# xcmyz/FastVocoder

Measured on AMD Instinct MI355X. Metric: audio samples/sec + RTF @22.05kHz, HiFi-GAN-light, 1/2/4/8 MI355X, higher is better.
Workload: dtype f32 (products as split-f16 pairs, fp32 accumulate); 1 GPU; HiFi-GAN light (conf/hifigan/light.yaml) generator forward, mel 80x1000, batch 1 utterance(s) per GPU, 240000 samples each; BASELINE.json configs[1]; global_batch=1, frames=1000, parallelism=single GPU, plan_ops_per_forward=33

## Files before the change

### fastvocoder_amd/_native.py

```python
import ctypes
import os
import subprocess

import torch

_HERE = os.path.dirname(os.path.abspath(__file__))
LIB_PATH = os.path.join(_HERE, "libfastvocoder_hip.so")
_CSRC = os.path.join(_HERE, "csrc")
SOURCES = ["conv_mfma.hip", "api.hip", "plan.hip", "pack.hip", "pqmf.hip", "wav_sink.hip", "mel.hip", "resample.hip", "griffin_lim.hip", "stft_loss.hip", "stft_loss_grad.hip", "stft_mag_grad.hip", "disc.hip", "disc_grad.hip", "disc_wgrad.hip", "mpd.hip", "mpd_grad.hip", "mpd_wgrad.hip", "gen_grad.hip", "gen_grad_bf16.hip", "basis_grad.hip", "basis_learn.hip", "optim.hip", "conv_inst_narrow.hip",
           "pair_launch.hip", "pair_inst_c16.hip", "pair_inst_c32.hip", "pairh_inst_c16.hip", "pairh_inst_c32.hip",
           "convh_launch.hip", "convh_inst_c64.hip", "convh_inst_c128.hip", "convt_inst.hip",
           "convg_inst.hip", "convr_inst.hip", "convtn_inst.hip", "convk_inst.hip", "convq2_inst.hip",
           "mrfh_launch.hip", "mrfh_inst_a.hip", "mrfh_inst_b.hip", "mrfw_inst.hip", "convtl_inst.hip", "convs2_inst.hip", "convu2_inst.hip"] + \
          [f"conv_inst_s{i}.hip" for i in range(6)]
HEADERS = ["fv_internal.h", "launch_host.hpp", "conv_kernels.hpp", "pair_kernels.hpp", "pair_inst.hpp", "pairh_kernels.hpp",
           "pairh_inst.hpp", "convh_kernels.hpp", "convh_inst.hpp", "convr_kernels.hpp",
           "convtn_kernels.hpp", "convk_kernels.hpp", "convq2_kernels.hpp", "mrfh_kernels.hpp", "mrfh_inst.hpp", "mrfw_kernels.hpp", "convtl_kernels.hpp", "convs2_kernels.hpp", "convu2_kernels.hpp", "api_internal.h", "stft_core.hpp", "basis_grad_host.hpp", "wgrad_tile.hpp", "gen_grad_host.hpp"]

PAD_ZERO, PAD_REFLECT = 0, 1
PAD_CAUSAL = 2
POST_NONE, POST_TANH, POST_RELU = 0, 1, 2
SLOT_NONE, SLOT_IN, SLOT_OUT, SLOT_TMP0, MAX_SLOTS = -1, 0, 1, 2, 32
SLOT_AUX_IN0, SLOT_AUX_IN1, SLOT_OUT2 = 28, 29, 30
ABI_VERSION = 18
# ... 260 lines not shown
                                     ctypes.POINTER(f), i, i, vp]
    L.fv_mpd_conv_first.argtypes = [vp, vp, vp, vp, i, i64, i, f, vp]
    L.fv_packed_period_conv_floats.argtypes = [i, i]
    L.fv_packed_period_conv_floats.restype = i64
    L.fv_pack_period_conv.argtypes = [vp, vp, i, i, vp]
    L.fv_period_conv.argtypes = [vp, vp, vp, vp, i, i, i, i, i, f, vp]
    L.fv_packed_period_conv_grad_floats.argtypes = [i, i]
    L.fv_packed_period_conv_grad_floats.restype = i64
    L.fv_pack_period_conv_grad.argtypes = [vp, vp, i, i, vp]
    L.fv_period_conv_input_grad.argtypes = [vp, vp, vp, vp, vp, i, i, i, i, i, f, vp]
    L.fv_mpd_first_input_grad.argtypes = [vp, vp, vp, vp, vp, i, i64, i, f, vp]
    L.fv_fold_batchnorm_conv.argtypes = [vp, vp, vp, vp, vp, vp, f, vp, vp, i, i, i, vp]
    L.fv_packed_upsample_conv1d_floats.argtypes = [i, i, i, i, i]
    L.fv_packed_upsample_conv1d_floats.restype = i64
    L.fv_pack_upsample_conv1d_weight.argtypes = [vp, vp, i, i, i, i, i, vp]
    L.fv_upsample_conv1d_fused.argtypes = [vp, vp, vp, vp, vp, i, i, i, i, i, i, i, f, i, f, vp]
    L.fv_plan_add_upsample_conv1d.argtypes = [vp, i, i, i, vp, vp, i, i, i, i, i, f, i, f]
    pp = ctypes.POINTER(vp)
    L.fv_packed_pair_floats.argtypes = [i, i]
    L.fv_packed_pair_floats.restype = i64
    L.fv_pack_pair_weight.argtypes = [vp, vp, i, i, vp]
    L.fv_resblock1_fused.argtypes = [i, pp, pp, pp, pp, pp, pp, pp, ctypes.POINTER(i), i, i, i, i, f, f, vp]
    L.fv_mrf_stage.argtypes = [pp, pp, pp, pp, pp, vp, vp, ctypes.POINTER(i), i, i, i, i, f, f, i, f, vp]
    L.fv_plan_add_resblock_pair.argtypes = [vp, i, i, i, vp, vp, vp, vp, i, i, i, f, f]
    L.fv_packed_pair_floats_ex.argtypes = [i, i, i]
    L.fv_packed_pair_floats_ex.restype = i64
    L.fv_pack_pair_weight_ex.argtypes = [vp, vp, i, i, i, vp, vp]
    L.fv_resblock1_fused_ex.argtypes = [i, pp, pp, pp, pp, pp, pp, pp, pp, pp, pp, ctypes.POINTER(i), i, i, i, i, f, f,
                                        i, f, i, vp, vp]
    L.fv_plan_add_resblock_pair_ex.argtypes = [vp, i, i, i, i, i, i, vp, vp, vp, vp, i, i, i, f, f, i, f, i]
    L.fv_conv1d_split_f16.argtypes = [i, pp, pp, pp, pp, pp, pp, pp, pp, ctypes.POINTER(i), i, i, i, i, i, f, f, i, f, vp, vp]
    L.fv_plan_set_pair_output_conv.argtypes = [vp, vp, vp, i, f, i]
    L.fv_packed_mrf_stage_floats.argtypes = [i, ctypes.POINTER(i)]
    L.fv_packed_mrf_stage_floats.restype = i64
    L.fv_pack_mrf_stage_split_f16.argtypes = [pp, pp, pp, pp, vp, i, ctypes.POINTER(i), vp, vp]
    L.fv_mrf_stage_workspace_bytes.argtypes = [i]
    L.fv_mrf_stage_workspace_bytes.restype = i64
    L.fv_mrf_stage_split_f16.argtypes = [vp, vp, vp, vp, i, i, i, ctypes.POINTER(i), ctypes.POINTER(i), f, f, i, f, vp, vp, vp,
                                         vp, i64, vp, vp]
    L.fv_plan_add_mrf_stage_split_f16.argtypes = [vp, i, i, i, vp, i, ctypes.POINTER(i), ctypes.POINTER(i), f, f, i, f, vp, i64]
    L.fv_plan_add_conv1d_split_f16.argtypes = [vp, i, i, i, i, i, i, vp, vp, i, i, i, i, f, f, i, f]
    L.fv_plan_add_mrf_sum.argtypes = [vp, ctypes.POINTER(i), i, i, pp, pp, pp, pp, i, ctypes.POINTER(i), i, f, f, i, f]
    L.fv_plan_create.argtypes = [i]
    L.fv_plan_create.restype = vp
    L.fv_plan_destroy.argtypes = [vp]
    L.fv_plan_destroy.restype = None
    L.fv_plan_add_conv1d.argtypes = [vp, i, i, i, i, i, i, vp, vp, i, i, i, i, i, i, f, f, i, f]
    L.fv_plan_add_conv_transpose1d.argtypes = [vp, i, i, i, vp, vp, i, i, i, i, i, i, f, i, f]
    L.fv_plan_add_pqmf_synthesis.argtypes = [vp, i, i, vp, i, i]
    L.fv_plan_set_guard.argtypes = [vp, vp]
    L.fv_plan_check_range.argtypes = [vp, vp]
    L.fv_tuning_set.argtypes = [ctypes.c_char_p, i]
    L.fv_debug_pair_schedule.argtypes = [i, ctypes.POINTER(i), ctypes.POINTER(i), i, i, i, ctypes.POINTER(ctypes.c_uint)]
    L.fv_plan_set_group.argtypes = [vp, i]
    L.fv_plan_output_shape.argtypes = [vp, i, ctypes.POINTER(i), ctypes.POINTER(i64)]
    L.fv_plan_workspace_bytes.argtypes = [vp, i, i]
    L.fv_plan_workspace_bytes.restype = i64
    L.fv_plan_run.argtypes = [vp, i, i, vp, vp, vp, i64, vp]
    L.fv_plan_run_aux.argtypes = [vp, i, i, vp, vp, vp, ctypes.POINTER(vp), ctypes.POINTER(i), vp, i64, vp]
    L.fv_plan_set_output_offset.argtypes = [vp, i, i]
    L.fv_plan_slot_shape.argtypes = [vp, i, i, ctypes.POINTER(i), ctypes.POINTER(i64)]
    L.fv_plan_num_ops.argtypes = [vp]
    L.fv_profile_enable.argtypes = [i]
    L.fv_profile_bracket_cost.argtypes = [vp, i, ctypes.POINTER(ctypes.c_double)]
    L.fv_profile_mfma_f16_rate.argtypes = [vp, i64, i, i, vp, ctypes.POINTER(ctypes.c_double)]
    L.fv_profile_collect.argtypes = [i, ctypes.POINTER(i64), ctypes.POINTER(ctypes.c_double),
                                     ctypes.POINTER(ctypes.c_double), ctypes.POINTER(ctypes.c_double)]
    if L.fv_version() != ABI_VERSION:
        raise NativeError(f"ABI mismatch: library reports {L.fv_version()}, binding expects {ABI_VERSION}")
    _lib = L
    return L


def check(rc):
    if rc != 0:
        raise NativeError(f"libfastvocoder_hip error {rc}: {lib().fv_last_error().decode()}")


def _ptr(t, name="tensor", allow_none=False):
    if t is None:
        if allow_none:
            return None
        raise NativeError(f"{name} is None")
    if not t.is_cuda:
        raise NativeError(f"{name} lives on {t.device}; the HIP kernels need a ROCm device "
                          "tensor (there is no CPU path in fastvocoder_amd)")
    if t.dtype != torch.float32 or not t.is_contiguous():
        raise NativeError(f"{name} must be contiguous float32, got {t.dtype} "
                          f"contiguous={t.is_contiguous()}")
    return t.data_ptr()


class _on:

    def __init__(self, *tensors):
        devs = {t.device for t in tensors if t is not None}
        if len(devs) != 1:
            raise NativeError(f"operands of a native call must share one ROCm device, got {sorted(map(str, devs))}")
        self.dev = devs.pop()
        if self.dev.type != "cuda":
            raise NativeError(f"operands live on {self.dev}; the HIP kernels need a ROCm device tensor "
                              "(there is no CPU path in fastvocoder_amd)")
        self._guard = torch.cuda.device(self.dev)

    def __enter__(self):
        self._guard.__enter__()
        return torch.cuda.current_stream(self.dev).cuda_stream

    def __exit__(self, *exc):
        return self._guard.__exit__(*exc)


class GuardWord:

    def __init__(self):
        self.t = torch.zeros(2, dtype=torch.int32).pin_memory()

    def ptr(self, i=0):
        return self.t.data_ptr() + 4 * i

    def peek(self, i=0):
        return int(self.t[i])

    def clear(self, i=0):
        self.t[i] = 0


def tuning_set(key, value):
    check(lib().fv_tuning_set(key.encode(), int(value)))


def debug_pair_schedule(n_items, cost, nblk, mode=0, three_members=False):
    n = len(n_items)
    arr = ctypes.c_int * n
    table = (ctypes.c_uint * 512)()
    rc = lib().fv_debug_pair_schedule(n, arr(*[int(v) for v in n_items]), arr(*[int(v) for v in cost]), int(nblk), int(mode),
                                      1 if three_members else 0, table)
    check(rc if rc < 0 else 0)
    if rc == 1:
        out = []
        for b in range(nblk):
            w0, w1 = table[2 * b], table[2 * b + 1]
            e = [w0 & 0xFFFF, w0 >> 16, w1 & 0xFFFF]
            out.append([(v & 2047, v >> 11) for v in e[:n]])
        return 1, out
    if rc == 2:
        return 2, [int(table[i]) for i in range(nblk)]
    return 0, None


def _flag_ptr(flag):
    if flag is None:
        return None
    if isinstance(flag, GuardWord):
        return flag.ptr(1)
    if isinstance(flag, int):
        return flag
    return flag.data_ptr()


def _guard_ptr(guard):
    if guard is None:
        return None
    if isinstance(guard, GuardWord):
        return guard.ptr(0)
    return guard.data_ptr()



def fold_weight_norm(v, g):
    v = v.detach().contiguous().float()
    g = g.detach().contiguous().float()
    w = torch.empty_like(v)
    with _on(v, g) as stream:
        check(lib().fv_fold_weight_norm(_ptr(v, "v"), _ptr(g, "g"), _ptr(w), v.shape[0], v[0].numel(), stream))
    return w


def pack_conv1d(w):
    w = w.detach().contiguous().float()
    cout, cin, k = w.shape
    out = torch.empty(lib().fv_packed_conv1d_floats(cout, cin, k), dtype=torch.float32, device=w.device)
    with _on(w) as stream:
        check(lib().fv_pack_conv1d_weight(_ptr(w, "w"), _ptr(out), cout, cin, k, stream))
    return out


def pack_conv_transpose1d(w, stride, pad):
    w = w.detach().contiguous().float()
    cin, cout, k = w.shape
    n = lib().fv_packed_conv_transpose1d_floats(cin, cout, k, stride, pad)
    out = torch.empty(n, dtype=torch.float32, device=w.device)
    with _on(w) as stream:
        check(lib().fv_pack_conv_transpose1d_weight(_ptr(w, "w"), _ptr(out), cin, cout, k, stride, pad, stream))
    return out


def conv_transpose_split_supported(cin, cout, k, stride, pad, out_pad):
    if conv_transpose_small(cin, cout, k, stride):
        return pad == 1 and out_pad == 0
    return (cin in (32, 64, 128, 256, 512) and 2 <= stride <= 16 and k == 2 * stride and cout * stride >= 32
# ... 170 lines not shown
def mrf_stage_workspace(channels, device):
    n = lib().fv_mrf_stage_workspace_bytes(int(channels))
    return torch.empty((n + 3) // 4, dtype=torch.float32, device=device) if n > 0 else None


def _work_args(work):
    return (_ptr(work, "workspace", True), 0 if work is None else work.numel() * 4)


def pack_mrf_stage(w1s, w2s, b1s, b2s, ks, flag=None):
    w1s = [w.detach().contiguous().float() for w in w1s]
    w2s = [w.detach().contiguous().float() for w in w2s]
    b1s = [None if b is None else b.detach().contiguous().float() for b in b1s]
    b2s = [None if b is None else b.detach().contiguous().float() for b in b2s]
    if not (len(w1s) == len(w2s) == len(b1s) == len(b2s) == 9 and len(ks) == 3):
        raise NativeError("pack_mrf_stage: nine pairs (three ResBlocks x three positions) expected")
    c = w1s[0].shape[0]
    for i, w in enumerate(w1s + w2s):
        if tuple(w.shape) != (c, c, ks[(i % 9) // 3]):
            raise NativeError(f"pack_mrf_stage: weight {i} has shape {tuple(w.shape)}, expected {(c, c, ks[(i % 9) // 3])}")
    karr = (ctypes.c_int * 3)(*ks)
    nfl = lib().fv_packed_mrf_stage_floats(c, karr)
    if nfl <= 0:
        raise NativeError(f"pack_mrf_stage: no packed layout for C={c} taps={list(ks)}")
    out = torch.empty(nfl, dtype=torch.float32, device=w1s[0].device)
    with _on(*w1s, *w2s, *b1s, *b2s, out) as stream:
        check(lib().fv_pack_mrf_stage_split_f16(_vp_array(w1s, "w1"), _vp_array(w2s, "w2"), _vp_array(b1s, "b1", True),
                                                _vp_array(b2s, "b2", True), _ptr(out), c, karr, _flag_ptr(flag), stream))
    return out


def mrf_stage_split_f16(x, packed, ks, dils=MRF_STAGE_DILATIONS, slope=0.1, out_div=3.0, post=POST_NONE, act_slope=1.0,
                        out=None, out_act=None, fold=None, guard=None):
    B, C, T = x.shape
    karr, darr = (ctypes.c_int * 3)(*ks), (ctypes.c_int * 3)(*dils)
    work = mrf_stage_workspace(C, x.device)
    if fold is not None:
        fw, fb = fold
        fw = fw.detach().contiguous().float()
        fb = None if fb is None else fb.detach().contiguous().float()
        res = torch.empty((B, 1, T), dtype=torch.float32, device=x.device)
        with _on(x, packed, fw, fb, res) as stream:
            check(lib().fv_mrf_stage_split_f16(_ptr(x, "x"), _ptr(packed, "packed"), None, None, B, C, T, karr, darr,
                                               float(slope), float(out_div), post, float(act_slope), _ptr(fw, "fold_w"),
                                               _ptr(fb, "fold_b", True), _ptr(res), *_work_args(work), _guard_ptr(guard), stream))
        return res
    if out is None:
        out = torch.empty_like(x)
    with _on(x, packed, out, out_act, work) as stream:
        check(lib().fv_mrf_stage_split_f16(_ptr(x, "x"), _ptr(packed, "packed"), _ptr(out, "y"), _ptr(out_act, "y_act", True),
                                           B, C, T, karr, darr, float(slope), float(out_div), post, float(act_slope), None,
                                           None, None, *_work_args(work), _guard_ptr(guard), stream))
    return out


def mrf_stage(xs, w1s, w2s, b1s, b2s, ks, dil, slope, out_div=3.0, post=POST_NONE, act_slope=1.0, out=None,
              out_act=None):
    B, C, T = xs[0].shape
    if out is None:
        out = torch.empty_like(xs[0])
    with _on(*xs, *w1s, *w2s, *b1s, *b2s, out, out_act) as stream:
        check(lib().fv_mrf_stage(_vp_array(xs, "x"), _vp_array(w1s, "w1"), _vp_array(w2s, "w2"),
                                 _vp_array(b1s, "b1", True), _vp_array(b2s, "b2", True), _ptr(out, "y"),
                                 _ptr(out_act, "y_act", True), (ctypes.c_int * 3)(*ks), B, C, T, dil, float(slope),
                                 float(out_div), post, float(act_slope), stream))
    return out


def conv1d_fused(x, packed, bias, cout, k, dil=1, pad=0, pad_mode=PAD_ZERO, pre_slope=1.0,
                 res=None, acc_in=None, out_div=1.0, post=POST_NONE, out=None, out_act=None,
                 act_slope=1.0, acc_in2=None):
    B, cin, T = x.shape
    tout = T if pad_mode & PAD_CAUSAL else T + 2 * pad - dil * (k - 1)
    if out is None:
        out = torch.empty((B, cout, tout), dtype=torch.float32, device=x.device)
    with _on(x, packed, bias, res, acc_in, acc_in2, out, out_act) as stream:
        check(lib().fv_conv1d_fused(_ptr(x, "x"), _ptr(packed, "packed"), _ptr(bias, "bias", True),
                                    _ptr(res, "res", True), _ptr(acc_in, "acc_in", True),
                                    _ptr(acc_in2, "acc_in2", True), _ptr(out, "out"),
                                    _ptr(out_act, "out_act", True), B, cin, cout, T, k, dil, pad, pad_mode,
                                    float(pre_slope), float(out_div), post, float(act_slope), stream))
    return out


def conv1d_2src_fused(x, x2, packed, bias, cout, res=None, post=POST_NONE, out=None, out_act=None,
                      act_slope=1.0):
    B, c1, T = x.shape
    c2 = x2.shape[1]
    if out is None:
        out = torch.empty((B, cout, T), dtype=torch.float32, device=x.device)
    with _on(x, x2, packed, bias, res, out, out_act) as stream:
        check(lib().fv_conv1d_2src_fused(_ptr(x, "x"), _ptr(x2, "x2"), _ptr(packed, "packed"),
                                         _ptr(bias, "bias", True), _ptr(res, "res", True), _ptr(out, "out"),
                                         _ptr(out_act, "out_act", True), B, c1, c2, cout, T, post,
                                         float(act_slope), stream))
    return out


def conv1x1_2src_split_f16(x, x2, packed, bias, pre_slope=1.0, res=None, post=POST_NONE, out=None, out_act=None,
                           act_slope=1.0, guard=None):
    B, c, T = x.shape
    if out is None:
        out = torch.empty_like(x)
    with _on(x, x2, packed, bias, res, out, out_act) as stream:
        check(lib().fv_conv1x1_2src_split_f16(_ptr(x, "x"), _ptr(x2, "x2"), _ptr(packed, "packed"), _ptr(bias, "bias", True),
                                              _ptr(res, "res", True), _ptr(out, "out"), _ptr(out_act, "out_act", True), B, c,
# ... 1049 lines not shown
        for b in (bias_dilated, bias_out):
            if b is not None:
                self.keep(b)
        check(lib().fv_plan_add_residual_stack_split_f16(self._h, x, y, y_act, _ptr(packed, "packed"),
                                                         _ptr(bias_dilated, "bias_dilated", True), _ptr(bias_out, "bias_out", True),
                                                         channels, k, dil, float(slope), pad_mode, post, float(act_slope)))
        if two_launch is not None:
            hidden, pd, pp = two_launch
            self.keep(pd)
            self.keep(pp)
            check(lib().fv_plan_set_stack_two_launch(self._h, hidden, _ptr(pd, "packed_dilated"), _ptr(pp, "packed_pair")))

    def add_upsample_conv1d(self, x, y, packed, bias, cin, cout, k, rate, pad, pre_slope=1.0,
                            post=POST_NONE, y_act=SLOT_NONE, act_slope=1.0):
        self.keep(packed)
        if bias is not None:
            self.keep(bias)
        check(lib().fv_plan_add_upsample_conv1d(self._h, x, y, y_act, _ptr(packed, "packed"),
                                                _ptr(bias, "bias", True), cin, cout, k, rate, pad,
                                                float(pre_slope), post, float(act_slope)))

    def add_conv1d_sum3(self, xs, ress, tmps, y, packed, bias_sum, channels, ks, out_div=1.0, post=POST_NONE,
                        y_act=SLOT_NONE, act_slope=1.0):
        for t in packed:
            self.keep(t)
        if bias_sum is not None:
            self.keep(bias_sum)
        i3 = ctypes.c_int * 3
        wp = (ctypes.c_void_p * 3)(*[_ptr(t, "packed") for t in packed])
        check(lib().fv_plan_add_conv1d_sum3(self._h, i3(*xs), i3(*ress), (ctypes.c_int * 2)(*tmps), y, y_act, wp,
                                            _ptr(bias_sum, "bias_sum", True), channels, i3(*ks),
                                            float(out_div), post, float(act_slope)))

    def add_resblock_pair(self, x, y, packed1, packed2, bias1, bias2, channels, k, dil, slope,
                          y_act=SLOT_NONE, act_slope=1.0, prec=PAIR_F32, add1=SLOT_NONE, add2=SLOT_NONE,
                          out_div=1.0, post=POST_NONE, mid=SLOT_NONE):
        for t in (packed1, packed2, bias1, bias2):
            if t is not None:
                self.keep(t)
        check(lib().fv_plan_add_resblock_pair_ex(self._h, x, y, y_act, mid, add1, add2, _ptr(packed1, "packed1"),
                                                 _ptr(packed2, "packed2"), _ptr(bias1, "bias1", True),
                                                 _ptr(bias2, "bias2", True), channels, k, dil, float(slope),
                                                 float(out_div), post, float(act_slope), prec))

    def add_mrf_stage(self, x, y, packed, channels, ks, dils, slope, out_div=3.0, post=POST_NONE, y_act=SLOT_NONE,
                      act_slope=1.0):
        self.keep(packed)
        work = mrf_stage_workspace(channels, packed.device)
        if work is not None:
            self.keep(work)
        check(lib().fv_plan_add_mrf_stage_split_f16(self._h, x, y, y_act, _ptr(packed, "packed"), channels,
                                                    (ctypes.c_int * 3)(*ks), (ctypes.c_int * 3)(*dils), float(slope),
                                                    float(out_div), post, float(act_slope), *_work_args(work)))

    def set_pair_output_conv(self, w, bias, y, act_slope, post=POST_NONE):
        self.keep(w)
        if bias is not None:
            self.keep(bias)
        check(lib().fv_plan_set_pair_output_conv(self._h, _ptr(w, "w"), _ptr(bias, "bias", True), y, float(act_slope), post))

    def add_conv1d_split_f16(self, x, y, packed, bias, channels, k, dil, pre_slope=1.0, res=SLOT_NONE, add1=SLOT_NONE,
                             add2=SLOT_NONE, out_div=1.0, post=POST_NONE, y_act=SLOT_NONE, act_slope=1.0,
                             pad_mode=PAD_ZERO):
        for t in (packed, bias):
            if t is not None:
                self.keep(t)
        check(lib().fv_plan_add_conv1d_split_f16(self._h, x, y, y_act, res, add1, add2, _ptr(packed, "packed"),
                                                 _ptr(bias, "bias", True), channels, k, dil, pad_mode,
                                                 float(pre_slope), float(out_div), post, float(act_slope)))

    def add_mrf_sum(self, xs, y, packed1, packed2, bias1, bias2, channels, ks, dil, slope, out_div=3.0,
                    post=POST_NONE, y_act=SLOT_NONE, act_slope=1.0):
        for t in list(packed1) + list(packed2) + list(bias1) + list(bias2):
            if t is not None:
                self.keep(t)
        i3 = ctypes.c_int * 3
        check(lib().fv_plan_add_mrf_sum(self._h, i3(*xs), y, y_act, _vp_array(packed1, "packed1"),
                                        _vp_array(packed2, "packed2"), _vp_array(bias1, "bias1", True),
                                        _vp_array(bias2, "bias2", True), channels, i3(*ks), dil, float(slope),
                                        float(out_div), post, float(act_slope)))

    def set_sum_order(self, own_first):
        check(lib().fv_plan_set_sum_order(self._h, 1 if own_first else 0))

    def set_guard(self, guard):
        self._guard = self.keep(guard) if guard is not None else None
        check(lib().fv_plan_set_guard(self._h, guard.ptr(0) if guard is not None else None))

    def check_range(self):
        if self._guard is None:
            return False
        rc = lib().fv_plan_check_range(self._h, torch.cuda.current_stream(self._dev).cuda_stream)
        if rc == ERR_RANGE:
            return True
        if rc == ERR_RANGE_LOW:
            return "low"
        check(rc)
        return False

    def set_group(self, group):
        check(lib().fv_plan_set_group(self._h, group))

    def add_pqmf_synthesis(self, x, y, h):
        self.keep(h)
        check(lib().fv_plan_add_pqmf_synthesis(self._h, x, y, _ptr(h, "h"), h.shape[0], h.shape[1]))

# ... 129 lines not shown
```

### fastvocoder_amd/csrc/api.hip

```cpp
#include <stdarg.h>
#include <stdio.h>
#include <stdlib.h>

#include <string>
#include <mutex>
#include <utility>
#include <vector>

#include <ctype.h>
#include <string.h>
#include <unistd.h>

#include "api_internal.h"
#include "launch_host.hpp"

namespace fv {

static thread_local std::string g_err;

int fail(int code, const char* fmt, ...) {
    char buf[512];
    va_list ap;
    va_start(ap, fmt);
    vsnprintf(buf, sizeof(buf), fmt, ap);
// ... 182 lines not shown
    pp.T = (int)T;
    pp.slope = o.pre_slope;
    pp.act_slope = o.act_slope;
    pp.out_div = o.out_div;
    pp.post = o.post;
    pp.prec = o.prec;
    pp.guard = guard;
    pp.reflect = (o.pad_mode & FV_PAD_REFLECT) ? 1 : 0;
    pp.sub = sub;
    pp.sub_batched = sub_batched;
    return pp;
}

PairMember pair_member(const float* x, const float* w1, const float* w2, const float* b1, const float* b2, int k, float* y,
                       float* y_act, const float* res, const float* add1, const float* add2, const float* x2) {
    PairMember mb = {};
    mb.x = x;
    mb.x2 = x2;
    mb.w1 = w1;
    mb.w2 = w2;
    mb.b1 = b1;
    mb.b2 = b2;
    mb.k = k;
    mb.y = y;
    mb.y_act = y_act;
    mb.res = res;
    mb.add1 = add1;
    mb.add2 = add2;
    return mb;
}

MrfParams mrf_params(const Op& o, const float* x, float* y, float* y_act, float* fold_y, int B, int64_t T, int* guard) {
    MrfParams mp = {};
    mp.x = x;
    mp.y = y;
    mp.y_act = y_act;
    mp.blob = o.wp;
    for (int j = 0; j < 3; ++j) mp.k[j] = o.pk[j];
    mp.B = B;
    mp.T = (int)T;
    mp.slope = o.pre_slope;
    mp.out_div = o.out_div;
    mp.act_slope = o.act_slope;
    mp.post = o.post;
    mp.fold_w = o.fold_w;
    mp.fold_b = o.fold_b;
    mp.fold_y = fold_y;
    mp.guard = guard;
    mp.hist = static_cast<float*>(o.work);
    mp.hist_bytes = o.work_bytes;
    return mp;
}

int check_pad_mode(int pad_mode, int pad, int k, int dil) {
    if (pad_mode < 0 || pad_mode > (FV_PAD_REFLECT | FV_PAD_CAUSAL))
        return fail(FV_ERR_INVALID_ARG, "unknown pad_mode %d", pad_mode);
    if ((pad_mode & FV_PAD_CAUSAL) && 2LL * pad < (int64_t)dil * (k - 1))
        return fail(FV_ERR_INVALID_ARG, "causal conv: pad=%d leaves fewer than Tin outputs (k=%d dil=%d)",
                    pad, k, dil);
    return 0;
}

int check_conv_args(int Cin, int Cout, int k, int dil) {
    if (Cin <= 0 || Cout <= 0 || k <= 0 || dil <= 0)
        return fail(FV_ERR_INVALID_ARG, "bad conv shape Cin=%d Cout=%d k=%d dil=%d", Cin, Cout, k, dil);
    return 0;
}

int check_convt_split_args(int Cin, int Cout, int k, int stride, int pad, int out_pad) {
    if (Cin != 32 && Cin != 64 && Cin != 128 && Cin != 256 && Cin != 512)
        return fail(FV_ERR_UNSUPPORTED, "conv_transpose1d_split_f16: Cin = %d (32, 64, 128, 256 or 512)", Cin);
    if (stride < 2 || stride > 16 || k != 2 * stride)
        return fail(FV_ERR_UNSUPPORTED, "conv_transpose1d_split_f16: kernel %d, stride %d (kernel = 2 x stride, stride 2..16)", k, stride);
    if (Cout <= 0 || Cout * stride < 32)
        return fail(FV_ERR_UNSUPPORTED, "conv_transpose1d_split_f16: Cout * stride = %d (32 or more)", Cout * stride);
    if (pad < 0 || pad > stride || out_pad < -stride || out_pad >= stride)
        return fail(FV_ERR_INVALID_ARG, "conv_transpose1d_split_f16: pad=%d (0..stride) out_pad=%d", pad, out_pad);
    if (convtn_shape(Cin, Cout, k, stride) && (pad != 1 || out_pad != 0))
        return fail(FV_ERR_UNSUPPORTED, "conv_transpose1d_split_f16: 32 -> 16 channels, kernel 4, stride 2 exists with pad=1, "
                    "out_pad=0 only (got %d, %d)", pad, out_pad);
    return 0;
}

}

using namespace fv;

namespace fv {
int allow_dynamic_lds(const void* kernel, size_t bytes) {
    if (bytes <= 64 * 1024) return 0;
    struct Grant { const void* kernel; int device; size_t bytes; };
    static std::mutex mu;
    static std::vector<Grant> granted;
    int dev = 0;
    FV_HIP(hipGetDevice(&dev));
    std::lock_guard<std::mutex> lock(mu);
    for (Grant& g : granted)
        if (g.kernel == kernel && g.device == dev) {
            if (g.bytes >= bytes) return 0;
            FV_HIP(hipFuncSetAttribute(kernel, hipFuncAttributeMaxDynamicSharedMemorySize, (int)bytes));
            g.bytes = bytes;
            return 0;
        }
    FV_HIP(hipFuncSetAttribute(kernel, hipFuncAttributeMaxDynamicSharedMemorySize, (int)bytes));
    granted.push_back({kernel, dev, bytes});
    return 0;
}

static Tuning g_tuning;
static std::once_flag g_tuning_once;
struct TuningEntry {
    const char* key;
    int Tuning::*field;
};
static const TuningEntry kTuningTable[] = {
    {"pair_dbg", &Tuning::pair_dbg},       {"dbg", &Tuning::conv_dbg},           {"sched", &Tuning::sched},
    {"sched_switch", &Tuning::sched_switch}, {"convh_skel", &Tuning::convh_skel}, {"convp_skel", &Tuning::convp_skel},
    {"convq_skel", &Tuning::convq_skel},   {"pair128_unfused", &Tuning::pair128_unfused},
    {"convg_rows64", &Tuning::convg_rows64}, {"stack_items", &Tuning::stack_items}, {"stack_wide", &Tuning::stack_wide},
    {"convp_wide", &Tuning::convp_wide},   {"convq_wide", &Tuning::convq_wide},
    {"convh_rows64", &Tuning::convh_rows64},  {"convt_rows64", &Tuning::convt_rows64},
    {"pairh_skel", &Tuning::pairh_skel},   {"pair_skel", &Tuning::pair_skel},    {"convh_blocks", &Tuning::convh_blocks},
    {"pair_blocks", &Tuning::pair_blocks}, {"sum3_min", &Tuning::sum3_min},      {"lds_budget", &Tuning::lds_budget},
    {"units", &Tuning::units},             {"shape16", &Tuning::shape16},        {"shape32", &Tuning::shape32},
    {"shape64", &Tuning::shape64},         {"krows", &Tuning::krows},            {"grid_cap", &Tuning::grid_cap},
    {"no_group", &Tuning::no_group},       {"mrf_blocks", &Tuning::mrf_blocks},  {"mrf_shape", &Tuning::mrf_shape},
    {"mrf_prio", &Tuning::mrf_prio},       {"convt_lean", &Tuning::convt_lean},
    {"convs_ringfree", &Tuning::convs_ringfree}, {"convu_resident", &Tuning::convu_resident},
};
static void tuning_from_env() {
    const char* on = getenv("FV_TUNING");
    if (!on || atoi(on) != 1) return;
    for (const TuningEntry& e : kTuningTable) {
        char name[64] = "FV_";
        size_t n = 3;
        for (const char* c = e.key; *c && n + 1 < sizeof(name); ++c) name[n++] = (char)toupper((unsigned char)*c);
        name[n] = 0;
        const char* v = getenv(name);
        if (v && *v) g_tuning.*(e.field) = atoi(v);
    }
    const char* tp = getenv("FV_PAIR_TRACE_PTR");
    if (tp && *tp) g_tuning.trace_ptr = strtoull(tp, nullptr, 0);
}
const Tuning& tuning() {
    std::call_once(g_tuning_once, tuning_from_env);
    return g_tuning;
}

int device_cu_count() {
    static int cus = 0;
    if (!cus) {
        int dev = 0, v = 0;
        cus = hipGetDevice(&dev) == hipSuccess &&
                      hipDeviceGetAttribute(&v, hipDeviceAttributeMultiprocessorCount, dev) == hipSuccess && v > 0
                  ? v : 256;
    }
    return cus;
}
}

extern "C" {

int fv_version(void) { return FV_ABI_VERSION; }


#ifndef FV_BUILD_ID
#define FV_BUILD_ID "unknown"
#endif
const char* fv_build_id(void) { return "fv-build-id:" FV_BUILD_ID + 12; }

const char* fv_last_error(void) { return g_err.c_str(); }

int fv_upsample_conv1d_fused(const float* x, const float* packed, const float* bias, float* y,
                             float* y_act, int B, int Cin, int Cout, int Tin, int k, int rate, int pad,
                             float pre_slope, int post, float act_slope, void* stream) {
    if (int rc = check_conv_args(Cin, Cout, k, 1)) return rc;
    if (!x || !packed || !y) return fail(FV_ERR_INVALID_ARG, "upsample_conv1d: null tensor");
    if (rate <= 0 || pad < 0) return fail(FV_ERR_INVALID_ARG, "upsample_conv1d: rate=%d pad=%d", rate, pad);
    if (x == y || x == y_act || (y_act && y_act == y))
        return fail(FV_ERR_INVALID_ARG, "upsample_conv1d: y / y_act must not alias x or each other");
// ... 718 lines not shown
    }
    return launch_pair_family(pp, mid, C, dil, prec, (hipStream_t)stream);
}

int fv_mrf_stage(const float* const* x, const float* const* w1, const float* const* w2, const float* const* b1,
                 const float* const* b2, float* y, float* y_act, const int* k, int B, int C, int T, int dil,
                 float slope, float out_div, int post, float act_slope, void* stream) {
    if (!x || !w1 || !w2 || !y || !k) return fail(FV_ERR_INVALID_ARG, "mrf_stage: null argument");
    if (int rc = check_pair_args(3, C, k, dil)) return rc;
    PairParams pp = pair_params(pair_op(OP_MRFSUM, C, dil, FV_PAD_ZERO, slope, out_div, post, act_slope, FV_PAIR_F32), 3, B, T, nullptr);
    pp.sum = 1;
    for (int j = 0; j < 3; ++j) {
        if (!x[j] || x[j] == y || x[j] == y_act || (y_act && y_act == y))
            return fail(FV_ERR_INVALID_ARG, "mrf_stage: member %d: null input, or y / y_act aliases an input or each other", j);
        pp.m[j] = pair_member(x[j], w1[j], w2[j], at(b1, j), at(b2, j), k[j], y, y_act);
    }
    return launch_pairs(pp, C, dil, (hipStream_t)stream);
}

}

namespace fv {
int check_stage_args(int C, const int* k, const int* dil, float slope, float act_slope, int post) {
    if (!k || !dil) return fail(FV_ERR_INVALID_ARG, "mrf stage: null taps / dilations");
    if (!mrf_stage_shape(C, k, dil))
        return fail(FV_ERR_UNSUPPORTED, "mrf stage: C = %d, taps (%d, %d, %d), dilations (%d, %d, %d): built for 16 / 32 channels, "
                    "taps 3 / 7 / 11, dilations (1, 3, 5)", C, k[0], k[1], k[2], dil[0], dil[1], dil[2]);
    if (int rc = check_slopes("mrf stage", slope, act_slope)) return rc;
    if (post != FV_POST_NONE && post != FV_POST_TANH && post != FV_POST_RELU) return fail(FV_ERR_INVALID_ARG, "mrf stage: post %d", post);
    return 0;
}
}

extern "C" {

int64_t fv_mrf_stage_workspace_bytes(int C) { return mrf_workspace_bytes(C); }

int fv_mrf_stage_split_f16(const float* x, const float* packed, float* y, float* y_act, int B, int C, int T, const int* k,
                           const int* dil, float slope, float out_div, int post, float act_slope, const float* fold_w,
                           const float* fold_b, float* fold_y, void* workspace, int64_t workspace_bytes, int* guard,
                           void* stream) {
    if (int rc = check_stage_args(C, k, dil, slope, act_slope, post)) return rc;
    if (B < 0 || T < 0) return fail(FV_ERR_INVALID_ARG, "mrf stage: B=%d T=%d", B, T);
    Op o = pair_op(OP_STAGE, C, dil[0], FV_PAD_ZERO, slope, out_div, post, act_slope, FV_PAIR_SPLIT_F16);
    o.wp = packed;
    for (int j = 0; j < 3; ++j) o.pk[j] = k[j];
    o.fold_w = fold_w;
    o.fold_b = fold_b;
    o.work = workspace;
    o.work_bytes = workspace_bytes;
    return launch_mrfh(mrf_params(o, x, y, y_act, fold_y, B, T, guard), C, dil, (hipStream_t)stream);
}

}

namespace fv {
int check_convh_args(int n, int C, const int* k, int dil, int pad_mode) {
    if (pad_mode != FV_PAD_ZERO && pad_mode != FV_PAD_REFLECT)
        return fail(FV_ERR_UNSUPPORTED, "conv1d_split_f16: pad_mode %d (FV_PAD_ZERO or FV_PAD_REFLECT)", pad_mode);
    if (n < 1 || n > 3) return fail(FV_ERR_INVALID_ARG, "conv1d_split_f16: %d members (1..3)", n);
    if (C != 64 && C != 128 && C != 256 && C != 512)
        return fail(FV_ERR_UNSUPPORTED, "conv1d_split_f16: C = %d (64, 128, 256 or 512)", C);
    if (dil != 1 && dil != 3 && dil != 5 && dil != 9)
        return fail(FV_ERR_UNSUPPORTED, "conv1d_split_f16: dilation %d (1, 3, 5; 9 with 3 taps)", dil);
    for (int j = 0; j < n; ++j)
        if ((k[j] != 3 && k[j] != 7 && k[j] != 11) || (dil == 9 && k[j] != 3))
            return fail(FV_ERR_UNSUPPORTED, "conv1d_split_f16: %d taps at dilation %d (3, 7 or 11; 3 at dilation 9)", k[j], dil);
    return 0;
}
}

extern "C" {

int fv_conv1d_split_f16(int n, const float* const* x, const float* const* packed, const float* const* bias,
                        const float* const* res, const float* const* add1, const float* const* add2, float* const* y,
                        float* const* y_act, const int* k, int B, int C, int T, int dil, int pad_mode, float pre_slope,
                        float out_div, int post, float act_slope, int* guard, void* stream) {
    if (!x || !packed || !y || !k) return fail(FV_ERR_INVALID_ARG, "conv1d_split_f16: null argument");
    if (int rc = check_convh_args(n, C, k, dil, pad_mode)) return rc;
    PairParams pp = pair_params(pair_op(OP_CONVH, C, dil, pad_mode, pre_slope, out_div, post, act_slope, FV_PAIR_SPLIT_F16), n, B, T, guard);
    for (int j = 0; j < n; ++j) {
        const PairMember& mb = pp.m[j] = pair_member(x[j], packed[j], nullptr, at(bias, j), nullptr, k[j], y[j], at(y_act, j),
                                                     at(res, j), at(add1, j), at(add2, j));
        if (!mb.x || !mb.y || mb.x == mb.y || mb.y == mb.res || mb.y == mb.add1 || mb.y == mb.add2 ||
            (mb.y_act && (mb.y_act == mb.y || mb.y_act == mb.x || mb.y_act == mb.res)))
            return fail(FV_ERR_INVALID_ARG, "conv1d_split_f16: member %d: null tensor or an output aliases an input", j);
    }
    return launch_convh(pp, C, dil, (hipStream_t)stream);
}

int fv_div_probe(unsigned first_bits, int64_t n, float d, unsigned long long* mismatches, void* stream) {
    if (!mismatches || n <= 0) return fail(FV_ERR_INVALID_ARG, "div_probe: null counter / empty range");
    return fv::launch_div_probe(first_bits, (long long)n, d, mismatches, (hipStream_t)stream);
}

int fv_tuning_set(const char* key, int value) {
    if (!key) return fail(FV_ERR_INVALID_ARG, "tuning_set: null key");
    (void)tuning();
    for (const TuningEntry& e : kTuningTable)
        if (strcmp(e.key, key) == 0) {
            g_tuning.*(e.field) = value;
            return 0;
        }
    static const char* const kRetiredKeys[] = {"convp_pp"};
    for (const char* retired : kRetiredKeys)
        if (value == 0 && strcmp(retired, key) == 0) return 0;
// ... 135 lines not shown
```

### fastvocoder_amd/csrc/api_internal.h

```cpp
#pragma once
#include <stdint.h>

#include <vector>

#include "fv_internal.h"

namespace fv {

enum OpType { OP_CONV = 0, OP_CONVT = 1, OP_PQMF = 2, OP_UPCONV = 3, OP_PAIR = 4, OP_MRFSUM = 5, OP_CONVH = 6, OP_CONVG = 7, OP_STACK = 8, OP_STAGE = 9 };

struct Op {
    int type;
    int x, y, res, acc, y2, acc2;
    int group;
    const float* wp;
    const float* bias;
    const float* bias2 = nullptr;
    const float* alt_w1 = nullptr;
    const float* alt_w2 = nullptr;
    int alt_mid = FV_SLOT_NONE;
    int Cin, Cout, k, dil, pad, pad_mode, stride, out_pad;
    float pre_slope, out_div, act_slope;
    int post;
    int x2 = FV_SLOT_NONE;
    int Cin1 = 0;
    int own_first = 0;
    bool sum3 = false;
    int xb = FV_SLOT_NONE, xc = FV_SLOT_NONE, resb = FV_SLOT_NONE, resc = FV_SLOT_NONE;
    int tmpb = FV_SLOT_NONE, tmpc = FV_SLOT_NONE;
    const float* wpb = nullptr;
    const float* wpc = nullptr;
    int kb = 0, kc = 0;
    const float* pw1[3] = {nullptr, nullptr, nullptr};
    const float* pw2[3] = {nullptr, nullptr, nullptr};
    const float* pb1[3] = {nullptr, nullptr, nullptr};
    const float* pb2[3] = {nullptr, nullptr, nullptr};
    int pk[3] = {0, 0, 0};
    int sdil[3] = {0, 0, 0};
    void* work = nullptr;
    int64_t work_bytes = 0;
    int prec = 0;
    bool in_merge = false;
    const float* fold_w = nullptr;
    const float* fold_b = nullptr;
    int sub = FV_SLOT_NONE;
    const float* pq_h = nullptr;
    int pq_taps = 0;
};

struct Shape {
    int C;
    int64_t T;
    bool set;
};

}

struct fv_plan {
    int in_channels;
    std::vector<fv::Op> ops;
    int cur_group = 0;
    int cur_own_first = 0;
    int* guard_host = nullptr;
    int* guard_dev = nullptr;
};

namespace fv {

int64_t conv_out_len(const Op& o, int64_t Tin);
ConvParams make_params(const Op& o, const float* x, float* y, float* y2, const float* res,
                              const float* acc, const float* acc2, int B, int64_t Tin,
                              const float* x2 = nullptr, const float* sub = nullptr, int sub_batched = 0);
int run_op(const Op& o, const float* x, float* y, float* y2, const float* res, const float* acc,
                  const float* acc2, int B, int64_t Tin, hipStream_t s, const float* x2 = nullptr,
                  const float* sub = nullptr, int sub_batched = 0, int* guard = nullptr);
int check_pad_mode(int pad_mode, int pad, int k, int dil);
int check_stack_args(int C, int k, int dil, int pad_mode, float slope, float act_slope, int post = FV_POST_NONE);

inline float* ptr(float* const* base, int slot) { return slot == FV_SLOT_NONE ? nullptr : base[slot]; }
PairParams pair_params(const Op& o, int n_members, int B, int64_t T, int* guard, const float* sub = nullptr, int sub_batched = 0);
PairMember pair_member(const float* x, const float* w1, const float* w2, const float* b1, const float* b2, int k, float* y,
                       float* y_act, const float* res = nullptr, const float* add1 = nullptr, const float* add2 = nullptr,
                       const float* x2 = nullptr);
MrfParams mrf_params(const Op& o, const float* x, float* y, float* y_act, float* fold_y, int B, int64_t T, int* guard);
int launch_pair_family(const PairParams& pp, float* const* mid, int C, int dil, int prec, hipStream_t s);
int check_pair_args(int n, int C, const int* k, int dil, int prec = FV_PAIR_F32);
int check_stage_args(int C, const int* k, const int* dil, float slope, float act_slope, int post);
int check_convh_args(int n, int C, const int* k, int dil, int pad_mode);

}
```

### fastvocoder_amd/csrc/convtn_kernels.hpp

```cpp
#pragma once
#include "pairh_kernels.hpp"

namespace fv {

struct ConvTnParams {
    const float* x;
    const float* add1;
    const float* add2;
    const float* w;
    const float* bias;
    float* y;
    float* y_act;
    int B, T, Tout, n_tiles;
    float slope, act_slope, out_div;
    int* guard;
};

constexpr int kTnCin = 32, kTnCout = 16, kTnCols = 256, kTnRows = 260, kTnRP = 272;
constexpr int kTnHalf = (kTnCin / 8) * kTnRP * 16;
constexpr int kTnImageFloats = 2 * 2 * 2 * 64 * 8 / 2;

__global__ __launch_bounds__(256) __attribute__((amdgpu_waves_per_eu(2, 2))) void convtn_kernel(ConvTnParams p) {
    typedef __attribute__((address_space(3))) const f16x8 LdsH8;
    __shared__ __attribute__((aligned(16))) char ximg[2 * kTnHalf];
    __shared__ unsigned lowbits[4];
    const int tid = threadIdx.x, lane = tid & 63;
    const int wave = __builtin_amdgcn_readfirstlane(tid >> 6);
    const int b = (int)blockIdx.x / p.n_tiles, tile = (int)blockIdx.x - b * p.n_tiles;
    const int u0 = tile * kTnCols;
    const size_t xoff = (size_t)b * kTnCin * (size_t)p.T;
    const unsigned xbytes = (unsigned)kTnCin * (unsigned)p.T * 4u, t4 = (unsigned)p.T * 4u;
    const __amdgpu_buffer_rsrc_t r0 = make_rsrc(p.x + xoff, xbytes);
    const __amdgpu_buffer_rsrc_t r1 = make_rsrc(p.add1 ? p.add1 + xoff : p.x, p.add1 ? xbytes : 0u);
    const __amdgpu_buffer_rsrc_t r2 = make_rsrc(p.add2 ? p.add2 + xoff : p.x, p.add2 ? xbytes : 0u);
    constexpr int TASKS = kTnRows * (kTnCin / 8), NR = (TASKS + 255) / 256;
    float v[NR][8], a1[NR][8], a2[NR][8];
    const bool merge = p.add1 != nullptr;
#pragma unroll
    for (int q = 0; q < NR; ++q) {
        const int idx = tid + q * 256;
        const int cb = idx / kTnRows, row = idx - cb * kTnRows;
        const int t = u0 - 1 + row;
        const unsigned voff = idx < TASKS && t >= 0 && t < p.T ? (unsigned)(cb * 8 * p.T + t) * 4u : kOutOfRange;
#pragma unroll
        for (int j = 0; j < 8; ++j) v[q][j] = buffer_load1s(r0, voff, (unsigned)j * t4);
        if (merge) {
#pragma unroll
            for (int j = 0; j < 8; ++j) a1[q][j] = buffer_load1s(r1, voff, (unsigned)j * t4);
#pragma unroll
            for (int j = 0; j < 8; ++j) a2[q][j] = buffer_load1s(r2, voff, (unsigned)j * t4);
        }
    }
    pair_wait_vm0();
    float lowm = 0.f;
    const float rcp = div_rcp(p.out_div);
#pragma unroll
    for (int q = 0; q < NR; ++q) {
        const int idx = tid + q * 256;
        const int cb = idx / kTnRows, row = idx - cb * kTnRows;
        if (idx < TASKS) {
            F16x8Parts h1, h2;
#pragma unroll
            for (int j = 0; j < 4; ++j) {
                f32x2 raw = {v[q][2 * j], v[q][2 * j + 1]};
                if (merge) {
                    raw = (raw + f32x2{a1[q][2 * j], a1[q][2 * j + 1]}) + f32x2{a2[q][2 * j], a2[q][2 * j + 1]};
                    if (p.out_div != 1.f) {
                        raw.x = rcp != 0.f ? div_exact(raw.x, p.out_div, rcp) : raw.x / p.out_div;
                        raw.y = rcp != 0.f ? div_exact(raw.y, p.out_div, rcp) : raw.y / p.out_div;
                    }
                }
                const f32x2 a = split_act2(raw, p.slope);
                lowm = low_max3(lowm, a.x, a.y);
                split2(a, h1.p[j], h2.p[j]);
            }
            *reinterpret_cast<f16x8*>(ximg + (cb * kTnRP + row) * 16) = __builtin_bit_cast(f16x8, h1);
            *reinterpret_cast<f16x8*>(ximg + (cb * kTnRP + row) * 16 + kTnHalf) = __builtin_bit_cast(f16x8, h2);
        }
    }
    f16x8 A[2][2][2];
    {
        const f16x8* wl = reinterpret_cast<const f16x8*>(p.w) + lane;
#pragma unroll
        for (int s = 0; s < 2; ++s)
#pragma unroll
            for (int h = 0; h < 2; ++h)
#pragma unroll
                for (int e = 0; e < 2; ++e) A[s][h][e] = wl[((s * 2 + h) * 2 + e) * 64];
    }
    LowGuard low;
    low_note(low, 0, lowm);
    if (p.guard && lane == 0) lowbits[wave] = low.bits;
    pair_barrier();
    if (p.guard && tid == 0) {
        const unsigned all = lowbits[0] | lowbits[1] | lowbits[2] | lowbits[3];
        if ((all & 2u) && !(all & 1u)) guard_raise_low(p.guard);
    }
    const int n = lane & 15, kb = lane >> 4;
    const int col0 = wave * 64 + n;
    LdsCF* const bb = lds_opaque(reinterpret_cast<const float*>(ximg + (kb * kTnRP + col0) * 16));
    f32x4 hi[2][4], lo[2][4];
#pragma unroll
    for (int h = 0; h < 2; ++h)
#pragma unroll
        for (int f = 0; f < 4; ++f) hi[h][f] = lo[h][f] = f32x4{0.f, 0.f, 0.f, 0.f};
#pragma unroll
    for (int s = 0; s < 2; ++s) {
        f16x8 B1[4], B2[4];
#pragma unroll
        for (int f = 0; f < 4; ++f) {
            B1[f] = *reinterpret_cast<LdsH8*>(bb + (s * 16 + f * 256) / 4);
            B2[f] = *reinterpret_cast<LdsH8*>(bb + (s * 16 + f * 256 + kTnHalf) / 4);
        }
#pragma unroll
        for (int h = 0; h < 2; ++h)
#pragma unroll
            for (int f = 0; f < 4; ++f) hi[h][f] = __builtin_amdgcn_mfma_f32_16x16x32_f16(A[s][h][0], B1[f], hi[h][f], 0, 0, 0);
#pragma unroll
        for (int h = 0; h < 2; ++h)
// ... 58 lines not shown
```

### fastvocoder_amd/csrc/fv_internal.h

```cpp
#pragma once
#include <hip/hip_runtime.h>

#include <vector>
#include <stdint.h>

#include "../../include/fastvocoder_hip.h"

namespace fv {

int fail(int code, const char* fmt, ...);

#define FV_HIP(call)                                                              \
    do {                                                                          \
        hipError_t e_ = (call);                                                   \
        if (e_ != hipSuccess)                                                     \
            return ::fv::fail((int)e_, "%s failed: %s", #call, hipGetErrorString(e_)); \
    } while (0)

static inline int round_up(int v, int m) { return (v + m - 1) / m * m; }

int check_conv_args(int Cin, int Cout, int k, int dil);
int check_convt_split_args(int Cin, int Cout, int k, int stride, int pad, int out_pad);

static inline int pad_rows(int M) { return M <= 16 ? 16 : round_up(M, 32); }
// ... 54 lines not shown
    int nchunks;
    int xw;
    int ncol4;
    int ncol4c;
    unsigned ncol4c_magic;
    int xbuf, wbuf;
    int n_tiles;
    int m_tiles, tiles_per_run;
    int nx_inst, nw_inst;
    int red_off;
    int vec_ok;
    int dbg;
    double alg_flops;
};

struct GroupParams {
    ConvParams p[3];
    int grid_x[3];
};

struct Sum3Params {
    ConvParams p[3];
    int xbuf_max, wbuf_max;
};
int launch_conv_sum3(ConvParams* ps, hipStream_t stream);

int allow_dynamic_lds(const void* kernel, size_t bytes);
int device_cu_count();
struct Tuning {
    int pair_dbg = 0;
    int conv_dbg = 0;
    int sched = 1;
    int sched_switch = 4;
    int convh_skel = -1;
    int convp_skel = 5;
    int convq_skel = -1;
    int pair128_unfused = 0;
    int convh_rows64 = -1;
    int convt_rows64 = -1;
    int convs_ringfree = -1;
    int convu_resident = 1;
    int convt_lean = 50;
    int convq_wide = 20;
    int convp_wide = 20;
    int stack_wide = 10;
    int stack_items = 1 << 20;
    int convg_rows64 = -1;
    int pairh_skel = -1;
    int pair_skel = -1;
    int convh_blocks = 0;
    int pair_blocks = 0;
    int mrf_blocks = 0;
    int mrf_shape = 0;
    int mrf_prio = 1;
    int sum3_min = 800;
    int lds_budget = 39;
    int units = 500;
    int shape16 = -1, shape32 = -1, shape64 = -1;
    int krows = 176;
    int grid_cap = 1024;
    int no_group = 0;
    unsigned long long trace_ptr = 0;
};
const Tuning& tuning();

struct PairMember {
    const float* x;
    const float* x2;
    const float* w1;
    const float* w2;
    const float* b1;
    const float* b2;
    float* y;
    float* y_act;
    const float* res;
    int n_items;
    const float* add1;
    const float* add2;
    int k;
    int cost;
    int n_tiles;
    int w_off;
};

constexpr int kSchedBlocks = 256;

struct PairCore {
    PairMember m[3];
    int n_members;
    int sum;
    int B, T;
    int n_out_sum;
    float slope;
    float out_div;
    float act_slope;
    int post;
    int nblk;
    int ctot, nch, nmt;
    const float* fold_w;
    const float* fold_b;
    float* fold_y;
    const float* sub;
    int sub_batched;
    int* guard;
    int sched_on;
    int reflect;
// ... 81 lines not shown
int launch_pair_geom(const PairParams& p, int dil, size_t lds, hipStream_t s);
template <int MH, int NF, int NG>
int launch_pairh_geom(const PairParams& p, int dil, size_t lds, hipStream_t s);

struct MrfParams {
    const float* x;
    float* y;
    float* y_act;
    const float* blob;
    unsigned blob_bytes;
    unsigned blk_off[9];
    int k[3];
    int B, T;
    int halo;
    int ol;
    float slope;
    float out_div;
    float act_slope;
    int post;
    const float* fold_w;
    const float* fold_b;
    float* fold_y;
    int* guard;
    int nblk;
    long long total;
    int prio;
    unsigned long long* trace;
    float* hist;
    long long hist_bytes;
};

inline int mrf_block_bytes(int C, int k) { return 2 * ((k + (32 / C) - 1) / (32 / C)) * (C / 16) * 2048 + 1024; }
inline bool mrf_stage_shape(int C, const int* k, const int* dil) {
    if ((C != 16 && C != 32) || !k || !dil || dil[0] != 1 || dil[1] != 3 || dil[2] != 5) return false;
    for (int j = 0; j < 3; ++j)
        if (k[j] != 3 && k[j] != 7 && k[j] != 11) return false;
    return true;
}
inline int mrf_halo(const int* k, const int* dil) {
    int h = 0;
    for (int j = 0; j < 3; ++j) {
        int r = 0;
        for (int q = 0; q < 3; ++q) r += (k[j] - 1) * dil[q] / 2 + (k[j] - 1) / 2;
        if (r > h) h = r;
    }
    return h;
}
int launch_mrfh(MrfParams p, int C, const int* dil, hipStream_t stream);
template <int NF, int NG>
int launch_mrfh_geom(const MrfParams& p, hipStream_t s);
constexpr int kMrfwHistBytes = 9 * 30 * 128;
long long mrf_workspace_bytes(int C);
int launch_mrfw_geom(const MrfParams& p, hipStream_t s);

#ifndef FV_RING
#define FV_RING 2
#endif
constexpr int kRingStages(bool slow, bool act) { return (slow || act) ? 2 : FV_RING; }
constexpr int kMaxDmaX = 6, kMaxDmaW = 8;

struct PqmfTail {
    const float* h;
    float* y;
    float* y2;
    const float* sub;
    int sub_batched;
    int ntaps;
    int tail_off;
};
constexpr int kPqmfHalo = 8, kPqmfAdvance = 256 - 2 * kPqmfHalo;
int launch_conv_post_pqmf(ConvParams p, const float* h, int ntaps, float* y, float* y2, const float* sub, int sub_batched,
                          hipStream_t stream);

int launch_conv(ConvParams p, hipStream_t stream);
int launch_conv_group(ConvParams* ps, int n, hipStream_t stream);
int launch_pqmf(const float* x, const float* h, float* y, float* y2, const float* sub, int sub_batched, int B, int S,
                int ntaps, int Tsub, hipStream_t stream);
int launch_encode16(float* x, int B, int64_t n, float rescale, short* out, unsigned* peak_bits,
                    int scale_in_place, hipStream_t s);
int launch_pqmf_analysis(const float* xin, const float* ha, float* x, int B, int S, int ntaps,
                         int64_t T, hipStream_t s);
int launch_melspectrogram(const float* x, float* mel, const float* tab, int B, int64_t n, hipStream_t s);
int launch_stft_complex(const float* y, float* spec, const float* tab, int B, int64_t n, hipStream_t s);
int launch_istft(const float* spec, float* y, const float* tab, int B, int T, float* frames, hipStream_t s);
int launch_griffin_lim(const float* S, const float* phase0, float* y, const float* tab, int B, int T, int iters,
                       float* frames, hipStream_t s);
int launch_mel_to_linear(const float* mel, const float* invb, float* S, int B, int T, float power, hipStream_t s);
int launch_inv_preemphasis(const float* y, float* out, int B, int64_t n, float coef, hipStream_t s);
static inline int64_t resample_window(int L, int M, int half) {
    return ((int64_t)L - 1 + 255 * (int64_t)M) / L + 2 * (int64_t)half + 2;
}
int launch_resample(const void* x, int format, float* y, const float* tab, int B, int64_t n_in, int64_t n_out, int L,
                    int M, int half, hipStream_t s);
int64_t stft_chunks(int64_t n, int hop);
int launch_stft_distance(const float* x, const float* y, const float* const* tables, int B, int64_t n, int R,
                         const int* nfft, const int* hop, const int* win, double* out, double* ws, hipStream_t s);
int launch_stft_magnitude(const float* x, float* mag, const float* tab, int B, int64_t n, int nfft, int hop, int win,
                          hipStream_t s, bool bins_major = false);
int64_t stft_grad_chunks(int64_t n, int hop);
int launch_stft_distance_grad(const float* x, const float* y, const float* const* tables, int B, int64_t n, int R,
                              const int* nfft, const int* hop, const int* win, const float* coef, float* gx,
                              float* ws, hipStream_t s);
int launch_stft_grad_ola(const float* ws, const float* tab, int B, int64_t n, int nfft, int hop, int win, float* gx,
                         hipStream_t s);
int64_t stft_mag_grad_chunks(int64_t n, int hop);
int launch_stft_magnitude_bins_grad(const float* x, const float* gmag, const float* tab, int B, int64_t n, int nfft,
// ... 35 lines not shown
```

### fastvocoder_amd/csrc/mrfh_launch.hip

```cpp
#include "launch_host.hpp"

namespace fv {

extern template int launch_mrfh_geom<3, 12>(const MrfParams&, hipStream_t);
extern template int launch_mrfh_geom<2, 16>(const MrfParams&, hipStream_t);

static long long mrfw_max_blocks() {
    const long long cus = device_cu_count(), asked = tuning().mrf_blocks;
    return asked > cus ? asked : cus;
}
long long mrf_workspace_bytes(int C) { return C == 32 ? mrfw_max_blocks() * kMrfwHistBytes : 0; }

int launch_mrfh(MrfParams p, int C, const int* dil, hipStream_t s) {
    const char* const fam = "mrf stage";
    if (p.B <= 0 || p.T <= 0) return 0;
    if (!mrf_stage_shape(C, p.k, dil))
        return fail(FV_ERR_UNSUPPORTED, "mrf stage: C = %d, taps (%d, %d, %d), dilations (%d, %d, %d): built for 16 / 32 channels, taps "
                    "3 / 7 / 11, dilations (1, 3, 5)", C, p.k[0], p.k[1], p.k[2], dil ? dil[0] : 0, dil ? dil[1] : 0, dil ? dil[2] : 0);
    const bool fold = p.fold_w != nullptr;
    if (!p.x || !p.blob || (!fold && !p.y) || (fold && (!p.fold_y || p.y || p.y_act)))
        return fail(FV_ERR_INVALID_ARG, "mrf stage: null tensor (or both an output tensor and a folded output conv)");
    if (p.y == p.x || p.y_act == p.x || (p.y_act && p.y_act == p.y) || p.fold_y == p.x)
        return fail(FV_ERR_INVALID_ARG, "mrf stage: an output tensor aliases the input (or y_act aliases y)");
    if ((reinterpret_cast<uintptr_t>(p.blob) & 15) != 0) return fail(FV_ERR_UNSUPPORTED, "mrf stage: the packed stage must be 16-byte aligned");
    if (int rc = check_desc_range(fam, C, p.T)) return rc;
    if ((double)p.B * p.T >= 2147483647.0) return fail(FV_ERR_UNSUPPORTED, "mrf stage: B x T = %d x %d columns exceed 2^31", p.B, p.T);
    if (int rc = check_slopes(fam, p.slope, p.act_slope)) return rc;
    unsigned off = 0;
    double flops = 0;
    for (int j = 0; j < 3; ++j)
        for (int q = 0; q < 3; ++q) {
            p.blk_off[3 * j + q] = off;
            off += (unsigned)mrf_block_bytes(C, p.k[j]);
            flops += 2.0 * 2.0 * p.B * (double)C * C * p.k[j] * p.T;
        }
    p.blob_bytes = off;
    p.halo = mrf_halo(p.k, dil);
    p.ol = fold ? 3 : 0;
    p.total = (long long)p.B * p.T;
    const int shape = tuning().mrf_shape;
    const int W = C == 32 ? 384 : shape == 1 ? 512 : 576;
    const int vcols = W - p.halo, adv = vcols - 2 * p.ol;
    if (adv < 64) return fail(FV_ERR_UNSUPPORTED, "mrf stage: a %d-column window leaves %d final columns", W, adv);
    long long nblk = persistent_blocks((p.total + 127) / 128, 1, tuning().mrf_blocks);
    if (nblk < 1) nblk = 1;
    p.nblk = (int)nblk;
    if (C == 32) {
        if (!p.hist || p.hist_bytes < nblk * kMrfwHistBytes || (reinterpret_cast<uintptr_t>(p.hist) & 15) != 0)
            return fail(FV_ERR_WORKSPACE, "mrf stage: 32 channels need a 16-byte aligned workspace of fv_mrf_stage_workspace_bytes "
                        "(%lld bytes for %lld blocks; given %lld)", nblk * kMrfwHistBytes, nblk, p.hist ? p.hist_bytes : 0LL);
    } else {
        p.hist = nullptr;
    }
    p.prio = tuning().mrf_prio;
    p.trace = trace_buffer();
    double bytes = 4.0 * ((double)p.B * C * p.T * (fold ? 1.0 : (p.y_act ? 3.0 : 2.0)) + (fold ? (double)p.B * p.T : 0.0)) + off;
    if (fold) flops += 2.0 * p.B * (double)C * 7 * p.T;
    ProfileScope prof(s, C == 32 ? FV_KERNEL_MRF32 : FV_KERNEL_MRF16, Work{flops, bytes});
    return C == 32 ? launch_mrfw_geom(p, s) : shape == 1 ? launch_mrfh_geom<2, 16>(p, s) : launch_mrfh_geom<3, 12>(p, s);
}

}
```

### fastvocoder_amd/csrc/mrfw_inst.hip

```cpp
#include "mrfw_kernels.hpp"

namespace fv {

int launch_mrfw_geom(const MrfParams& p, hipStream_t s) {
    typedef MrfwTile<3, 8> TL;
    static_assert(9 * TL::HSLOT == kMrfwHistBytes, "history bytes per block");
    auto kern = p.fold_w ? mrfw_kernel<3, 8, 1, 3, 5, true> : mrfw_kernel<3, 8, 1, 3, 5, false>;
    if (int rc = allow_dynamic_lds(reinterpret_cast<const void*>(kern), TL::LDS)) return rc;
    hipLaunchKernelGGL(kern, dim3(p.nblk), dim3(TL::NT), TL::LDS, s, p);
    FV_HIP(hipGetLastError());
    return 0;
}

}
```

### fastvocoder_amd/csrc/mrfw_kernels.hpp

```cpp
#pragma once
#include "mrfh_kernels.hpp"

namespace fv {

template <int NF_, int NG_>
struct MrfwTile {
    static constexpr int NF = NF_, NG = NG_, C = 32;
    static constexpr int NT = 64 * NG;
    static constexpr int W = 16 * NF * NG;
    static constexpr int FM = 32;
    static constexpr int RP = W + 2 * FM;
    static constexpr int BLK = RP * 16;
    static constexpr int HALF = 4 * BLK;
    static constexpr int IMG = 2 * HALF;
    static constexpr int PT = 4;
    static constexpr int STEP = 4096;
    static constexpr int PIECE = PT * STEP;
    static constexpr int TAIL = 512;
    static constexpr int HROW = 128;
    static constexpr int HX = 0, HM = 25 * HROW, HSLOT = 30 * HROW;
    static constexpr int OFF_W = 0, OFF_X = 2 * PIECE, OFF_M = OFF_X + IMG, OFF_B = OFF_M + IMG, OFF_S = OFF_B + 9 * TAIL;
    static constexpr int OFF_F = OFF_S + 256;
    static constexpr int LDS = OFF_F + 1024;
    static_assert(W * 128 <= IMG, "FOLD: the activated fp32 tile [column][32 channels] lies over the intermediate image");
    static_assert(RP % 16 == 0, "whole bank rows");
    static_assert(NG >= 5 && NG <= 8, "history copies: waves 0 ... 4; a piece is at most two LDS-DMA instructions per wave");
    static_assert(LDS <= 160 * 1024, "LDS");
};

template <class TL>
struct MrfwLane {
    int tid, lane, wave;
    int colw;
    int row0;
    int rdoff;
    int wroff;
    int cpslot;
    int cpimg;
    char* sm;
};

template <int NG>
__device__ __forceinline__ void mrfw_dma(__amdgpu_buffer_rsrc_t rb, float* dst, unsigned off, int kb, int wave, int lane) {
#pragma unroll
    for (int r = 0; r < 2; ++r) {
        const int i = wave + r * NG;
        if (i < kb) dma16(rb, dst + i * 256, off + (unsigned)(i * 1024 + lane * 16));
    }
}

template <int NF, int STEPS, int TAPB, int HALF>
__device__ __forceinline__ void mrfw_mma(const float* wl, const char* img, f32x4 (&hi)[2][NF], f32x4 (&lo)[2][NF], int lane) {
    typedef __attribute__((address_space(3))) const f16x8 LdsH8;
// ... 175 lines not shown
    mrfw_conv<TL, KT, 16>(p, L, wbuf, par, mimg + (rdoff - P2 * 16), hi, lo, rb, pair_off + (unsigned)WB, next_off, next_kb);
    mrf_stamp(p, TL::NG, L.wave, L.lane, tile_no, 7 * q + 4);
    {
        u32x4 hv = {0u, 0u, 0u, 0u};
        if (wv == 4) {
            if (wh.save && cpslot < TL::HROW * P2) hv = *reinterpret_cast<const u32x4*>(mimg + cpimg + (TL::FM + wh.adv - P2) * 16);
        } else if (wv < 4) {
            if (!wh.zero_next && cpslot < TL::HROW * pnext) hv = __builtin_bit_cast(u32x4, __builtin_amdgcn_raw_buffer_load_b128(rh, hq_next + TL::HX + cpslot, 0, 0));
        }
#pragma unroll
        for (int h = 0; h < 2; ++h) {
            const f32x2* const b2 = reinterpret_cast<const f32x2*>(bl + 32 + 16 * h + row0);
            const f32x2* const s2 = reinterpret_cast<const f32x2*>(bl + 96 + 16 * h + row0);
            const f32x2 b01 = b2[0], b23 = b2[1], s01 = s2[0], s23 = s2[1];
            if (wh.inside) {
#pragma unroll
                for (int f = 0; f < NF; ++f) {
                    combine4(hi[h][f], lo[h][f], s01, s23, b01, b23, xr[h][f]);
#pragma unroll
                    for (int i = 0; i < 4; ++i) xr[h][f][i] = hi[h][f][i];
                }
            } else {
                int cm = colw;
                asm volatile("" : "+v"(cm));
#pragma unroll
                for (int f = 0; f < NF; ++f) {
                    combine4(hi[h][f], lo[h][f], s01, s23, b01, b23, xr[h][f]);
                    const int t = wh.tw + cm + f * 16;
                    const bool ok = t >= 0 && t < p.T;
#pragma unroll
                    for (int i = 0; i < 4; ++i) xr[h][f][i] = ok ? hi[h][f][i] : 0.f;
                }
            }
        }
        if (wv == 4) {
            if (wh.save && cpslot < TL::HROW * P2) __builtin_amdgcn_raw_buffer_store_b128(hv, rh, hq + TL::HM + cpslot, 0, 0);
        }
        if constexpr (NEXT == 0) mrfw_write_x<TL>(ximg + wroff, xr, p.slope, low);
        else if (write_next) mrfw_write_x<TL>(ximg + wroff, x0, p.slope, low);
        if (wv < 4) {
            if (cpslot < TL::HROW * pnext) *reinterpret_cast<u32x4*>(ximg + cpimg + (TL::FM - pnext) * 16) = hv;
        }
    }
    mrf_stamp(p, TL::NG, L.wave, L.lane, tile_no, 7 * q + 5);
    pair_wait_vm0();
    mrf_stamp(p, TL::NG, L.wave, L.lane, tile_no, 7 * q + 6);
    pair_barrier();
}

template <class TL, int KT, int D0, int D1, int D2>
__device__ __forceinline__ void mrfw_block_run(const MrfParams& p, const MrfwLane<TL>& L, float* wbuf, int& par, int j, int pnext,
                                               float (&xr)[2][TL::NF][4], const float (&x0)[2][TL::NF][4], bool write_next,
                                               MrfwWhen wh, bool zero_after, LowGuard& low, __amdgpu_buffer_rsrc_t rb,
                                               __amdgpu_buffer_rsrc_t rh, unsigned next_off, int next_kb, int tile_no) {
    constexpr int KB0 = 4 * mrfw_piece_taps(KT, 0);
    const int q0 = 3 * j;
    const float* const bl = reinterpret_cast<const float*>(L.sm + TL::OFF_B) + q0 * (TL::TAIL / 4);
    const int h0 = q0 * TL::HSLOT, hn = (j == 2 ? 0 : q0 + 3) * TL::HSLOT;
    const unsigned o0 = p.blk_off[q0], o1 = p.blk_off[q0 + 1], o2 = p.blk_off[q0 + 2];
    mrfw_pair<TL, KT, D0, 0>(p, L, wbuf, par, bl, xr, x0, true, wh, h0, h0 + TL::HSLOT, (KT - 1) * D1 / 2, low, rb, rh, o0, o1, KB0,
                             tile_no, q0);
    mrfw_pair<TL, KT, D1, 0>(p, L, wbuf, par, bl + TL::TAIL / 4, xr, x0, true, wh, h0 + TL::HSLOT, h0 + 2 * TL::HSLOT,
                             (KT - 1) * D2 / 2, low, rb, rh, o1, o2, KB0, tile_no, q0 + 1);
    wh.zero_next = zero_after;
    mrfw_pair<TL, KT, D2, 1>(p, L, wbuf, par, bl + 2 * (TL::TAIL / 4), xr, x0, write_next, wh, h0 + 2 * TL::HSLOT, hn, pnext, low, rb,
                             rh, o2, next_off, next_kb, tile_no, q0 + 2);
}

template <int NF, int NG, int D0, int D1, int D2, bool FOLD>
__global__ __launch_bounds__(64 * NG) __attribute__((amdgpu_waves_per_eu((NG + 3) / 4, (NG + 3) / 4))) void mrfw_kernel(MrfParams p) {
    typedef MrfwTile<NF, NG> TL;
    extern __shared__ __attribute__((aligned(16))) float smem[];
    char* const sm = reinterpret_cast<char*>(smem);
    MrfwLane<TL> L;
    L.tid = threadIdx.x;
    L.lane = L.tid & 63;
    L.wave = __builtin_amdgcn_readfirstlane(L.tid >> 6);
    L.sm = sm;
    {
        const int n = L.lane & 15, g = L.lane >> 4;
        L.colw = L.wave * (16 * NF) + n;
        L.row0 = 4 * g;
        L.rdoff = (g * TL::RP + TL::FM + L.colw) * 16;
        L.wroff = ((g >> 1) * TL::RP + TL::FM + L.colw) * 16 + 8 * (g & 1);
        const int u = L.tid & 255, part = u & 7, row = u >> 3;
        L.cpslot = u * 16;
        L.cpimg = (part >> 2) * TL::HALF + (part & 3) * TL::BLK + row * 16;
    }
    char* const ximg0 = sm + TL::OFF_X;
    char* const mimg0 = sm + TL::OFF_M;
    float* const wbuf = smem + TL::OFF_W / 4;
    float* const scratch = smem + TL::OFF_S / 4;
    const int T = p.T, halo = p.halo, ol = p.ol;
    const int vcols = TL::W - halo;
    const int adv = vcols - 2 * ol;
    const int k0 = p.k[0], k1 = p.k[1], k2 = p.k[2];
    const unsigned off0 = p.blk_off[0], off3 = p.blk_off[3], off6 = p.blk_off[6];
    asm volatile("" ::"s"(T), "s"(halo), "s"(ol), "s"(k0), "s"(k1), "s"(k2), "s"(off0), "s"(off3), "s"(off6));
    const __amdgpu_buffer_rsrc_t rb = make_rsrc(p.blob, p.blob_bytes);
    const __amdgpu_buffer_rsrc_t rh = make_rsrc(p.hist + (size_t)blockIdx.x * (9 * TL::HSLOT / 4), p.hist ? 9 * TL::HSLOT : 0);

    const int share = xcd_remap((int)blockIdx.x, (int)gridDim.x);
    const long long g_lo = p.total * share / p.nblk, g_hi = p.total * (share + 1) / p.nblk;
    if (g_lo >= g_hi) return;
    MrfIter it;
    mrf_first(it, g_lo, g_hi, T, halo, ol, vcols);

    const unsigned t4 = (unsigned)T * 4u, ubytes = (unsigned)TL::C * (unsigned)T * 4u;
    const size_t ustride = (size_t)TL::C * (size_t)T;
    float x0[2][NF][4], xr[2][NF][4], sum[2][NF][4];
    auto load_x0 = [&](const MrfIter& at) {
        const __amdgpu_buffer_rsrc_t rx = make_rsrc(p.x + at.b * ustride, ubytes);
#pragma unroll
        for (int h = 0; h < 2; ++h)
#pragma unroll
            for (int f = 0; f < NF; ++f) {
                const int t = at.tw + L.colw + f * 16;
                const unsigned voff = t >= 0 && t < T ? (unsigned)((L.row0 + 16 * h) * T + t) * 4u : kOutOfRange;
#pragma unroll
                for (int i = 0; i < 4; ++i) x0[h][f][i] = buffer_load1s(rx, voff, (unsigned)i * t4);
            }
    };
    u32x4 warm0, warm1;
    {
        const unsigned per_xcd = gridDim.x >= 8 ? gridDim.x >> 3 : 1u;
        const unsigned slice = ((p.blob_bytes + per_xcd - 1) / per_xcd + 15u) & ~15u;
        const unsigned lo = ((blockIdx.x >> 3) % per_xcd) * slice;
        const unsigned o0 = (unsigned)L.tid * 16u, o1 = o0 + TL::NT * 16u;
        warm0 = __builtin_bit_cast(u32x4, __builtin_amdgcn_raw_buffer_load_b128(rb, (int)(o0 < slice ? lo + o0 : kOutOfRange), 0, 0));
        warm1 = __builtin_bit_cast(u32x4, __builtin_amdgcn_raw_buffer_load_b128(rb, (int)(o1 < slice ? lo + o1 : kOutOfRange), 0, 0));
        for (unsigned o = o1 + TL::NT * 16u; o < slice; o += TL::NT * 16u) {
            const u32x4 w = __builtin_bit_cast(u32x4, __builtin_amdgcn_raw_buffer_load_b128(rb, (int)(lo + o), 0, 0));
            asm volatile("" ::"v"(w));
        }
    }
    load_x0(it);
    mrfw_dma<NG>(rb, wbuf, off0, 4 * (k0 < 4 ? k0 : 4), L.wave, L.lane);
    for (int idx = L.tid; idx < 2 * 8 * 2 * TL::FM * 4; idx += TL::NT) {
        const int dw = idx & 3, row = (idx >> 2) % TL::FM, fb = (idx >> 2) / TL::FM % 2, part = (idx >> 2) / (2 * TL::FM) % 8,
                  im = (idx >> 2) / (16 * TL::FM);
        char* const img = im ? mimg0 : ximg0;
        reinterpret_cast<float*>(img + (part >> 2) * TL::HALF + (part & 3) * TL::BLK + ((fb ? TL::FM + TL::W : 0) + row) * 16)[dw] = 0.f;
    }
    for (int idx = L.tid; idx < 9 * (TL::TAIL / 4); idx += TL::NT) {
        const int q = idx >> 7, e = idx & 127, j = q / 3;
        const int kj = j == 0 ? k0 : j == 1 ? k1 : k2;
        const unsigned base = (j == 0 ? off0 : j == 1 ? off3 : off6) + (unsigned)((q - 3 * j) * (2 * kj * TL::STEP + 1024));
        reinterpret_cast<float*>(sm + TL::OFF_B)[idx] = p.blob[(base + 2u * (unsigned)kj * TL::STEP) / 4 + e];
    }
    if constexpr (FOLD) {
        float* const fw = reinterpret_cast<float*>(sm + TL::OFF_F);
        if (L.tid < 224) {
            const int q = L.tid / 28, j = (L.tid % 28) / 4, cc = L.tid & 3;
            fw[L.tid] = p.fold_w[(4 * q + cc) * 7 + j];
        }
        if (L.tid == 224) fw[224] = p.fold_b ? p.fold_b[0] : 0.f;
    }
    LowGuard low;
    float bad = 0.f;
    const float rcp = div_rcp(p.out_div);
    mrf_stamp(p, NG, L.wave, L.lane, 2, 0);
    pair_wait_vm0();
    asm volatile("" ::"v"(warm0), "v"(warm1));
    mrf_stamp(p, NG, L.wave, L.lane, 2, 1);
    mrfw_write_x<TL>(ximg0 + L.wroff, x0, p.slope, low);
    pair_barrier();
    int tile_no = 0, par = 0;
    for (;;) {
        const MrfIter cur = it;
        const bool more = mrf_next(it, g_hi, T, halo, ol, vcols, adv);
        MrfwWhen wh;
        wh.tw = cur.tw;
        wh.inside = cur.tw >= 0 && cur.tw + TL::W <= T;
        wh.adv = adv;
        wh.save = more && !it.cold;
        wh.zero_mid = wh.zero_next = cur.cold;
#pragma unroll 1
        for (int j = 0; j < 3; ++j) {
            const int kj = j == 0 ? k0 : j == 1 ? k1 : k2, kn = j == 0 ? k1 : j == 1 ? k2 : k0;
            const unsigned offn = j == 0 ? off3 : j == 1 ? off6 : off0;
            const int kbn = (j < 2 || more) ? 4 * (kn < 4 ? kn : 4) : 0;
            const int pnext = (kn - 1) * D0 / 2;
            const bool zero_after = j == 2 ? !wh.save : cur.cold;
#pragma unroll
            for (int h = 0; h < 2; ++h)
#pragma unroll
                for (int f = 0; f < NF; ++f)
#pragma unroll
                    for (int i = 0; i < 4; ++i) xr[h][f][i] = x0[h][f][i];
            if (j == 2 && more) load_x0(it);
            const bool wn = j < 2 || more;
            if (kj == 11) mrfw_block_run<TL, 11, D0, D1, D2>(p, L, wbuf, par, j, pnext, xr, x0, wn, wh, zero_after, low, rb, rh, offn, kbn, tile_no);
            else if (kj == 7) mrfw_block_run<TL, 7, D0, D1, D2>(p, L, wbuf, par, j, pnext, xr, x0, wn, wh, zero_after, low, rb, rh, offn, kbn, tile_no);
            else mrfw_block_run<TL, 3, D0, D1, D2>(p, L, wbuf, par, j, pnext, xr, x0, wn, wh, zero_after, low, rb, rh, offn, kbn, tile_no);
            if (j < 2) {
#pragma unroll
                for (int h = 0; h < 2; ++h)
#pragma unroll
                    for (int f = 0; f < NF; ++f)
#pragma unroll
                        for (int i = 0; i < 4; ++i) sum[h][f][i] = j == 0 ? xr[h][f][i] : sum[h][f][i] + xr[h][f][i];
            }
        }
        if (tile_no == 0) mrf_stamp(p, NG, L.wave, L.lane, 2, 2);
        if constexpr (FOLD) {
            char* const sb = mimg0;
#pragma unroll
            for (int h = 0; h < 2; ++h) {
                float out[NF][4];
#pragma unroll
                for (int f = 0; f < NF; ++f)
#pragma unroll
                    for (int i = 0; i < 4; ++i) out[f][i] = sum[h][f][i] + xr[h][f][i];
                if (rcp != 0.f) {
#pragma unroll
                    for (int f = 0; f < NF; ++f)
#pragma unroll
                        for (int i = 0; i < 4; ++i) out[f][i] = div_exact(out[f][i], p.out_div, rcp);
                } else if (p.out_div != 1.f) {
#pragma unroll
                    for (int f = 0; f < NF; ++f)
#pragma unroll
                        for (int i = 0; i < 4; ++i) out[f][i] = out[f][i] / p.out_div;
                }
#pragma unroll
                for (int f = 0; f < NF; ++f) {
                    const int col = L.colw + f * 16, t = cur.tw + col;
                    const bool ok = t >= 0 && t < T;
                    range_note4(bad, out[f][0], out[f][1], out[f][2], out[f][3], t >= cur.lo - ol && t < cur.hi + ol && ok);
                    f32x4 v;
#pragma unroll
                    for (int i = 0; i < 4; ++i) v[i] = ok ? act(out[f][i], p.act_slope) : 0.f;
                    *reinterpret_cast<f32x4*>(sb + col * 128 + (((4 * h + (L.row0 >> 2)) + (col >> 1)) & 7) * 16) = v;
                }
            }
            pair_barrier();
            const float* const fw = reinterpret_cast<const float*>(sm + TL::OFF_F);
            for (int c0 = L.tid; c0 < vcols - 2 * ol; c0 += TL::NT) {
                const int col = c0 + ol, t = cur.tw + col;
                float o = 0.f;
#pragma unroll 1
                for (int q = 0; q < 8; ++q) {
                    f32x4 d[7], w[7];
#pragma unroll
                    for (int j = 0; j < 7; ++j) {
                        const int row = col - 3 + j;
                        d[j] = *reinterpret_cast<const f32x4*>(sb + row * 128 + ((q + (row >> 1)) & 7) * 16);
                        w[j] = *reinterpret_cast<const f32x4*>(fw + (q * 7 + j) * 4);
                    }
#pragma unroll
                    for (int cc = 0; cc < 4; ++cc)
#pragma unroll
                        for (int j = 0; j < 7; ++j) o = fmaf(w[j][cc], d[j][cc], o);
                }
                o = o + fw[224];
                if (p.post == FV_POST_TANH) o = tanhf(o);
                else if (p.post == FV_POST_RELU) o = fmaxf(o, 0.f);
                if (t >= cur.lo && t < cur.hi) p.fold_y[(size_t)cur.b * T + t] = o;
// ... 66 lines not shown
```

### fastvocoder_amd/csrc/plan.hip

```cpp
#include <stdarg.h>
#include <stdio.h>
#include <stdlib.h>
#include <string.h>

#include <initializer_list>
#include <string>
#include <utility>
#include <vector>

#include "api_internal.h"
#include "launch_host.hpp"

using namespace fv;

namespace fv {

static int out_channels(const Op& o) { return (o.type == OP_PQMF || o.pq_h) ? 1 : o.Cout; }

static void put_shape(Shape* sh, int64_t* slot_elems, int B, int slot, int C, int64_t T) {
    sh[slot] = {C, T, true};
    const int64_t e = (int64_t)B * C * T;
    if (slot_elems && e > slot_elems[slot]) slot_elems[slot] = e;
}

// ... 358 lines not shown
    if (int rc = check_slot(x_slot, false)) return rc;
    if (int rc = check_slot(y_slot, false)) return rc;
    Op o = {};
    o.type = OP_PQMF;
    o.x = x_slot;
    o.y = y_slot;
    o.y2 = FV_SLOT_NONE;
    o.res = FV_SLOT_NONE;
    o.acc = FV_SLOT_NONE;
    o.acc2 = FV_SLOT_NONE;
    o.wp = h;
    o.Cin = S;
    o.Cout = 1;
    o.k = ntaps;
    plan->ops.push_back(o);
    return 0;
}

int fv_plan_add_mrf_stage_split_f16(fv_plan_t* plan, int x_slot, int y_slot, int y_act_slot, const float* packed, int C,
                                    const int* k, const int* dil, float slope, float out_div, int post, float act_slope,
                                    void* workspace, int64_t workspace_bytes) {
    if (!plan || !packed) return fail(FV_ERR_INVALID_ARG, "plan_add_mrf_stage: null");
    if (int rc = check_stage_args(C, k, dil, slope, act_slope, post)) return rc;
    if (workspace_bytes < mrf_workspace_bytes(C) || (mrf_workspace_bytes(C) > 0 && !workspace))
        return fail(FV_ERR_WORKSPACE, "plan_add_mrf_stage: C = %d needs a workspace of %lld bytes (fv_mrf_stage_workspace_bytes)", C,
                    (long long)mrf_workspace_bytes(C));
    if (int rc = check_op_slots(x_slot, y_slot, y_act_slot)) return rc;
    Op o = {};
    o.type = OP_STAGE;
    o.x = x_slot;
    o.y = y_slot;
    o.y2 = y_act_slot;
    o.res = o.acc = o.acc2 = FV_SLOT_NONE;
    o.group = 0;
    o.Cin = o.Cout = C;
    o.k = k[0];
    o.dil = dil[0];
    for (int j = 0; j < 3; ++j) {
        o.pk[j] = k[j];
        o.sdil[j] = dil[j];
    }
    o.wp = packed;
    o.work = workspace;
    o.work_bytes = workspace_bytes;
    o.pre_slope = slope;
    o.act_slope = act_slope;
    o.out_div = out_div;
    o.post = post;
    o.prec = FV_PAIR_SPLIT_F16;
    plan->ops.push_back(o);
    return 0;
}

int fv_plan_add_resblock_pair(fv_plan_t* plan, int x_slot, int y_slot, int y_act_slot, const float* packed1,
                              const float* packed2, const float* bias1, const float* bias2, int C, int k, int dil,
                              float slope, float act_slope) {
    return fv_plan_add_resblock_pair_ex(plan, x_slot, y_slot, y_act_slot, FV_SLOT_NONE, FV_SLOT_NONE, FV_SLOT_NONE,
                                        packed1, packed2, bias1, bias2, C, k, dil, slope, 1.f, FV_POST_NONE, act_slope,
                                        FV_PAIR_F32);
}

int fv_plan_add_resblock_pair_ex(fv_plan_t* plan, int x_slot, int y_slot, int y_act_slot, int mid_slot, int add1_slot,
                                 int add2_slot, const float* packed1, const float* packed2, const float* bias1,
                                 const float* bias2, int C, int k, int dil, float slope, float out_div, int post,
                                 float act_slope, int prec) {
    if (!plan || !packed1 || !packed2) return fail(FV_ERR_INVALID_ARG, "plan_add_resblock_pair: null");
    if (int rc = check_pair_args(1, C, &k, dil, prec)) return rc;
    if ((C >= 64) != (mid_slot != FV_SLOT_NONE))
        return fail(FV_ERR_INVALID_ARG, "plan_add_resblock_pair: a scratch slot is needed at C >= 64 and only there");
    if (int rc = check_slot(mid_slot, true)) return rc;
    if (prec != FV_PAIR_F32 && prec != FV_PAIR_SPLIT_F16)
        return fail(FV_ERR_INVALID_ARG, "plan_add_resblock_pair: unknown arithmetic %d", prec);
    if (prec == FV_PAIR_F32 && (add1_slot != FV_SLOT_NONE || add2_slot != FV_SLOT_NONE || out_div != 1.f || post != FV_POST_NONE))
        return fail(FV_ERR_UNSUPPORTED, "plan_add_resblock_pair: add1 / add2 / out_div / post exist with FV_PAIR_SPLIT_F16 only");
    if (int rc = check_adds("plan_add_resblock_pair", add1_slot != FV_SLOT_NONE, add2_slot != FV_SLOT_NONE)) return rc;
    if (int rc = check_op_slots(x_slot, y_slot, y_act_slot, {add1_slot, add2_slot})) return rc;
    Op o = {};
    o.type = OP_PAIR;
    o.x = x_slot;
    o.y = y_slot;
    o.y2 = y_act_slot;
    o.res = FV_SLOT_NONE;
    o.acc = add1_slot;
    o.acc2 = add2_slot;
    o.tmpb = mid_slot;
    o.group = plan->cur_group;
    o.Cin = o.Cout = C;
    o.k = k;
    o.dil = dil;
    o.pre_slope = slope;
    o.act_slope = act_slope;
    o.out_div = out_div;
    o.post = post;
    o.prec = prec;
    o.pw1[0] = packed1;
    o.pw2[0] = packed2;
    o.pb1[0] = bias1;
    o.pb2[0] = bias2;
    o.pk[0] = k;
    plan->ops.push_back(o);
    return 0;
}

int fv_plan_add_conv1d_split_f16(fv_plan_t* plan, int x_slot, int y_slot, int y_act_slot, int res_slot, int add1_slot,
                                 int add2_slot, const float* packed, const float* bias, int C, int k, int dil,
                                 int pad_mode, float pre_slope, float out_div, int post, float act_slope) {
// ... 139 lines not shown
    if (int rc = infer(plan, B, T, sh, elems)) return rc < 0 ? rc : -rc;
    return arena(elems);
}

}

namespace fv {

struct Run {
    const fv_plan* plan;
    int B;
    float* const* base;
    const Shape* sh;
    const int* aux_b;
    hipStream_t s;
    const Op& op(size_t n) const { return plan->ops[n]; }
    float* at(int slot) const { return ptr(base, slot); }
    int64_t T(const Op& o) const { return sh[o.x].T; }
    int* guard() const { return plan->guard_dev; }
    const float* sub(const Op& o) const { return ptr(base, o.sub); }
    int sub_batched(const Op& o) const { return o.sub == FV_SLOT_NONE ? 0 : aux_b[o.sub - FV_SLOT_AUX_IN0]; }
};

static bool same_convh(const Op& a, const Op& b) {
    return b.type == OP_CONVH && b.group == a.group && b.Cin == a.Cin && b.dil == a.dil && b.pad_mode == a.pad_mode &&
           b.pre_slope == a.pre_slope && b.act_slope == a.act_slope && b.out_div == a.out_div && b.post == a.post;
}
static bool same_pair(const Op& a, const Op& b) {
    return b.type == OP_PAIR && b.group == a.group && b.Cin == a.Cin && b.dil == a.dil && b.pre_slope == a.pre_slope &&
           b.act_slope == a.act_slope && !a.fold_w && !b.fold_w && b.prec == a.prec && b.out_div == a.out_div && b.post == a.post;
}
static bool same_conv(const Op& a, const Op& b) { return b.type == OP_CONV && b.group == a.group; }

static size_t group_end(const fv_plan* plan, size_t n, bool (*same)(const Op&, const Op&)) {
    size_t m = n + 1;
    if (plan->ops[n].group != 0)
        while (m < plan->ops.size() && m - n < 3 && same(plan->ops[n], plan->ops[m])) ++m;
    return m;
}

static int run_convh_group(const Run& r, size_t n, size_t m) {
    const Op& o = r.op(n);
    PairParams pp = pair_params(o, (int)(m - n), r.B, r.T(o), r.guard());
    for (size_t q = n; q < m; ++q) {
        const Op& qo = r.op(q);
        pp.m[q - n] = pair_member(r.base[qo.x], qo.pw1[0], nullptr, qo.pb1[0], nullptr, qo.pk[0], r.base[qo.y], r.at(qo.y2),
                                  r.at(qo.res), r.at(qo.acc), r.at(qo.acc2));
    }
    return launch_convh(pp, o.Cin, o.dil, r.s);
}

static int run_stage(const Run& r, const Op& o) {
    float* const y = r.base[o.y];
    return launch_mrfh(mrf_params(o, r.base[o.x], o.fold_w ? nullptr : y, o.fold_w ? nullptr : r.at(o.y2), o.fold_w ? y : nullptr,
                                  r.B, r.T(o), r.guard()),
                       o.Cin, o.sdil, r.s);
}

static int run_pair_group(const Run& r, size_t n, size_t m) {
    const Op& o = r.op(n);
    const bool sum = o.type == OP_MRFSUM;
    PairParams pp = pair_params(o, sum ? 3 : (int)(m - n), r.B, r.T(o), r.guard());
    float* mids[3] = {nullptr, nullptr, nullptr};
    if (sum) {
        const int xs3[3] = {o.x, o.xb, o.xc};
        pp.sum = 1;
        for (int j = 0; j < 3; ++j)
            pp.m[j] = pair_member(r.base[xs3[j]], o.pw1[j], o.pw2[j], o.pb1[j], o.pb2[j], o.pk[j], r.base[o.y], r.at(o.y2));
    } else {
        for (size_t q = n; q < m; ++q) {
            const Op& qo = r.op(q);
            pp.m[q - n] = pair_member(r.base[qo.x], qo.pw1[0], qo.pw2[0], qo.pb1[0], qo.pb2[0], qo.pk[0],
                                      qo.fold_w ? nullptr : r.base[qo.y], r.at(qo.y2), nullptr, r.at(qo.acc), r.at(qo.acc2));
            mids[q - n] = r.at(qo.tmpb);
            if (qo.fold_w) {
                pp.fold_w = qo.fold_w;
                pp.fold_b = qo.fold_b;
                pp.fold_y = r.base[qo.y];
            }
        }
    }
    return launch_pair_family(pp, mids, o.Cin, o.dil, o.prec, r.s);
}

static int run_conv_group(const Run& r, size_t n, size_t m) {
    ConvParams gp[3];
    for (size_t q = n; q < m; ++q) {
        const Op& qo = r.op(q);
        gp[q - n] = make_params(qo, r.base[qo.x], r.base[qo.y], r.at(qo.y2), r.at(qo.res), r.at(qo.acc), r.at(qo.acc2), r.B,
                                r.T(qo), r.at(qo.x2));
    }
    return launch_conv_group(gp, (int)(m - n), r.s);
}

static int run_sum3(const Run& r, const Op& o) {
    float* const* base = r.base;
    Op mb = o, mc = o;
    mb.k = o.kb; mb.pad = (o.kb - 1) / 2; mb.wp = o.wpb; mb.bias = nullptr;
    mc.k = o.kc; mc.pad = (o.kc - 1) / 2; mc.wp = o.wpc; mc.bias = nullptr;
    float* y2s = r.at(o.y2);
    const int64_t T3 = r.T(o);
    const int Mp = pad_rows(o.Cout);
    const int64_t blocks = (int64_t)(Mp == 16 ? 1 : Mp / 32) * ((T3 + 127) / 128);
    const int min_blocks = tuning().sum3_min;
    if (blocks >= min_blocks && Mp == o.Cout) {
        ConvParams ps[3] = {
// ... 139 lines not shown
```

### fastvocoder_amd/generator/engine.py

```python
import warnings

import torch

from .. import _native
from .._native import (PAD_CAUSAL, PAD_REFLECT, PAD_ZERO, POST_NONE, POST_RELU, POST_TANH,
                       SLOT_AUX_IN0, SLOT_AUX_IN1, SLOT_IN, SLOT_NONE, SLOT_OUT, SLOT_OUT2)


def weight_norm(module):
    with warnings.catch_warnings():
        warnings.simplefilter("ignore")
        return torch.nn.utils.weight_norm(module)


def effective_weight(conv):
    if hasattr(conv, "weight_g") and hasattr(conv, "weight_v"):
        return _native.fold_weight_norm(conv.weight_v, conv.weight_g)
    return conv.weight.detach().contiguous().float()


def cached(module, key, build):
    hit = module._fv_plans.get(key)
    if hit is not None and hit[0] == module._fv_state():
        return hit[1]
# ... 163 lines not shown
    @staticmethod
    def pair_fusable(conv1, conv2, prec=None):
        k, c = conv1.kernel_size[0], conv1.in_channels
        prec = _native.PAIR_F32 if prec is None else prec
        return (all(cv.stride[0] == 1 and cv.groups == 1 and cv.in_channels == c and cv.out_channels == c
                    and cv.kernel_size[0] == k and cv.padding[0] == cv.dilation[0] * (k - 1) // 2
                    for cv in (conv1, conv2))
                and conv2.dilation[0] == 1 and _native.pair_supported(c, k, conv1.dilation[0], prec))

    def _pair_member(self, conv1, conv2, prec=_native.PAIR_F32):
        if not self.pair_fusable(conv1, conv2, prec):
            raise _native.NativeError("resblock pair: shape not built into the fused kernels")
        return dict(w1=_native.pack_pair(effective_weight(conv1), prec, self.guard),
                    w2=_native.pack_pair(effective_weight(conv2), prec, self.guard),
                    b1=self._bias(conv1), b2=self._bias(conv2), k=conv1.kernel_size[0])

    @staticmethod
    def pair_fold_supported(conv1, out_conv, prec, stage=False):
        c = conv1.in_channels
        return (prec == _native.PAIR_SPLIT_F16 and (c == 16 or (stage and c == 32))
                and isinstance(out_conv, torch.nn.Conv1d) and out_conv.in_channels == c and out_conv.out_channels == 1
                and out_conv.kernel_size[0] == 7 and out_conv.stride[0] == 1 and out_conv.dilation[0] == 1
                and out_conv.padding[0] == 3 and out_conv.groups == 1)

    def pair(self, conv1, conv2, src, dst, slope, prec=_native.PAIR_F32, add1=SLOT_NONE, add2=SLOT_NONE,
             out_div=1.0, post=POST_NONE, mid=SLOT_NONE, fold=None):
        m = self._pair_member(conv1, conv2, prec)
        if fold is not None:
            out_conv, fslope, fpost = fold
            if not self.pair_fold_supported(conv1, out_conv, prec) or post != POST_NONE or self.group:
                raise _native.NativeError("resblock pair: this output conv cannot be folded into the pair")
            m = dict(m, fold_w=effective_weight(out_conv).detach().float().reshape(16, 7).contiguous(),
                     fold_b=self._bias(out_conv), fold_post=fpost, act_slope=float(fslope))
        wide = conv1.in_channels >= 64
        if wide and mid == SLOT_NONE:
            raise _native.NativeError("resblock pair: a scratch slot (mid) is needed at 64 channels and above")
        self.ops.append(dict(kind="pair", group=self.group, x=src, y=dst, res=SLOT_NONE,
                             acc=add1, acc2=add2, pre_slope=1.0, slope=float(slope),
                             channels=conv1.in_channels, dil=conv1.dilation[0], prec=prec,
                             out_div=float(out_div), post=post, mid=mid if wide else SLOT_NONE,
                             tmps=[mid] if wide else [], **m))

    def mrf_stage_supported(self, blocks):
        if len(blocks) != 3 or self.pair_precision(blocks[0].channels) != _native.PAIR_SPLIT_F16:
            return False
        if any(len(b.convs1) != 3 or len(b.convs2) != 3 for b in blocks):
            return False
        ks = [b.convs1[0].kernel_size[0] for b in blocks]
        dils = [c.dilation[0] for c in blocks[0].convs1]
        return (_native.mrf_stage_supported(blocks[0].channels, ks, dils)
                and all([c.dilation[0] for c in b.convs1] == dils for b in blocks)
                and all(self.pair_fusable(c1, c2, _native.PAIR_SPLIT_F16) for b in blocks for c1, c2 in zip(b.convs1, b.convs2)))

    def mrf_stage(self, blocks, src, dst, slope, out_div, fold=None):
        if not self.mrf_stage_supported(blocks):
            raise _native.NativeError("mrf stage: shape not built into the one-launch kernel")
        ks = [b.convs1[0].kernel_size[0] for b in blocks]
        dils = [c.dilation[0] for c in blocks[0].convs1]
        c1s = [c for b in blocks for c in b.convs1]
        c2s = [c for b in blocks for c in b.convs2]
        packed = _native.pack_mrf_stage([effective_weight(c) for c in c1s], [effective_weight(c) for c in c2s],
                                        [self._bias(c) for c in c1s], [self._bias(c) for c in c2s], ks, self.guard)
        op = dict(kind="stage", group=0, x=src, y=dst, res=SLOT_NONE, acc=SLOT_NONE, acc2=SLOT_NONE, pre_slope=1.0,
                  slope=float(slope), channels=blocks[0].channels, ks=ks, dils=dils, packed=packed, out_div=float(out_div),
                  post=POST_NONE, prec=_native.PAIR_SPLIT_F16)
        if fold is not None:
            out_conv, fslope, fpost = fold
            if not self.pair_fold_supported(blocks[0].convs1[0], out_conv, _native.PAIR_SPLIT_F16, stage=True):
                raise _native.NativeError("mrf stage: this output conv cannot be folded into the stage")
            op.update(fold_w=effective_weight(out_conv).detach().float().reshape(blocks[0].channels, 7).contiguous(),
                      fold_b=self._bias(out_conv), fold_post=fpost, act_slope=float(fslope))
        self.ops.append(op)

    def conv_split_supported(self, conv, pad, pad_mode=PAD_ZERO):
        c, k, d = conv.in_channels, conv.kernel_size[0], conv.dilation[0]
        return (conv.stride[0] == 1 and conv.groups == 1 and conv.out_channels == c and pad == d * (k - 1) // 2
                and pad_mode in (PAD_ZERO, PAD_REFLECT) and c in (64, 128, 256, 512)
                and self.pair_precision(c) == _native.PAIR_SPLIT_F16
                and _native.conv_split_supported(c, k, d))

    def conv_split(self, conv, src, dst, slope, res=SLOT_NONE, add1=SLOT_NONE, add2=SLOT_NONE, out_div=1.0,
                   post=POST_NONE, pad=None, pad_mode=PAD_ZERO):
        c, k, d = conv.in_channels, conv.kernel_size[0], conv.dilation[0]
        pad = conv.padding[0] if pad is None else pad + conv.padding[0]
        if not (conv.stride[0] == 1 and conv.groups == 1 and conv.out_channels == c and pad == d * (k - 1) // 2
                and pad_mode in (PAD_ZERO, PAD_REFLECT) and (pad_mode == PAD_ZERO or conv.padding[0] == 0)
                and c in (64, 128, 256, 512) and _native.conv_split_supported(c, k, d)):
            raise _native.NativeError("conv_split: shape not built into the split-f16 conv kernels")
        self.ops.append(dict(kind="convh", group=self.group, x=src, y=dst, res=res, acc=add1, acc2=add2,
                             pre_slope=1.0, slope=float(slope), channels=c, k=k, dil=d, pad_mode=pad_mode,
                             packed=_native.pack_pair(effective_weight(conv), _native.PAIR_SPLIT_F16, self.guard),
                             bias=self._bias(conv), out_div=float(out_div), post=post))

    def residual_stack_supported(self, dilated, pointwise, skip, pad, pad_mode=PAD_ZERO):
        c, k, d = dilated.in_channels, dilated.kernel_size[0], dilated.dilation[0]
        return (self.precision != "f32" and dilated.stride[0] == 1 and dilated.groups == 1 and dilated.out_channels == c
                and dilated.padding[0] == 0 and pad == d * (k - 1) // 2 and pad_mode in (PAD_ZERO, PAD_REFLECT)
                and all(cv.kernel_size[0] == 1 and cv.stride[0] == 1 and cv.groups == 1 and cv.padding[0] == 0
                        and cv.in_channels == c and cv.out_channels == c for cv in (pointwise, skip))
                and _native.residual_stack_split_supported(c, k, d))

    def residual_stack(self, dilated, pointwise, skip, src, dst, slope, pad_mode=PAD_ZERO, hidden=SLOT_NONE, post=POST_NONE):
        c, k, d = dilated.in_channels, dilated.kernel_size[0], dilated.dilation[0]
        if not self.residual_stack_supported(dilated, pointwise, skip, d * (k - 1) // 2, pad_mode):
            raise _native.NativeError("residual_stack: shape not built into the one-launch kernel")
        ba, bb = self._bias(pointwise), self._bias(skip)
        bias_out = ba if bb is None else (bb if ba is None else (ba + bb).contiguous())
        w1, w2, ws = effective_weight(dilated), effective_weight(pointwise), effective_weight(skip)
        op = dict(kind="stack", x=src, y=dst, res=SLOT_NONE, acc=SLOT_NONE, pre_slope=1.0, slope=float(slope),
                  split=True, channels=c, k=k, dil=d, pad_mode=pad_mode,
                  packed=_native.pack_residual_stack_split(w1, w2, ws, self.guard),
                  bias=self._bias(dilated), bias_out=bias_out, post=post)
        if c >= 256:
            if hidden == SLOT_NONE:
                raise _native.NativeError("residual_stack: a scratch slot (hidden) is needed at 256 channels")
            op.update(tmps=[hidden], two_launch=(hidden, _native.pack_pair(w1, _native.PAIR_SPLIT_F16, self.guard),
                                                 _native.pack_conv1x1_2src_split(w2, ws, self.guard)))
        self.ops.append(op)

    def mrf_sum(self, pairs, srcs, dst, slope, out_div, post=POST_NONE):
        ms = [self._pair_member(c1, c2) for c1, c2 in pairs]
        c1 = pairs[0][0]
        if any(p[0].dilation[0] != c1.dilation[0] or p[0].in_channels != c1.in_channels for p in pairs):
            raise _native.NativeError("mrf_sum: the three pairs must share channels and dilation")
        self.ops.append(dict(kind="mrfsum", x=srcs[0], xb=srcs[1], xc=srcs[2], y=dst,
                             res=SLOT_NONE, acc=SLOT_NONE, pre_slope=1.0, slope=float(slope),
                             channels=c1.in_channels, dil=c1.dilation[0], members=ms, out_div=float(out_div),
                             post=post))

    def conv_transpose_takes_merge(self, convt):
        if not isinstance(convt, torch.nn.ConvTranspose1d) or convt.groups != 1 or convt.dilation[0] != 1:
            return False
        k, s = convt.kernel_size[0], convt.stride[0]
        return ((self.SPLIT_CONVT_MIN_CIN <= convt.in_channels <= 128
                 or _native.conv_transpose_small(convt.in_channels, convt.out_channels, k, s))
                and self.pair_precision(convt.in_channels) == _native.PAIR_SPLIT_F16
                and _native.conv_transpose_split_supported(convt.in_channels, convt.out_channels, k, s, convt.padding[0],
                                                           convt.output_padding[0]))

    SPLIT_CONVT_MIN_CIN = 64

    def conv_transpose(self, convt, src, dst, pre_slope=1.0, post=POST_NONE, trim=0, merge=None):
        if convt.groups != 1 or convt.dilation[0] != 1:
            raise _native.NativeError("only dense, undilated ConvTranspose1d layers exist on this path")
        k, s = convt.kernel_size[0], convt.stride[0]
        p, op = convt.padding[0], convt.output_padding[0]
        cin, cout = convt.in_channels, convt.out_channels
        if merge is not None and not (post == POST_NONE and trim == 0 and self.conv_transpose_takes_merge(convt)):
            raise _native.NativeError("conv_transpose: a merged input exists on the split-f16 kernel only")
        if (post == POST_NONE and (cin >= self.SPLIT_CONVT_MIN_CIN or _native.conv_transpose_small(cin, cout, k, s))
                and self.pair_precision(cin) == _native.PAIR_SPLIT_F16
                and _native.conv_transpose_split_supported(cin, cout, k, s, p, op - int(trim))):
            extra = {} if merge is None else dict(xb=merge[0], xc=merge[1], in_div=float(merge[2]))
            self.ops.append(dict(kind="convT", split=True, x=src, y=dst, res=SLOT_NONE, acc=SLOT_NONE,
                                 pre_slope=1.0, slope=float(pre_slope),
                                 packed=_native.pack_conv_transpose1d_split(effective_weight(convt), s, self.guard),
                                 bias=self._bias(convt), cin=cin, cout=cout, k=k, stride=s, pad=p,
                                 out_pad=op - int(trim), post=post, **extra))
            return
        self.ops.append(dict(kind="convT", x=src, y=dst, res=SLOT_NONE, acc=SLOT_NONE,
                             pre_slope=float(pre_slope),
                             packed=_native.pack_conv_transpose1d(effective_weight(convt), s, p),
                             bias=self._bias(convt), cin=cin, cout=cout,
                             k=k, stride=s, pad=p, out_pad=op - int(trim), post=post))

    def upsample_conv(self, layer, src, dst, pre_slope=1.0, post=POST_NONE):
        conv = layer.conv
        if conv.stride[0] != 1 or conv.dilation[0] != 1 or conv.groups != 1:
            raise _native.NativeError("UpsampleLayer: only a stride-1, undilated, dense conv is supported")
        k, p, u = conv.kernel_size[0], conv.padding[0], layer.upsample_rate
        self.ops.append(dict(kind="upconv", x=src, y=dst, res=SLOT_NONE, acc=SLOT_NONE,
                             pre_slope=float(pre_slope),
                             packed=_native.pack_upsample_conv1d(effective_weight(conv), u, p),
                             bias=self._bias(conv), cin=conv.in_channels, cout=conv.out_channels,
                             k=k, rate=u, pad=p, post=post))

    def basis_overlap_add(self, basis_weight, src, dst, hop, pre_slope=1.0):
        L, C = basis_weight.shape
        w = basis_weight.detach().float().t().contiguous().view(C, 1, L)
        self.ops.append(dict(kind="convT", x=src, y=dst, res=SLOT_NONE, acc=SLOT_NONE,
                             pre_slope=float(pre_slope), packed=_native.pack_conv_transpose1d(w, hop, 0),
                             bias=None, cin=C, cout=1, k=L, stride=hop, pad=0, out_pad=0, post=POST_NONE))

    def subtract_output(self, aux=0, second=True):
        op = self.ops[-1]
        if (op["kind"] not in ("conv", "conv2", "conv2h", "stack", "convT", "upconv", "pqmf", "postpqmf") or op.get("group", 0)
                or (op.get("split") and op["kind"] not in ("conv2h", "stack"))):
            raise _native.NativeError("subtract_output: the last op must be a plain conv / transposed conv / two-source "
                                      "1x1 conv / residual stack / pqmf")
# ... 16 lines not shown
                             cin=conv.in_channels, k=conv.kernel_size[0], pad=conv.padding[0], post=post, h=h))

    def pqmf_synthesis(self, synthesis_filter, src, dst):
        S = synthesis_filter.shape[1]
        h = synthesis_filter.detach().reshape(S, -1).contiguous().float()
        self.ops.append(dict(kind="pqmf", x=src, y=dst, res=SLOT_NONE, acc=SLOT_NONE, pre_slope=1.0, h=h))

    def _hoist_activations(self):
        ops = self.ops
        twin_of = {}
        for i, op in enumerate(ops):
            op.setdefault("y_act", SLOT_NONE)
            op.setdefault("act_slope", 1.0)
        for i, op in enumerate(ops):
            if op["kind"] in ("pqmf", "postpqmf"):
                continue
            y = op["y"]
            act_uses, raw_needed = {}, y == SLOT_OUT
            for j in range(i + 1, len(ops)):
                c = ops[j]
                for key in ("x", "xb", "xc"):
                    if c.get(key, SLOT_NONE) == y:
                        if c["pre_slope"] != 1.0:
                            act_uses.setdefault(c["pre_slope"], []).append((j, key))
                        else:
                            raw_needed = True
                if y in (c["res"], c["acc"], c.get("acc2", SLOT_NONE), c.get("x2", SLOT_NONE),
                         c.get("resb", SLOT_NONE), c.get("resc", SLOT_NONE)):
                    raw_needed = True
                if c["y"] == y or c.get("y_act") == y or y in c.get("tmps", ()):
                    break
            if not act_uses:
                continue
            slope = max(act_uses, key=lambda s: len(act_uses[s]))
            if len(act_uses) > 1:
                raw_needed = True
            if raw_needed:
                if y not in twin_of:
                    twin_of[y] = self.tmp()
                op["y_act"], op["act_slope"], target = twin_of[y], slope, twin_of[y]
            else:
                op["act_slope"], target = slope, y
            for j, key in act_uses[slope]:
                ops[j][key] = target
                ops[j].setdefault("_hoisted", set()).add(key)
        for op in ops:
            keys = [k for k in ("x", "xb", "xc") if op.get(k, SLOT_NONE) != SLOT_NONE]
            if op.get("_hoisted") and set(keys) <= op["_hoisted"]:
                op["pre_slope"] = 1.0

    def receptive_halo(self):
        need = {}
        for op in reversed(self.ops):
            h_out = max(need.pop(op["y"], 0), need.pop(op.get("y_act", SLOT_NONE), 0))
            if op["kind"] == "conv":
                reach = op["dil"] * (op["k"] - 1)
                own, rate = max(op["pad"], reach - op["pad"]), 1
            elif op["kind"] == "sum3":
                own, rate = max(op["ks"]) // 2, 1
            elif op["kind"] in ("conv2", "conv2h"):
                own, rate = 0, 1
            elif op["kind"] in ("convh", "stack"):
                own, rate = (op["k"] - 1) // 2 * op["dil"], 1
            elif op["kind"] == "pair":
                own, rate = (op["k"] - 1) // 2 * (op["dil"] + 1) + (3 if "fold_w" in op else 0), 1
            elif op["kind"] == "mrfsum":
                own, rate = max((m["k"] - 1) // 2 * (op["dil"] + 1) for m in op["members"]), 1
            elif op["kind"] == "stage":
                own = max(sum((k - 1) // 2 * (d + 1) for d in op["dils"]) for k in op["ks"]) + (3 if "fold_w" in op else 0)
                rate = 1
            elif op["kind"] == "convT":
                own, rate = -(-op["k"] // op["stride"]) + 1, op["stride"]
            elif op["kind"] == "upconv":
                own, rate = -(-(op["k"] + op["rate"]) // op["rate"]) + 1, op["rate"]
            elif op["kind"] == "postpqmf":
                S, ntaps = op["h"].shape
                own, rate = -(-(ntaps // 2) // S) + 1 + op["k"] // 2, S
            else:
                S, ntaps = op["h"].shape
                own, rate = -(-(ntaps // 2) // S) + 1, S
            need[op["x"]] = max(need.get(op["x"], 0), -(-h_out // rate) + own)
            for key in ("xb", "xc"):
                if op.get(key, SLOT_NONE) != SLOT_NONE:
                    need[op[key]] = max(need.get(op[key], 0), -(-h_out // rate) + own)
            for aux in (op["res"], op["acc"], op.get("acc2", SLOT_NONE), op.get("x2", SLOT_NONE),
                        op.get("resb", SLOT_NONE), op.get("resc", SLOT_NONE)):
                if aux != SLOT_NONE:
                    need[aux] = max(need.get(aux, 0), h_out)
        return need.get(SLOT_IN, 0)

    def finalize(self):
        self._hoist_activations()
        self.plan.halo_frames = self.receptive_halo()
        for op in self.ops:
            self.plan.set_group(op.get("group", 0))
            self.plan.set_sum_order(op.get("own_first", False))
            if op["kind"] == "conv":
                self.plan.add_conv1d(op["x"], op["y"], op["packed"], op["bias"], op["cin"], op["cout"],
                                     op["k"], dil=op["dil"], pad=op["pad"], pad_mode=op["pad_mode"],
                                     pre_slope=op["pre_slope"], res=op["res"], acc=op["acc"],
                                     out_div=op["out_div"], post=op["post"], y_act=op["y_act"],
                                     act_slope=op["act_slope"], acc2=op.get("acc2", SLOT_NONE))
            elif op["kind"] == "sum3":
                if op["pre_slope"] != 1.0:
                    raise _native.NativeError("conv_sum3: the activation of its inputs could not be hoisted")
                self.plan.add_conv1d_sum3([op["x"], op["xb"], op["xc"]], [op["res"], op["resb"], op["resc"]],
                                          op["tmps"], op["y"], op["packed"], op["bias"], op["channels"], op["ks"],
                                          out_div=op["out_div"], post=op["post"], y_act=op["y_act"],
                                          act_slope=op["act_slope"])
            elif op["kind"] == "pair":
                self.plan.add_resblock_pair(op["x"], op["y"], op["w1"], op["w2"], op["b1"], op["b2"],
                                            op["channels"], op["k"], op["dil"], op["slope"],
                                            y_act=op["y_act"], act_slope=op["act_slope"], prec=op["prec"],
                                            add1=op["acc"], add2=op["acc2"], out_div=op["out_div"],
                                            post=op["post"], mid=op["mid"])
                if "fold_w" in op:
                    self.plan.set_pair_output_conv(op["fold_w"], op["fold_b"], op["y"], op["act_slope"], op["fold_post"])
            elif op["kind"] == "stage":
                self.plan.add_mrf_stage(op["x"], op["y"], op["packed"], op["channels"], op["ks"], op["dils"], op["slope"],
                                        out_div=op["out_div"], y_act=op["y_act"], act_slope=op["act_slope"])
                if "fold_w" in op:
                    self.plan.set_pair_output_conv(op["fold_w"], op["fold_b"], op["y"], op["act_slope"], op["fold_post"])
            elif op["kind"] == "convh":
                self.plan.add_conv1d_split_f16(op["x"], op["y"], op["packed"], op["bias"], op["channels"], op["k"],
                                               op["dil"], pre_slope=op["slope"], res=op["res"], add1=op["acc"],
                                               add2=op["acc2"], out_div=op["out_div"], post=op["post"],
                                               y_act=op["y_act"], act_slope=op["act_slope"], pad_mode=op["pad_mode"])
            elif op["kind"] == "mrfsum":
                ms = op["members"]
                self.plan.add_mrf_sum([op["x"], op["xb"], op["xc"]], op["y"], [m["w1"] for m in ms],
                                      [m["w2"] for m in ms], [m["b1"] for m in ms], [m["b2"] for m in ms],
                                      op["channels"], [m["k"] for m in ms], op["dil"], op["slope"],
                                      out_div=op["out_div"], post=op["post"], y_act=op["y_act"],
                                      act_slope=op["act_slope"])
            elif op["kind"] == "conv2":
                if op["pre_slope"] != 1.0:
                    raise _native.NativeError("conv_sum_1x1: the activation of the first input could not "
                                              "be hoisted into its producer")
                self.plan.add_conv1d_2src(op["x"], op["x2"], op["y"], op["packed"], op["bias"], op["cin1"],
                                          op["cin2"], op["cout"], res=op["res"], post=op["post"],
                                          y_act=op["y_act"], act_slope=op["act_slope"])
            elif op["kind"] == "conv2h":
                self.plan.add_conv1x1_2src_split_f16(op["x"], op["x2"], op["y"], op["packed"], op["bias"], op["channels"],
                                                     pre_slope=op["slope"], res=op["res"], post=op["post"],
                                                     y_act=op["y_act"], act_slope=op["act_slope"])
            elif op["kind"] == "stack":
                self.plan.add_residual_stack_split_f16(op["x"], op["y"], op["packed"], op["bias"], op["bias_out"],
                                                       op["channels"], op["k"], op["dil"], op["slope"],
                                                       pad_mode=op["pad_mode"], y_act=op["y_act"], act_slope=op["act_slope"],
                                                       two_launch=op.get("two_launch"), post=op["post"])
            elif op["kind"] == "convT" and op.get("split"):
                self.plan.add_conv_transpose1d_split_f16(op["x"], op["y"], op["packed"], op["bias"], op["cin"],
                                                         op["cout"], op["k"], op["stride"], op["pad"], op["out_pad"],
                                                         pre_slope=op["slope"], y_act=op["y_act"],
                                                         act_slope=op["act_slope"],
                                                         merge=(op["xb"], op["xc"], op["in_div"]) if "in_div" in op else None)
            elif op["kind"] == "convT":
                self.plan.add_conv_transpose1d(op["x"], op["y"], op["packed"], op["bias"], op["cin"],
                                               op["cout"], op["k"], op["stride"], op["pad"],
                                               op["out_pad"], pre_slope=op["pre_slope"], post=op["post"],
                                               y_act=op["y_act"], act_slope=op["act_slope"])
            elif op["kind"] == "upconv":
                self.plan.add_upsample_conv1d(op["x"], op["y"], op["packed"], op["bias"], op["cin"],
                                              op["cout"], op["k"], op["rate"], op["pad"],
                                              pre_slope=op["pre_slope"], post=op["post"],
                                              y_act=op["y_act"], act_slope=op["act_slope"])
            elif op["kind"] == "postpqmf":
                self.plan.add_conv_post_pqmf(op["x"], op["y"], op["packed"], op["bias"], op["cin"], op["k"], op["pad"],
                                             op["h"], pre_slope=op["pre_slope"], post=op["post"])
            else:
                self.plan.add_pqmf_synthesis(op["x"], op["y"], op["h"])
            if "sub" in op:
                self.plan.set_output_offset(op["sub"], op["sub_y2"], op["y"])
        self.plan.guarded = any(op["kind"] == "convh" or op.get("split") or op.get("prec") == _native.PAIR_SPLIT_F16
                                for op in self.ops)
        if self.plan.guarded and self.guard is not None:
            self.plan.set_guard(self.guard)
        return self.plan


_registration_epoch = [0]


def _bump_epoch(*_args):
    _registration_epoch[0] += 1


torch.nn.modules.module.register_module_parameter_registration_hook(_bump_epoch)
torch.nn.modules.module.register_module_buffer_registration_hook(_bump_epoch)


class NativeModule(torch.nn.Module):

    precision = "split"
    range_guard = "auto"
    low_range_patience = 3
    fuse_pairs = True
    fuse_stage = True
    fold_post = True
    merge_in_upsampler = True

    def __init__(self):
        super().__init__()
        self._fv_plans = {}
        self._fv_fast = {}
        self._fv_tensors = None
        self._fv_ids = ()
        self._fv_epoch = -1
        self._fv_key = None
        self._fv_guard = None
        self._fv_overflow = False
        self._fv_low_hits = 0
        self._fv_force_f32 = False

    def _fv_policy(self):
        prec = "f32" if (self.precision == "f32" or self._fv_overflow or getattr(self, "_fv_force_f32", False)) else "split"
        return (prec, bool(self.fuse_pairs), bool(self.fold_post), self.range_guard != "off", bool(self.merge_in_upsampler),
                self.fuse_stage if isinstance(self.fuse_stage, tuple) else bool(self.fuse_stage))

    def _fv_state(self):
        if self._fv_tensors is None or self._fv_epoch != _registration_epoch[0]:
            self._fv_tensors = list(self.parameters()) + list(self.buffers())
            self._fv_ids = tuple(id(t) for t in self._fv_tensors)
            self._fv_epoch = _registration_epoch[0]
        return (self._fv_ids, tuple([t._version for t in self._fv_tensors])), self._fv_policy()

    def __getstate__(self):
        state = self.__dict__.copy()
        state["_fv_plans"] = {}
        state["_fv_fast"] = {}
        state["_fv_tensors"] = None
        state["_fv_epoch"] = -1
        state["_fv_guard"] = None
        state.pop("_fv_zero", None)
        state.pop("_zero_cache", None)
        return state

    def invalidate_plans(self):
        self._fv_plans = {}
        self._fv_fast = {}
        self._fv_tensors = None
        self._fv_overflow = False
        self._fv_low_hits = 0
        self.__dict__.pop("_fv_zero", None)
        self.__dict__.pop("_zero_cache", None)

    def _apply(self, fn, *args, **kwargs):
        out = super()._apply(fn, *args, **kwargs)
        for m in self.modules():
            if isinstance(m, NativeModule):
                m.invalidate_plans()
        return out

    def load_state_dict(self, *args, **kwargs):
        out = super().load_state_dict(*args, **kwargs)
        for m in self.modules():
            if isinstance(m, NativeModule):
                m.invalidate_plans()
        return out

    def train(self, mode=True):
        changed = any(m.training != mode for m in self.modules())
        out = super().train(mode)
        if changed:
            for m in self.modules():
                if isinstance(m, NativeModule):
                    m.invalidate_plans()
        return out

    def _device(self):
        dev = next(self.parameters()).device
# ... 164 lines not shown
```

### fastvocoder_amd/generator/hifigan.py

```python
import torch

from .._native import PAIR_SPLIT_F16
from .engine import (GradPrecision, NativeModule, PlanBuilder, POST_TANH, SLOT_IN, SLOT_NONE, SLOT_OUT, pair_precision,
                     weight_norm)
from . import grad
from .modules import LRELU_SLOPE, ResBlock1, ResBlock2, UpsampleLayer
from .pqmf import PQMF

DEFAULT_LRELU_SLOPE = 0.01


_CU_COUNT = {}


def stage32_windows_fit(cols, cus, fill=0.65):
    cols = int(cols)
    if cols <= 0:
        return False
    nblk = max(1, min(int(cus), -(-cols // 128)))
    share = -(-cols // nblk)
    windows = 1 if share <= 264 else 1 + -(-(share - 264) // 324)
    return share >= fill * 384 * windows


class _HiFiGANBase(GradPrecision, NativeModule):
    _post_channels = 1
    fuse_pqmf = True
    _parameter_grad = False

    @property
    def parameter_grad(self):
        return self._parameter_grad

    @parameter_grad.setter
    def parameter_grad(self, value):
        if value:
            grad.check_supported(self)
        self._parameter_grad = bool(value)

    def __init__(self, resblock_kernel_sizes, upsample_rates, upsample_initial_channel,
                 resblock_type, upsample_kernel_sizes, resblock_dilation_sizes, transposedconv,
                 bias):
        super().__init__()
        self.num_kernels = len(resblock_kernel_sizes)
        self.num_upsamples = len(upsample_rates)
        c0 = upsample_initial_channel
        self.conv_pre = torch.nn.Conv1d(80, c0, 7, 1, padding=3, bias=bias)
        block = ResBlock1 if resblock_type == "1" else ResBlock2

        self.ups = torch.nn.ModuleList()
        for i, (u, k) in enumerate(zip(upsample_rates, upsample_kernel_sizes)):
            cin, cout = c0 // (2 ** i), c0 // (2 ** (i + 1))
            if transposedconv:
                up = torch.nn.ConvTranspose1d(cin, cout, k, u, padding=(u // 2 + u % 2),
                                              output_padding=u % 2, bias=bias)
            else:
                up = UpsampleLayer(cin, cout, upsample_rate=u, kernel_size=k, stride=1,
                                   padding=k // 2, bias=bias)
            self.ups.append(up)

        self.resblocks = torch.nn.ModuleList()
        ch = c0
        for i in range(len(self.ups)):
            ch = c0 // (2 ** (i + 1))
            for k, d in zip(resblock_kernel_sizes, resblock_dilation_sizes):
                self.resblocks.append(block(ch, k, d, bias=bias))
        self.conv_post = torch.nn.Conv1d(ch, self._post_channels, 7, 1, padding=3, bias=bias)

    def _finish_init(self):
        self.apply_weight_norm()
        self.reset_parameters()

    def _stage_fusable(self, i, precision):
        nk = self.num_kernels
        blocks = [self.resblocks[i * nk + j] for j in range(nk)]
        if nk != 3 or not all(isinstance(b, ResBlock1) for b in blocks):
            return False
        if sorted(b.convs1[0].kernel_size[0] for b in blocks) != [3, 7, 11]:
            return False
        dils = [[c.dilation[0] for c in b.convs1] for b in blocks]
        if any(d != dils[0] for d in dils):
            return False
        prec = pair_precision(precision, blocks[0].channels)
        return all(PlanBuilder.pair_fusable(c1, c2, prec) for b in blocks for c1, c2 in zip(b.convs1, b.convs2))

    def _fused_flags(self, T):
        precision, fuse = self._fv_policy()[:2]
        if not fuse:
            return (False,) * self.num_upsamples
        flags, t = [], int(T)
        for i in range(self.num_upsamples):
            up = self.ups[i]
            if isinstance(up, UpsampleLayer):
                t = t * up.upsample_rate + 2 * up.conv.padding[0] - (up.conv.kernel_size[0] - 1)
            else:
                t = (t - 1) * up.stride[0] - 2 * up.padding[0] + up.kernel_size[0] + up.output_padding[0]
            fusable = t > 0 and t % 4 == 0 and self._stage_fusable(i, precision)
            ch = self.resblocks[i * self.num_kernels].channels
            flags.append("s" if fusable and self._stage_one_launch(ch, t) else bool(fusable))
        return tuple(flags)

    def _stage_one_launch(self, channels, t):
        fs = self.fuse_stage
        if isinstance(fs, (tuple, list)):
            return channels in fs
        if not fs or channels == 16:
            return bool(fs)
        if channels != 32:
            return False
        dev = self._device()
        cus = _CU_COUNT.get(dev)
        if cus is None:
            cus = _CU_COUNT[dev] = torch.cuda.get_device_properties(dev).multi_processor_count
        return stage32_windows_fit(getattr(self, "_fv_batch", 1) * int(t), cus)

    def _emit_fused_stage(self, pb, blocks, up, x, scratch, parts, fold=None, merge_next=False, one_launch=False):
        nk = len(blocks)
        npairs = len(blocks[0].convs1)
        ch = blocks[0].channels
        curs = [up] * nk
        prec = pb.pair_precision(ch)
        if one_launch and pb.mrf_stage_supported(blocks):
            if fold is not None:
                pb.mrf_stage(blocks, up, fold[3], LRELU_SLOPE, float(nk), fold=fold[:3])
            else:
                pb.mrf_stage(blocks, up, x, LRELU_SLOPE, float(nk))
            return
        if prec == PAIR_SPLIT_F16 and ch > 128:
            for pi in range(npairs):
                last = pi == npairs - 1
                pb.begin_group()
                for j in range(nk):
                    pb.conv_split(blocks[j].convs1[pi], curs[j], scratch[j][0], LRELU_SLOPE)
                pb.end_group()
                nxt = []
                pb.begin_group()
                for j in range(1 if (last and not merge_next) else 0, nk):
                    ping, pong = scratch[j][1], scratch[j][2]
                    d = (x if j == 0 else parts[j - 1]) if last else (ping if curs[j] != ping else pong)
                    pb.conv_split(blocks[j].convs2[pi], scratch[j][0], d, LRELU_SLOPE, res=curs[j])
                    nxt.append(d)
                pb.end_group()
                if last and not merge_next:
                    pb.conv_split(blocks[0].convs2[pi], scratch[0][0], x, LRELU_SLOPE, res=curs[0],
                                  add1=parts[0], add2=parts[1] if nk > 2 else SLOT_NONE, out_div=float(nk))
                curs = nxt
            return
        for pi in range(npairs - 1):
            pb.begin_group()
            nxt = []
            for j in range(nk):
                ping, pong = scratch[j][1], scratch[j][2]
                d = ping if curs[j] != ping else pong
                pb.pair(blocks[j].convs1[pi], blocks[j].convs2[pi], curs[j], d, LRELU_SLOPE, prec, mid=scratch[j][0])
                nxt.append(d)
            pb.end_group()
            curs = nxt
        if prec == PAIR_SPLIT_F16 and merge_next:
            pb.begin_group()
            for j in range(nk):
                pb.pair(blocks[j].convs1[-1], blocks[j].convs2[-1], curs[j], x if j == 0 else parts[j - 1], LRELU_SLOPE, prec,
                        mid=scratch[j][0])
            pb.end_group()
            return
        if prec == PAIR_SPLIT_F16:
            pb.begin_group()
            for j in range(1, nk):
                pb.pair(blocks[j].convs1[-1], blocks[j].convs2[-1], curs[j], parts[j - 1], LRELU_SLOPE, prec,
                        mid=scratch[j][0])
            pb.end_group()
            if fold is not None:
                pb.pair(blocks[0].convs1[-1], blocks[0].convs2[-1], curs[0], fold[3], LRELU_SLOPE, prec,
                        add1=parts[0], add2=parts[1], out_div=float(nk), mid=scratch[0][0], fold=fold[:3])
                return
            pb.pair(blocks[0].convs1[-1], blocks[0].convs2[-1], curs[0], x, LRELU_SLOPE, prec,
                    add1=parts[0], add2=parts[1], out_div=float(nk), mid=scratch[0][0])
            return
        if ch == 16:
            pb.mrf_sum([(b.convs1[-1], b.convs2[-1]) for b in blocks], curs, x, LRELU_SLOPE, float(nk))
            return
        states = [dict(cur=c) for c in curs]
        steps = blocks[0].num_steps()
        pb.begin_group()
        for j in range(nk):
            blocks[j].emit_step(pb, steps - 2, states[j], up, x, scratch[j])
        pb.end_group()
        convs, srcs, ress = zip(*[blocks[j].last_conv_inputs(states[j], up, scratch[j]) for j in range(nk)])
        pb.conv_sum3(convs, srcs, ress, parts[:2], x, pre_slope=LRELU_SLOPE, out_div=float(nk))

    def _fold_post(self, pb, fused):
        if not pb.fold_post or not fused or not fused[-1] or self.num_kernels != 3:
            return False
        blocks = self.resblocks[-3:]
        return PlanBuilder.pair_fold_supported(blocks[0].convs1[-1], self.conv_post, pb.pair_precision(blocks[0].channels),
                                               stage=fused[-1] == "s" and pb.mrf_stage_supported(blocks))

    def _emit_trunk(self, pb, dst, fused=None, fold_post=False, pqmf=None):
        fold_post = fold_post and self._fold_post(pb, fused)
        x, up = pb.tmp(), pb.tmp()
        nk = self.num_kernels
        parts = [pb.tmp() for _ in range(nk - 1)]
        scratch = [[pb.tmp(), pb.tmp(), pb.tmp()] for _ in range(nk)]
        pb.conv(self.conv_pre, SLOT_IN, x)
        merged = False
        for i in range(self.num_upsamples):
            if isinstance(self.ups[i], UpsampleLayer):
                pb.upsample_conv(self.ups[i], x, up, pre_slope=LRELU_SLOPE)
            else:
                pb.conv_transpose(self.ups[i], x, up, pre_slope=LRELU_SLOPE,
                                  merge=(parts[0], parts[1], float(nk)) if merged else None)
            merged = False
            blocks = [self.resblocks[i * nk + j] for j in range(nk)]
            if fused is not None and fused[i]:
                if fold_post and i == self.num_upsamples - 1:
                    self._emit_fused_stage(pb, blocks, up, x, scratch, parts, one_launch=fused[i] == "s",
                                           fold=(self.conv_post, DEFAULT_LRELU_SLOPE, POST_TANH, dst))
                    return
                merged = (self.merge_in_upsampler and nk == 3 and i + 1 < self.num_upsamples
                          and pb.pair_precision(blocks[0].channels) == PAIR_SPLIT_F16
                          and pb.conv_transpose_takes_merge(self.ups[i + 1])
                          and not (fused[i] == "s" and pb.mrf_stage_supported(blocks)))
                self._emit_fused_stage(pb, blocks, up, x, scratch, parts, merge_next=merged, one_launch=fused[i] == "s")
                continue
            if nk <= 3:
                steps = blocks[0].num_steps()
                states = [dict() for _ in range(nk)]
                sum3 = (nk == 3 and all(isinstance(b, ResBlock1) for b in blocks)
                        and sorted(b.convs2[-1].kernel_size[0] for b in blocks) == [3, 7, 11])
                if sum3:
                    for st in range(steps - 1):
                        pb.begin_group()
                        for j in range(nk):
                            blocks[j].emit_step(pb, st, states[j], up, x, scratch[j])
                        pb.end_group()
                    convs, srcs, ress = zip(*[blocks[j].last_conv_inputs(states[j], up, scratch[j])
                                              for j in range(nk)])
                    pb.conv_sum3(convs, srcs, ress, parts[:2], x, pre_slope=LRELU_SLOPE, out_div=float(nk))
                    continue
                others = list(range(1, nk))
                for st in range(steps):
                    final = st == steps - 1
                    members = others if final else range(nk)
                    pb.begin_group()
                    for j in members:
                        blocks[j].emit_step(pb, st, states[j], up, parts[others.index(j)] if final else x,
                                            scratch[j])
                    pb.end_group()
                blocks[0].emit_step(pb, steps - 1, states[0], up, x, scratch[0],
                                    acc=parts[0] if nk > 1 else SLOT_NONE,
                                    acc2=parts[1] if nk > 2 else SLOT_NONE, out_div=float(nk), own_first=True)
            else:
                for j in range(nk):
                    last = j == nk - 1
                    blocks[j].emit(pb, up, x if last else parts[0], scratch[0],
                                   acc=parts[0] if j > 0 else SLOT_NONE,
                                   out_div=float(nk) if last else 1.0)
        if pqmf is not None and pb.post_pqmf_supported(self.conv_post, pqmf) and self.fuse_pqmf:
            pb.conv_post_pqmf(self.conv_post, pqmf, x, dst, pre_slope=DEFAULT_LRELU_SLOPE, post=POST_TANH)
        elif pqmf is not None:
            sub = pb.tmp()
            pb.conv(self.conv_post, x, sub, pre_slope=DEFAULT_LRELU_SLOPE, post=POST_TANH)
            pb.pqmf_synthesis(pqmf, sub, dst)
        else:
            pb.conv(self.conv_post, x, dst, pre_slope=DEFAULT_LRELU_SLOPE, post=POST_TANH)

    def _flag_tag(self, T):
        return "".join("s" if f == "s" else "f" if f else "-" for f in self._fused_flags(T))

    def _trunk_plan(self, T):
        return self._plan(lambda: "trunk" + self._flag_tag(T),
                          lambda pb: self._emit_trunk(pb, SLOT_OUT, self._fused_flags(T), fold_post=True), 80)

    def _emit_inference(self, pb, fused):
        self._emit_trunk(pb, SLOT_OUT, fused)

    def _minus_plan(self, T):
        def emit(pb):
            self._emit_inference(pb, self._fused_flags(T))
            pb.subtract_output(0, second=True)
        return self._plan(lambda: "minus" + self._flag_tag(T), emit, 80)

    def inference_minus(self, x, bias):
        x = self._prepare(x).transpose(1, 0).unsqueeze(0).contiguous()
        est, rem = self._run_minus(self._minus_plan, x, bias)
        return est.squeeze(), rem.squeeze()

    def _trunk(self, x, sync=False):
        return self._run_plan(self._trunk_plan, x, sync=sync)


class HiFiGANGenerator(_HiFiGANBase):

    def __init__(self, resblock_kernel_sizes=[3, 7, 11], upsample_rates=[8, 5, 3, 2],
                 upsample_initial_channel=256, resblock_type="1",
                 upsample_kernel_sizes=[16, 10, 6, 4],
                 resblock_dilation_sizes=[[1, 3, 5], [1, 3, 5], [1, 3, 5]],
                 transposedconv=True, bias=True):
        super().__init__(resblock_kernel_sizes, upsample_rates, upsample_initial_channel,
                         resblock_type, upsample_kernel_sizes, resblock_dilation_sizes,
                         transposedconv, bias)
        self._finish_init()

    def forward(self, x):
        if grad.wants_param_grad(self):
            return grad.run(self, x)[:, 0, :]
        return self._trunk(self._prepare(x))[:, 0, :]

    def inference(self, x):
        x = self._prepare(x)
        return self._trunk(x.transpose(1, 0).unsqueeze(0).contiguous(), sync=True).squeeze()


class MultiBandHiFiGANGenerator(_HiFiGANBase):

    _post_channels = 4

    def __init__(self, resblock_kernel_sizes=[3, 7, 11], upsample_rates=[10, 6],
                 upsample_initial_channel=256, resblock_type="1",
                 upsample_kernel_sizes=[20, 12],
                 resblock_dilation_sizes=[[1, 3, 5], [1, 3, 5], [1, 3, 5]],
                 transposedconv=True, bias=True):
        super().__init__(resblock_kernel_sizes, upsample_rates, upsample_initial_channel,
                         resblock_type, upsample_kernel_sizes, resblock_dilation_sizes,
                         transposedconv, bias)
        self.pqmf = PQMF()
        self._finish_init()

    def forward(self, x):
        if grad.wants_param_grad(self):
            return grad.run(self, x)
        return self._trunk(self._prepare(x))

    def _emit_full(self, pb, fused=None):
        self._emit_trunk(pb, SLOT_OUT, fused, pqmf=self.pqmf.synthesis_filter)

    def _emit_inference(self, pb, fused):
        self._emit_full(pb, fused)

    def _full_plan(self, T):
        return self._plan(lambda: "inference" + self._flag_tag(T),
                          lambda pb: self._emit_full(pb, self._fused_flags(T)), 80)

    def inference(self, x):
        x = self._prepare(x).transpose(1, 0).unsqueeze(0).contiguous()
        return self._run_plan(self._full_plan, x, sync=True).squeeze()

    def synthesize_batch(self, x):
        return self._run_plan(self._full_plan, self._prepare(x))[:, 0, :]
```

### include/fastvocoder_hip.h

```cpp
#ifndef FASTVOCODER_HIP_H
#define FASTVOCODER_HIP_H

#include <stddef.h>
#include <stdint.h>

#ifdef __cplusplus
extern "C" {
#endif

#define FV_ABI_VERSION 18

#define FV_ERR_INVALID_ARG (-1)
#define FV_ERR_UNSUPPORTED (-2)
#define FV_ERR_WORKSPACE (-3)
#define FV_ERR_RANGE (-4)
#define FV_ERR_RANGE_LOW (-5)
#define FV_GUARD_HIGH 0x001
#define FV_GUARD_LOW 0x100

#define FV_PAD_ZERO 0
#define FV_PAD_REFLECT 1
#define FV_PAD_CAUSAL 2

#define FV_POST_NONE 0
// ... 1 lines not shown
#define FV_POST_RELU 2

int fv_version(void);
const char* fv_build_id(void);
const char* fv_last_error(void);


int fv_fold_weight_norm(const float* v, const float* g, float* w, int dim0,
                        int64_t inner, void* stream);

int fv_fold_batchnorm_conv(const float* w, const float* b, const float* gamma, const float* beta,
                           const float* mean, const float* var, float eps, float* w_out,
                           float* b_out, int Cout, int Cin, int k, void* stream);

int64_t fv_packed_conv1d_floats(int Cout, int Cin, int k);
int64_t fv_packed_conv_transpose1d_floats(int Cin, int Cout, int k, int stride, int pad);

int fv_pack_conv1d_weight(const float* w, float* packed, int Cout, int Cin, int k,
                          void* stream);
int fv_pack_conv_transpose1d_weight(const float* w, float* packed, int Cin, int Cout,
                                    int k, int stride, int pad, void* stream);


int fv_conv1d_fused(const float* x, const float* packed, const float* bias,
                    const float* res, const float* acc_in, const float* acc_in2, float* y,
                    float* y_act, int B, int Cin, int Cout, int Tin, int k, int dil, int pad,
                    int pad_mode, float pre_slope, float out_div, int post, float act_slope,
                    void* stream);

int64_t fv_packed_pair_floats(int C, int k);
int fv_pack_pair_weight(const float* w, float* packed, int C, int k, void* stream);
int fv_resblock1_fused(int n, const float* const* x, const float* const* w1, const float* const* w2,
                       const float* const* b1, const float* const* b2, float* const* y, float* const* y_act,
                       const int* k, int B, int C, int T, int dil, float slope, float act_slope, void* stream);

#define FV_PAIR_F32 0
#define FV_PAIR_SPLIT_F16 1
int64_t fv_packed_pair_floats_ex(int C, int k, int prec);
int fv_pack_pair_weight_ex(const float* w, float* packed, int C, int k, int prec, int* range_flag, void* stream);
int fv_resblock1_fused_ex(int n, const float* const* x, const float* const* w1, const float* const* w2,
                          const float* const* b1, const float* const* b2, float* const* y, float* const* y_act,
                          float* const* mid, const float* const* add1, const float* const* add2, const int* k, int B,
                          int C, int T, int dil, float slope, float out_div, int post, float act_slope, int prec,
                          int* guard, void* stream);

int64_t fv_packed_mrf_stage_floats(int C, const int* k);
int fv_pack_mrf_stage_split_f16(const float* const* w1, const float* const* w2, const float* const* b1,
                                const float* const* b2, float* packed, int C, const int* k, int* range_flag, void* stream);
int64_t fv_mrf_stage_workspace_bytes(int C);
int fv_mrf_stage_split_f16(const float* x, const float* packed, float* y, float* y_act, int B, int C, int T, const int* k,
                           const int* dil, float slope, float out_div, int post, float act_slope, const float* fold_w,
                           const float* fold_b, float* fold_y, void* workspace, int64_t workspace_bytes, int* guard,
                           void* stream);

int fv_conv1d_split_f16(int n, const float* const* x, const float* const* packed, const float* const* bias,
                        const float* const* res, const float* const* add1, const float* const* add2, float* const* y,
                        float* const* y_act, const int* k, int B, int C, int T, int dil, int pad_mode, float pre_slope,
                        float out_div, int post, float act_slope, int* guard, void* stream);

int64_t fv_packed_conv_transpose1d_split_floats(int Cin, int Cout, int k, int stride);
int fv_pack_conv_transpose1d_split_f16(const float* w, float* packed, int Cin, int Cout, int k, int stride, int* range_flag,
                                       void* stream);
int fv_conv_transpose1d_split_f16(const float* x, const float* packed, const float* bias, float* y, float* y_act, int B,
                                  int Cin, int Cout, int Tin, int k, int stride, int pad, int out_pad, float pre_slope,
                                  float act_slope, int* guard, void* stream);

int fv_mrf_stage(const float* const* x, const float* const* w1, const float* const* w2, const float* const* b1,
                 const float* const* b2, float* y, float* y_act, const int* k, int B, int C, int T, int dil,
                 float slope, float out_div, int post, float act_slope, void* stream);

int fv_conv1d_2src_fused(const float* x, const float* x2, const float* packed, const float* bias,
                         const float* res, float* y, float* y_act, int B, int Cin1, int Cin2,
                         int Cout, int T, int post, float act_slope, void* stream);

int64_t fv_packed_conv1x1_2src_split_floats(int C);
int fv_pack_conv1x1_2src_split_f16(const float* w1, const float* w2, float* packed, int C, int* range_flag, void* stream);
int fv_conv1x1_2src_split_f16(const float* x, const float* x2, const float* packed, const float* bias, const float* res,
                              float* y, float* y_act, int B, int C, int T, float pre_slope, int post, float act_slope,
                              int* guard, void* stream);

int64_t fv_packed_residual_stack_floats(int C, int k);
int fv_pack_residual_stack_split_f16(const float* w_dilated, const float* w_pointwise, const float* w_skip, float* packed,
                                     int C, int k, int* range_flag, void* stream);
int fv_residual_stack_split_f16(const float* x, const float* packed, const float* bias_dilated, const float* bias_out, float* y,
                                float* y_act, int B, int C, int T, int k, int dil, float slope, int pad_mode, int post,
                                float act_slope, int* guard, void* stream);

int fv_conv_transpose1d_fused(const float* x, const float* packed, const float* bias,
                              float* y, float* y_act, int B, int Cin, int Cout, int Tin,
                              int k, int stride, int pad, int out_pad, float pre_slope,
                              int post, float act_slope, void* stream);

int64_t fv_packed_basis_floats(int L, int C);
int fv_pack_basis(const float* W, float* packed, int L, int C, void* stream);
int fv_basis_ola(const float* weight, const float* packed_basis, float* out, int B, int C, int F, int L, void* stream);

int64_t fv_packed_upsample_conv1d_floats(int Cout, int Cin, int k, int rate, int pad);
int fv_pack_upsample_conv1d_weight(const float* w, float* packed, int Cout, int Cin, int k,
                                   int rate, int pad, void* stream);
int fv_upsample_conv1d_fused(const float* x, const float* packed, const float* bias, float* y,
                             float* y_act, int B, int Cin, int Cout, int Tin, int k, int rate,
                             int pad, float pre_slope, int post, float act_slope, void* stream);

int fv_pqmf_synthesis(const float* x, const float* h, float* y, int B, int S, int ntaps,
                      int Tsub, void* stream);

// ... 197 lines not shown

int fv_grad_bucket_pack(const fv_adam_tensor* tensors, const fv_adam_chunk* chunks, int n_tensors, int64_t n_chunks,
                        const float* const* src, float scale, void* stream);


typedef struct fv_plan fv_plan_t;

#define FV_SLOT_NONE (-1)
#define FV_SLOT_IN 0
#define FV_SLOT_OUT 1
#define FV_SLOT_TMP0 2
#define FV_MAX_SLOTS 32
#define FV_SLOT_AUX_IN0 28
#define FV_SLOT_AUX_IN1 29
#define FV_SLOT_OUT2 30

fv_plan_t* fv_plan_create(int in_channels);
void fv_plan_destroy(fv_plan_t* plan);

int fv_plan_add_conv1d(fv_plan_t* plan, int x_slot, int y_slot, int y_act_slot,
                       int res_slot, int acc_slot, int acc2_slot, const float* packed,
                       const float* bias, int Cin, int Cout, int k, int dil, int pad,
                       int pad_mode, float pre_slope, float out_div, int post,
                       float act_slope);
int fv_plan_add_conv_transpose1d(fv_plan_t* plan, int x_slot, int y_slot, int y_act_slot,
                                 const float* packed, const float* bias, int Cin, int Cout,
                                 int k, int stride, int pad, int out_pad, float pre_slope,
                                 int post, float act_slope);
int fv_plan_add_conv1d_2src(fv_plan_t* plan, int x_slot, int x2_slot, int y_slot, int y_act_slot,
                            int res_slot, const float* packed, const float* bias, int Cin1,
                            int Cin2, int Cout, int post, float act_slope);
int fv_plan_add_conv1x1_2src_split_f16(fv_plan_t* plan, int x_slot, int x2_slot, int y_slot, int y_act_slot, int res_slot,
                                       const float* packed, const float* bias, int C, float pre_slope, int post,
                                       float act_slope);
int fv_plan_add_residual_stack_split_f16(fv_plan_t* plan, int x_slot, int y_slot, int y_act_slot, const float* packed,
                                         const float* bias_dilated, const float* bias_out, int C, int k, int dil, float slope,
                                         int pad_mode, int post, float act_slope);
int fv_plan_set_stack_two_launch(fv_plan_t* plan, int hidden_slot, const float* packed_dilated, const float* packed_pair);
int fv_plan_add_conv1d_sum3(fv_plan_t* plan, const int* x_slots, const int* res_slots,
                            const int* tmp_slots, int y_slot, int y_act_slot,
                            const float* const* packed, const float* bias_sum, int C, const int* k,
                            float out_div, int post, float act_slope);
int fv_plan_add_resblock_pair(fv_plan_t* plan, int x_slot, int y_slot, int y_act_slot, const float* packed1,
                              const float* packed2, const float* bias1, const float* bias2, int C, int k, int dil,
                              float slope, float act_slope);
int fv_plan_add_resblock_pair_ex(fv_plan_t* plan, int x_slot, int y_slot, int y_act_slot, int mid_slot, int add1_slot,
                                 int add2_slot, const float* packed1, const float* packed2, const float* bias1,
                                 const float* bias2, int C, int k, int dil, float slope, float out_div, int post,
                                 float act_slope, int prec);
int fv_plan_set_pair_output_conv(fv_plan_t* plan, const float* w, const float* bias, int y_slot, float act_slope, int post);
int fv_plan_add_mrf_stage_split_f16(fv_plan_t* plan, int x_slot, int y_slot, int y_act_slot, const float* packed, int C,
                                    const int* k, const int* dil, float slope, float out_div, int post, float act_slope,
                                    void* workspace, int64_t workspace_bytes);
int fv_plan_add_conv1d_split_f16(fv_plan_t* plan, int x_slot, int y_slot, int y_act_slot, int res_slot, int add1_slot,
                                 int add2_slot, const float* packed, const float* bias, int C, int k, int dil,
                                 int pad_mode, float pre_slope, float out_div, int post, float act_slope);
int fv_plan_add_conv_transpose1d_split_f16(fv_plan_t* plan, int x_slot, int y_slot, int y_act_slot, const float* packed,
                                           const float* bias, int Cin, int Cout, int k, int stride, int pad,
                                           int out_pad, float pre_slope, float act_slope);
int fv_plan_set_input_merge(fv_plan_t* plan, int add1_slot, int add2_slot, float div);
int fv_plan_add_mrf_sum(fv_plan_t* plan, const int* x_slots, int y_slot, int y_act_slot,
                        const float* const* packed1, const float* const* packed2, const float* const* bias1,
                        const float* const* bias2, int C, const int* k, int dil, float slope, float out_div,
                        int post, float act_slope);
int fv_plan_add_upsample_conv1d(fv_plan_t* plan, int x_slot, int y_slot, int y_act_slot,
                                const float* packed, const float* bias, int Cin, int Cout,
                                int k, int rate, int pad, float pre_slope, int post,
                                float act_slope);
int fv_plan_add_pqmf_synthesis(fv_plan_t* plan, int x_slot, int y_slot, const float* h,
                               int S, int ntaps);
int fv_plan_add_conv_post_pqmf(fv_plan_t* plan, int x_slot, int y_slot, const float* packed, const float* bias, int Cin,
                               int S, int k, int pad, float pre_slope, int post, const float* h, int ntaps);

int fv_plan_set_output_offset(fv_plan_t* plan, int aux_slot, int y2_slot);

int fv_plan_set_sum_order(fv_plan_t* plan, int own_first);

int fv_plan_set_group(fv_plan_t* plan, int group);

int fv_plan_output_shape(fv_plan_t* plan, int T, int* out_channels, int64_t* out_len);
int fv_plan_slot_shape(fv_plan_t* plan, int T, int slot, int* channels, int64_t* len);
int64_t fv_plan_workspace_bytes(fv_plan_t* plan, int B, int T);

int fv_plan_run(fv_plan_t* plan, int B, int T, const float* in, float* out,
                void* workspace, int64_t workspace_bytes, void* stream);

int fv_plan_run_aux(fv_plan_t* plan, int B, int T, const float* in, float* out, float* out2,
                    const float* const* aux_in, const int* aux_batched, void* workspace,
                    int64_t workspace_bytes, void* stream);

int fv_generator_run(fv_plan_t* plan, int B, int T, const float* mel, float* out, void* workspace,
                     int64_t workspace_bytes, void* stream);

int fv_div_probe(unsigned first_bits, int64_t n, float d, unsigned long long* mismatches, void* stream);

int fv_plan_num_ops(fv_plan_t* plan);

int fv_plan_set_guard(fv_plan_t* plan, int* word);
int fv_plan_check_range(fv_plan_t* plan, void* stream);

int fv_tuning_set(const char* key, int value);
int fv_debug_pair_schedule(int n_members, const int* n_items, const int* cost, int nblk, int mode, int three_members,
                           unsigned* table);

#define FV_KERNEL_CONV_MFMA32 0
#define FV_KERNEL_CONV_MFMA16 1
#define FV_KERNEL_CONV_NARROW 2
#define FV_KERNEL_PAIR16 3
#define FV_KERNEL_PAIR32 4
#define FV_KERNEL_PAIRH16 5
#define FV_KERNEL_PAIRH32 6
#define FV_KERNEL_CONVH64 7
#define FV_KERNEL_CONVH128 8
#define FV_KERNEL_CONVT 9
#define FV_KERNEL_CONVG 10
#define FV_KERNEL_STACK 11
#define FV_KERNEL_MRF16 12
#define FV_KERNEL_MRF32 13
int fv_profile_enable(int on);
int fv_profile_bracket_cost(void* stream, int n, double* ms_per_bracket);
int fv_profile_mfma_f16_rate(float* scratch, long long scratch_floats, int launches, int iters, void* stream, double* tflops);
int fv_profile_collect(int kind, int64_t* launches, double* ms, double* flops, double* bytes);

#ifdef __cplusplus
}
#endif
#endif
```

Measured before the change: 394.2 million samples/s.

## Split 32-channel MRF stage into two block classes with cost-model scheduling

Adds a two-class variant of the fused 32-channel MRF stage kernel. One set of blocks computes the short-reach branches and another the long-reach branch, each with its own halo and window partition. A host-side cost model with a cache picks the block split that minimises makespan and compares it against the single-class form. The second partial sum is merged into the next transposed convolution, which now accepts a single add operand. This is meant to cut halo recompute and balance load across CUs, at the cost of a second output buffer and new scheduling logic.

```diff
diff --git a/fastvocoder_amd/_native.py b/fastvocoder_amd/_native.py
--- a/fastvocoder_amd/_native.py
+++ b/fastvocoder_amd/_native.py
@@ -336,6 +336,10 @@
     L.fv_plan_check_range.argtypes = [vp, vp]
     L.fv_tuning_set.argtypes = [ctypes.c_char_p, i]
     L.fv_debug_pair_schedule.argtypes = [i, ctypes.POINTER(i), ctypes.POINTER(i), i, i, i, ctypes.POINTER(ctypes.c_uint)]
+    L.fv_debug_mrf_class_schedule.argtypes = [i, i, i, i, ctypes.POINTER(ctypes.c_int64), ctypes.POINTER(ctypes.c_uint)]
+    L.fv_debug_mrf_stage_class_f16.argtypes = [vp, vp, vp, i, i, i, i, ctypes.POINTER(i), ctypes.POINTER(i), f, vp, i64, vp]
+    L.fv_mrf_stage_classes_f16.argtypes = [vp, vp, vp, vp, i, i, i, ctypes.POINTER(i), ctypes.POINTER(i), f, vp, i64, vp, vp]
+    L.fv_plan_add_mrf_stage_classes_f16.argtypes = [vp, i, i, i, vp, i, ctypes.POINTER(i), ctypes.POINTER(i), f, vp, i64]
     L.fv_plan_set_group.argtypes = [vp, i]
     L.fv_plan_output_shape.argtypes = [vp, i, ctypes.POINTER(i), ctypes.POINTER(i64)]
     L.fv_plan_workspace_bytes.argtypes = [vp, i, i]
@@ -431,6 +435,17 @@
     if rc == 2:
         return 2, [int(table[i]) for i in range(nblk)]
     return 0, None
+
+
+def mrf_class_schedule(batch, t, nblk, force=False):
+    info = (ctypes.c_int64 * 12)()
+    table = (ctypes.c_uint * 512)()
+    check(lib().fv_debug_mrf_class_schedule(int(batch), int(t), int(nblk), 1 if force else 0, info, table))
+    keys = ("split", "n_a", "n_b", "makespan", "makespan_one", "reach_a", "reach_b", "window", "cost_a", "cost_b", "cost_one")
+    out = {k: int(info[i]) for i, k in enumerate(keys)}
+    out["split"] = bool(out["split"])
+    out["ranges"] = [(int(table[2 * i]), int(table[2 * i + 1])) for i in range(out["n_a"] + out["n_b"])]
+    return out
 
 
 def _flag_ptr(flag):
@@ -707,6 +722,30 @@
                                            B, C, T, karr, darr, float(slope), float(out_div), post, float(act_slope), None,
                                            None, None, *_work_args(work), _guard_ptr(guard), stream))
     return out
+
+
+def mrf_stage_classes_f16(x, packed, ks, dils=MRF_STAGE_DILATIONS, slope=0.1, guard=None, work=None):
+    B, C, T = x.shape
+    karr, darr = (ctypes.c_int * 3)(*ks), (ctypes.c_int * 3)(*dils)
+    if work is None:
+        work = mrf_stage_workspace(C, x.device)
+    y_s, y_r2 = torch.empty_like(x), torch.empty_like(x)
+    with _on(x, packed, y_s, y_r2, work) as stream:
+        check(lib().fv_mrf_stage_classes_f16(_ptr(x, "x"), _ptr(packed, "packed"), _ptr(y_s, "y_s"), _ptr(y_r2, "y_r2"), B, C, T,
+                                             karr, darr, float(slope), *_work_args(work), _guard_ptr(guard), stream))
+    return y_s, y_r2
+
+
+def mrf_stage_one_class_f16(x, packed, ks, cls, dils=MRF_STAGE_DILATIONS, slope=0.1, work=None):
+    B, C, T = x.shape
+    karr, darr = (ctypes.c_int * 3)(*ks), (ctypes.c_int * 3)(*dils)
+    if work is None:
+        work = mrf_stage_workspace(C, x.device)
+    y = torch.empty_like(x)
+    with _on(x, packed, y, work) as stream:
+        check(lib().fv_debug_mrf_stage_class_f16(_ptr(x, "x"), _ptr(packed, "packed"), _ptr(y, "y"), {"a": 1, "b": 2}[cls], B, C, T,
+                                                 karr, darr, float(slope), *_work_args(work), stream))
+    return y
 
 
 def mrf_stage(xs, w1s, w2s, b1s, b2s, ks, dil, slope, out_div=3.0, post=POST_NONE, act_slope=1.0, out=None,
@@ -1862,6 +1901,15 @@
         check(lib().fv_plan_add_mrf_stage_split_f16(self._h, x, y, y_act, _ptr(packed, "packed"), channels,
                                                     (ctypes.c_int * 3)(*ks), (ctypes.c_int * 3)(*dils), float(slope),
                                                     float(out_div), post, float(act_slope), *_work_args(work)))
+
+    def add_mrf_stage_classes(self, x, y_s, y_r2, packed, channels, ks, dils, slope):
+        self.keep(packed)
+        work = mrf_stage_workspace(channels, packed.device)
+        if work is not None:
+            self.keep(work)
+        check(lib().fv_plan_add_mrf_stage_classes_f16(self._h, x, y_s, y_r2, _ptr(packed, "packed"), channels,
+                                                      (ctypes.c_int * 3)(*ks), (ctypes.c_int * 3)(*dils), float(slope),
+                                                      *_work_args(work)))
 
     def set_pair_output_conv(self, w, bias, y, act_slope, post=POST_NONE):
         self.keep(w)
diff --git a/fastvocoder_amd/csrc/api.hip b/fastvocoder_amd/csrc/api.hip
--- a/fastvocoder_amd/csrc/api.hip
+++ b/fastvocoder_amd/csrc/api.hip
@@ -258,6 +258,13 @@
     return mp;
 }
 
+MrfSplitParams mrf_split_params(const Op& o, const float* x, float* y_s, float* y_r2, int B, int64_t T, int* guard) {
+    MrfSplitParams sp = {};
+    static_cast<MrfParams&>(sp) = mrf_params(o, x, y_s, nullptr, nullptr, B, T, guard);
+    sp.y2 = y_r2;
+    return sp;
+}
+
 int check_pad_mode(int pad_mode, int pad, int k, int dil) {
     if (pad_mode < 0 || pad_mode > (FV_PAD_REFLECT | FV_PAD_CAUSAL))
         return fail(FV_ERR_INVALID_ARG, "unknown pad_mode %d", pad_mode);
@@ -332,6 +339,7 @@
     {"shape64", &Tuning::shape64},         {"krows", &Tuning::krows},            {"grid_cap", &Tuning::grid_cap},
     {"no_group", &Tuning::no_group},       {"mrf_blocks", &Tuning::mrf_blocks},  {"mrf_shape", &Tuning::mrf_shape},
     {"mrf_prio", &Tuning::mrf_prio},       {"convt_lean", &Tuning::convt_lean},
+    {"mrf_cost_a", &Tuning::mrf_cost_a},   {"mrf_cost_b", &Tuning::mrf_cost_b},  {"mrf_cost_one", &Tuning::mrf_cost_one},
     {"convs_ringfree", &Tuning::convs_ringfree}, {"convu_resident", &Tuning::convu_resident},
 };
 static void tuning_from_env() {
@@ -1156,6 +1164,46 @@
     return launch_mrfh(mrf_params(o, x, y, y_act, fold_y, B, T, guard), C, dil, (hipStream_t)stream);
 }
 
+int fv_mrf_stage_classes_f16(const float* x, const float* packed, float* y_s, float* y_r2, int B, int C, int T, const int* k,
+                             const int* dil, float slope, void* workspace, int64_t workspace_bytes, int* guard, void* stream) {
+    if (int rc = check_stage_args(C, k, dil, slope, 1.f, FV_POST_NONE)) return rc;
+    if (C != 32) return fail(FV_ERR_UNSUPPORTED, "mrf stage (two classes): C = %d (32)", C);
+    if (B < 0 || T < 0) return fail(FV_ERR_INVALID_ARG, "mrf stage (two classes): B=%d T=%d", B, T);
+    Op o = pair_op(OP_STAGE, C, dil[0], FV_PAD_ZERO, slope, 1.f, FV_POST_NONE, 1.f, FV_PAIR_SPLIT_F16);
+    o.wp = packed;
+    for (int j = 0; j < 3; ++j) o.pk[j] = k[j];
+    o.work = workspace;
+    o.work_bytes = workspace_bytes;
+    return launch_mrfw_split(mrf_split_params(o, x, y_s, y_r2, B, T, guard), dil, (hipStream_t)stream);
+}
+
+int fv_debug_mrf_stage_class_f16(const float* x, const float* packed, float* y, int cls, int B, int C, int T, const int* k,
+                                 const int* dil, float slope, void* workspace, int64_t workspace_bytes, void* stream) {
+    if (cls != 1 && cls != 2) return fail(FV_ERR_INVALID_ARG, "debug_mrf_stage_class: class %d (1: A, 2: B)", cls);
+    if (int rc = check_stage_args(C, k, dil, slope, 1.f, FV_POST_NONE)) return rc;
+    if (C != 32) return fail(FV_ERR_UNSUPPORTED, "debug_mrf_stage_class: C = %d (32)", C);
+    if (B < 0 || T < 0) return fail(FV_ERR_INVALID_ARG, "debug_mrf_stage_class: B=%d T=%d", B, T);
+    Op o = pair_op(OP_STAGE, C, dil[0], FV_PAD_ZERO, slope, 1.f, FV_POST_NONE, 1.f, FV_PAIR_SPLIT_F16);
+    o.wp = packed;
+    for (int j = 0; j < 3; ++j) o.pk[j] = k[j];
+    o.work = workspace;
+    o.work_bytes = workspace_bytes;
+    return launch_mrfw_split(mrf_split_params(o, x, y, nullptr, B, T, nullptr), dil, (hipStream_t)stream, cls);
+}
+
+int fv_debug_mrf_class_schedule(int B, int T, int nblk, int force, int64_t* info, unsigned* table) {
+    if (!info || !table) return fail(FV_ERR_INVALID_ARG, "debug_mrf_class_schedule: null argument");
+    fv::MrfClassPlan pl;
+    if (!fv::mrf_class_plan(B, T, nblk, force != 0, pl))
+        return fail(FV_ERR_INVALID_ARG, "debug_mrf_class_schedule: B=%d T=%d on %d blocks (1 .. %d blocks, B x T < 2^31)", B, T, nblk, fv::kSchedBlocks);
+    const fv::Tuning& tn = fv::tuning();
+    const int64_t v[12] = {pl.split, pl.n_a, pl.n_b, pl.makespan, pl.makespan_one, pl.reach_a, pl.reach_b, 384,
+                           tn.mrf_cost_a, tn.mrf_cost_b, tn.mrf_cost_one, 0};
+    memcpy(info, v, sizeof(v));
+    memcpy(table, pl.range, sizeof(pl.range));
+    return 0;
+}
+
 }
 
 namespace fv {
diff --git a/fastvocoder_amd/csrc/api_internal.h b/fastvocoder_amd/csrc/api_internal.h
--- a/fastvocoder_amd/csrc/api_internal.h
+++ b/fastvocoder_amd/csrc/api_internal.h
@@ -38,6 +38,7 @@
     int pk[3] = {0, 0, 0};
     int sdil[3] = {0, 0, 0};
     void* work = nullptr;
+    bool classes = false;
     int64_t work_bytes = 0;
     int prec = 0;
     bool in_merge = false;
@@ -83,6 +84,7 @@
                        float* y_act, const float* res = nullptr, const float* add1 = nullptr, const float* add2 = nullptr,
                        const float* x2 = nullptr);
 MrfParams mrf_params(const Op& o, const float* x, float* y, float* y_act, float* fold_y, int B, int64_t T, int* guard);
+MrfSplitParams mrf_split_params(const Op& o, const float* x, float* y_s, float* y_r2, int B, int64_t T, int* guard);
 int launch_pair_family(const PairParams& pp, float* const* mid, int C, int dil, int prec, hipStream_t s);
 int check_pair_args(int n, int C, const int* k, int dil, int prec = FV_PAIR_F32);
 int check_stage_args(int C, const int* k, const int* dil, float slope, float act_slope, int post);
diff --git a/fastvocoder_amd/csrc/convtn_kernels.hpp b/fastvocoder_amd/csrc/convtn_kernels.hpp
--- a/fastvocoder_amd/csrc/convtn_kernels.hpp
+++ b/fastvocoder_amd/csrc/convtn_kernels.hpp
@@ -35,7 +35,7 @@
     const __amdgpu_buffer_rsrc_t r2 = make_rsrc(p.add2 ? p.add2 + xoff : p.x, p.add2 ? xbytes : 0u);
     constexpr int TASKS = kTnRows * (kTnCin / 8), NR = (TASKS + 255) / 256;
     float v[NR][8], a1[NR][8], a2[NR][8];
-    const bool merge = p.add1 != nullptr;
+    const bool merge = p.add1 != nullptr, merge3 = p.add2 != nullptr;
 #pragma unroll
     for (int q = 0; q < NR; ++q) {
         const int idx = tid + q * 256;
@@ -47,8 +47,10 @@
         if (merge) {
 #pragma unroll
             for (int j = 0; j < 8; ++j) a1[q][j] = buffer_load1s(r1, voff, (unsigned)j * t4);
+            if (merge3) {
 #pragma unroll
-            for (int j = 0; j < 8; ++j) a2[q][j] = buffer_load1s(r2, voff, (unsigned)j * t4);
+                for (int j = 0; j < 8; ++j) a2[q][j] = buffer_load1s(r2, voff, (unsigned)j * t4);
+            }
         }
     }
     pair_wait_vm0();
@@ -64,7 +66,8 @@
             for (int j = 0; j < 4; ++j) {
                 f32x2 raw = {v[q][2 * j], v[q][2 * j + 1]};
                 if (merge) {
-                    raw = (raw + f32x2{a1[q][2 * j], a1[q][2 * j + 1]}) + f32x2{a2[q][2 * j], a2[q][2 * j + 1]};
+                    raw = raw + f32x2{a1[q][2 * j], a1[q][2 * j + 1]};
+                    if (merge3) raw = raw + f32x2{a2[q][2 * j], a2[q][2 * j + 1]};
                     if (p.out_div != 1.f) {
                         raw.x = rcp != 0.f ? div_exact(raw.x, p.out_div, rcp) : raw.x / p.out_div;
                         raw.y = rcp != 0.f ? div_exact(raw.y, p.out_div, rcp) : raw.y / p.out_div;
diff --git a/fastvocoder_amd/csrc/fv_internal.h b/fastvocoder_amd/csrc/fv_internal.h
--- a/fastvocoder_amd/csrc/fv_internal.h
+++ b/fastvocoder_amd/csrc/fv_internal.h
@@ -130,6 +130,9 @@
     int pair_blocks = 0;
     int mrf_blocks = 0;
     int mrf_shape = 0;
+    int mrf_cost_a = 585;
+    int mrf_cost_b = 661;
+    int mrf_cost_one = 1490;
     int mrf_prio = 1;
     int sum3_min = 800;
     int lds_budget = 39;
@@ -317,6 +320,24 @@
 constexpr int kMrfwHistBytes = 9 * 30 * 128;
 long long mrf_workspace_bytes(int C);
 int launch_mrfw_geom(const MrfParams& p, hipStream_t s);
+
+struct MrfSplitParams : MrfParams {
+    float* y2;
+    int n_a;
+    int halo_b;
+    unsigned range[2 * kSchedBlocks];
+};
+struct MrfClassPlan {
+    int split;
+    int n_a, n_b;
+    long long makespan;
+    long long makespan_one;
+    int reach_a, reach_b;
+    unsigned range[2 * kSchedBlocks];
+};
+bool mrf_class_plan(int B, int T, int nblk, bool force, MrfClassPlan& out);
+int launch_mrfw_split(MrfSplitParams p, const int* dil, hipStream_t stream, int one_class = 0);
+int launch_mrfw_split_geom(const MrfSplitParams& p, hipStream_t s);
 
 #ifndef FV_RING
 #define FV_RING 2
diff --git a/fastvocoder_amd/csrc/mrfh_launch.hip b/fastvocoder_amd/csrc/mrfh_launch.hip
--- a/fastvocoder_amd/csrc/mrfh_launch.hip
+++ b/fastvocoder_amd/csrc/mrfh_launch.hip
@@ -1,3 +1,7 @@
+#include <string.h>
+#include <array>
+#include <map>
+#include <mutex>
 #include "launch_host.hpp"
 
 namespace fv {
@@ -60,4 +64,139 @@
     return C == 32 ? launch_mrfw_geom(p, s) : shape == 1 ? launch_mrfh_geom<2, 16>(p, s) : launch_mrfh_geom<3, 12>(p, s);
 }
 
-}
+constexpr int kMrfwW = 384, kMrfwReachA = 60, kMrfwReachB = 36;
+static long long mrfw_windows(long long cols, int reach) {
+    const long long first = kMrfwW - 2 * reach, next = kMrfwW - reach;
+    return cols <= first ? 1 : 1 + (cols - first + next - 1) / next;
+}
+static long long mrfw_window_cols(long long windows, int reach) { return (kMrfwW - 2 * reach) + (windows - 1) * (long long)(kMrfwW - reach); }
+static long long mrfw_class_cut(int B, int T, int n, int reach, unsigned* range, int* used) {
+    long long worst = 0;
+    for (int u = 0; u < B; ++u) {
+        const int m = n / B + (u < n % B ? 1 : 0);
+        const long long w = mrfw_windows((T + m - 1) / m, reach), cols = mrfw_window_cols(w, reach);
+        if (w > worst) worst = w;
+        if (!range) continue;
+        for (long long a = 0; a < T; a += cols) {
+            range[2 * *used] = (unsigned)((long long)u * T + a);
+            range[2 * *used + 1] = (unsigned)((long long)u * T + (a + cols < T ? a + cols : T));
+            ++*used;
+        }
+    }
+    return worst;
+}
+
+bool mrf_class_plan(int B, int T, int nblk, bool force, MrfClassPlan& out) {
+    if (B < 1 || T < 1 || nblk < 1 || nblk > kSchedBlocks || (double)B * T >= 2147483647.0) return false;
+    const Tuning& tn = tuning();
+    typedef std::array<long long, 7> Key;
+    static std::mutex mu;
+    static std::map<Key, MrfClassPlan> cache;
+    const Key key = {B, T, nblk, force, tn.mrf_cost_a, tn.mrf_cost_b, tn.mrf_cost_one};
+    std::lock_guard<std::mutex> lock(mu);
+    auto it = cache.find(key);
+    if (it == cache.end()) {
+        MrfClassPlan pl = {};
+        const long long total = (long long)B * T;
+        long long worst_one = 0;
+        for (int i = 0; i < nblk; ++i) {
+            const long long lo = total * i / nblk, hi = total * (i + 1) / nblk;
+            long long w = 0;
+            for (long long a = lo; a < hi;) {
+                const long long end = (a / T + 1) * T < hi ? (a / T + 1) * T : hi;
+                w += mrfw_windows(end - a, kMrfwReachA);
+                a = end;
+            }
+            if (w > worst_one) worst_one = w;
+        }
+        pl.makespan_one = worst_one * tn.mrf_cost_one;
+        int best = 0;
+        long long best_span = 0, best_sum = 0;
+        for (int na = B; nblk - na >= B; ++na) {
+            const long long ta = mrfw_class_cut(B, T, na, kMrfwReachA, nullptr, nullptr) * tn.mrf_cost_a;
+            const long long tb = mrfw_class_cut(B, T, nblk - na, kMrfwReachB, nullptr, nullptr) * tn.mrf_cost_b;
+            const long long span = ta > tb ? ta : tb;
+            if (!best || span < best_span || (span == best_span && ta + tb < best_sum)) {
+                best = na;
+                best_span = span;
+                best_sum = ta + tb;
+            }
+        }
+        if (best && (force || best_span < pl.makespan_one)) {
+            pl.split = 1;
+            pl.makespan = best_span;
+            pl.reach_a = kMrfwReachA;
+            pl.reach_b = kMrfwReachB;
+            int used = 0;
+            mrfw_class_cut(B, T, best, kMrfwReachA, pl.range, &used);
+            pl.n_a = used;
+            mrfw_class_cut(B, T, nblk - best, kMrfwReachB, pl.range, &used);
+            pl.n_b = used - pl.n_a;
+        } else {
+            pl.makespan = pl.makespan_one;
+            pl.n_b = nblk;
+            pl.reach_b = kMrfwReachA;
+            for (int i = 0; i < nblk; ++i) {
+                pl.range[2 * i] = (unsigned)(total * i / nblk);
+                pl.range[2 * i + 1] = (unsigned)(total * (i + 1) / nblk);
+            }
+        }
+        if (cache.size() >= 64) cache.clear();
+        it = cache.emplace(key, pl).first;
+    }
+    out = it->second;
+    return true;
+}
+
+int launch_mrfw_split(MrfSplitParams p, const int* dil, hipStream_t s, int one_class) {
+    const char* const fam = "mrf stage (two classes)";
+    if (p.B <= 0 || p.T <= 0) return 0;
+    if (!dil || dil[0] != 1 || dil[1] != 3 || dil[2] != 5 || p.k[0] != 3 || p.k[1] != 7 || p.k[2] != 11)
+        return fail(FV_ERR_UNSUPPORTED, "%s: 32 channels, taps (3, 7, 11) in this order -- the sum r_0 + r_1 is the reference's first "
+                    "-- and dilations (1, 3, 5)", fam);
+    if (one_class) p.y2 = p.y;
+    if (!p.x || !p.blob || !p.y || !p.y2) return fail(FV_ERR_INVALID_ARG, "%s: null tensor", fam);
+    if (p.y == p.x || p.y2 == p.x || (p.y == p.y2 && !one_class)) return fail(FV_ERR_INVALID_ARG, "%s: an output tensor aliases the input or the other output", fam);
+    if ((reinterpret_cast<uintptr_t>(p.blob) & 15) != 0) return fail(FV_ERR_UNSUPPORTED, "%s: the packed stage must be 16-byte aligned", fam);
+    if (int rc = check_desc_range(fam, 32, p.T)) return rc;
+    if ((double)p.B * p.T >= 2147483647.0) return fail(FV_ERR_UNSUPPORTED, "%s: B x T = %d x %d columns exceed 2^31", fam, p.B, p.T);
+    if (int rc = check_slopes(fam, p.slope, 1.f)) return rc;
+    unsigned off = 0;
+    double flops = 0;
+    for (int j = 0; j < 3; ++j)
+        for (int q = 0; q < 3; ++q) {
+            p.blk_off[3 * j + q] = off;
+            off += (unsigned)mrf_block_bytes(32, p.k[j]);
+            flops += 2.0 * 2.0 * p.B * 32.0 * 32.0 * p.k[j] * p.T;
+        }
+    p.blob_bytes = off;
+    p.halo = kMrfwReachA;
+    p.halo_b = kMrfwReachB;
+    if (p.halo != mrf_halo(p.k, dil)) return fail(FV_ERR_UNSUPPORTED, "%s: reach", fam);
+    p.ol = 0;
+    p.total = (long long)p.B * p.T;
+    long long nblk = persistent_blocks((p.total + 127) / 128, 1, tuning().mrf_blocks);
+    if (nblk > kSchedBlocks) nblk = kSchedBlocks;
+    if (nblk < 2LL * p.B) return fail(FV_ERR_UNSUPPORTED, "%s: %lld blocks for %d utterances (two per utterance at least)", fam, nblk, p.B);
+    MrfClassPlan pl;
+    if (!mrf_class_plan(p.B, p.T, (int)nblk, true, pl) || !pl.split) return fail(FV_ERR_UNSUPPORTED, "%s: no plan", fam);
+    p.n_a = pl.n_a;
+    p.nblk = pl.n_a + pl.n_b;
+    memcpy(p.range, pl.range, sizeof(p.range));
+    if (one_class == 1) {
+        p.nblk = pl.n_a;
+    } else if (one_class == 2) {
+        p.n_a = 0;
+        p.nblk = pl.n_b;
+        memcpy(p.range, pl.range + 2 * pl.n_a, sizeof(unsigned) * 2 * (size_t)pl.n_b);
+    }
+    if (!p.hist || p.hist_bytes < (long long)p.nblk * kMrfwHistBytes || (reinterpret_cast<uintptr_t>(p.hist) & 15) != 0)
+        return fail(FV_ERR_WORKSPACE, "%s: a 16-byte aligned workspace of fv_mrf_stage_workspace_bytes (%lld bytes for %d blocks; given %lld)",
+                    fam, (long long)p.nblk * kMrfwHistBytes, p.nblk, p.hist ? p.hist_bytes : 0LL);
+    p.prio = tuning().mrf_prio;
+    p.trace = trace_buffer();
+    ProfileScope prof(s, FV_KERNEL_MRF32, Work{flops, 4.0 * 3.0 * p.B * 32.0 * p.T + off});
+    return launch_mrfw_split_geom(p, s);
+}
+
+}
diff --git a/fastvocoder_amd/csrc/mrfw_inst.hip b/fastvocoder_amd/csrc/mrfw_inst.hip
--- a/fastvocoder_amd/csrc/mrfw_inst.hip
+++ b/fastvocoder_amd/csrc/mrfw_inst.hip
@@ -12,4 +12,13 @@
     return 0;
 }
 
+int launch_mrfw_split_geom(const MrfSplitParams& p, hipStream_t s) {
+    typedef MrfwTile<3, 8> TL;
+    auto kern = mrfw_kernel<3, 8, 1, 3, 5, false, true>;
+    if (int rc = allow_dynamic_lds(reinterpret_cast<const void*>(kern), TL::LDS)) return rc;
+    hipLaunchKernelGGL(kern, dim3(p.nblk), dim3(TL::NT), TL::LDS, s, p);
+    FV_HIP(hipGetLastError());
+    return 0;
 }
+
+}
diff --git a/fastvocoder_amd/csrc/mrfw_kernels.hpp b/fastvocoder_amd/csrc/mrfw_kernels.hpp
--- a/fastvocoder_amd/csrc/mrfw_kernels.hpp
+++ b/fastvocoder_amd/csrc/mrfw_kernels.hpp
@@ -1,4 +1,5 @@
 #pragma once
+#include <type_traits>
 #include "mrfh_kernels.hpp"
 
 namespace fv {
@@ -280,11 +281,12 @@
 __device__ __forceinline__ void mrfw_block_run(const MrfParams& p, const MrfwLane<TL>& L, float* wbuf, int& par, int j, int pnext,
                                                float (&xr)[2][TL::NF][4], const float (&x0)[2][TL::NF][4], bool write_next,
                                                MrfwWhen wh, bool zero_after, LowGuard& low, __amdgpu_buffer_rsrc_t rb,
-                                               __amdgpu_buffer_rsrc_t rh, unsigned next_off, int next_kb, int tile_no) {
+                                               __amdgpu_buffer_rsrc_t rh, unsigned next_off, int next_kb, int tile_no,
+                                               int j_first = 0, int j_last = 2) {
     constexpr int KB0 = 4 * mrfw_piece_taps(KT, 0);
     const int q0 = 3 * j;
     const float* const bl = reinterpret_cast<const float*>(L.sm + TL::OFF_B) + q0 * (TL::TAIL / 4);
-    const int h0 = q0 * TL::HSLOT, hn = (j == 2 ? 0 : q0 + 3) * TL::HSLOT;
+    const int h0 = q0 * TL::HSLOT, hn = (j == j_last ? 3 * j_first : q0 + 3) * TL::HSLOT;
     const unsigned o0 = p.blk_off[q0], o1 = p.blk_off[q0 + 1], o2 = p.blk_off[q0 + 2];
     mrfw_pair<TL, KT, D0, 0>(p, L, wbuf, par, bl, xr, x0, true, wh, h0, h0 + TL::HSLOT, (KT - 1) * D1 / 2, low, rb, rh, o0, o1, KB0,
                              tile_no, q0);
@@ -295,8 +297,10 @@
                              rh, o2, next_off, next_kb, tile_no, q0 + 2);
 }
 
-template <int NF, int NG, int D0, int D1, int D2, bool FOLD>
-__global__ __launch_bounds__(64 * NG) __attribute__((amdgpu_waves_per_eu((NG + 3) / 4, (NG + 3) / 4))) void mrfw_kernel(MrfParams p) {
+template <int NF, int NG, int D0, int D1, int D2, bool FOLD, bool SPLIT = false>
+__global__ __launch_bounds__(64 * NG) __attribute__((amdgpu_waves_per_eu((NG + 3) / 4, (NG + 3) / 4)))
+void mrfw_kernel(std::conditional_t<SPLIT, MrfSplitParams, MrfParams> p) {
+    static_assert(!(SPLIT && FOLD), "a class stores its sum: nothing to fold an output conv into");
     typedef MrfwTile<NF, NG> TL;
     extern __shared__ __attribute__((aligned(16))) float smem[];
     char* const sm = reinterpret_cast<char*>(smem);
@@ -319,7 +323,14 @@
     char* const mimg0 = sm + TL::OFF_M;
     float* const wbuf = smem + TL::OFF_W / 4;
     float* const scratch = smem + TL::OFF_S / 4;
-    const int T = p.T, halo = p.halo, ol = p.ol;
+    int j_lo = 0, j_hi = 3, halo_c = p.halo;
+    if constexpr (SPLIT) {
+        const bool class_a = (int)blockIdx.x < p.n_a;
+        j_lo = class_a ? 2 : 0;
+        j_hi = class_a ? 3 : 2;
+        halo_c = class_a ? p.halo : p.halo_b;
+    }
+    const int T = p.T, halo = halo_c, ol = p.ol;
     const int vcols = TL::W - halo;
     const int adv = vcols - 2 * ol;
     const int k0 = p.k[0], k1 = p.k[1], k2 = p.k[2];
@@ -328,8 +339,15 @@
     const __amdgpu_buffer_rsrc_t rb = make_rsrc(p.blob, p.blob_bytes);
     const __amdgpu_buffer_rsrc_t rh = make_rsrc(p.hist + (size_t)blockIdx.x * (9 * TL::HSLOT / 4), p.hist ? 9 * TL::HSLOT : 0);
 
-    const int share = xcd_remap((int)blockIdx.x, (int)gridDim.x);
-    const long long g_lo = p.total * share / p.nblk, g_hi = p.total * (share + 1) / p.nblk;
+    long long g_lo, g_hi;
+    if constexpr (SPLIT) {
+        g_lo = p.range[2 * blockIdx.x];
+        g_hi = p.range[2 * blockIdx.x + 1];
+    } else {
+        const int share = xcd_remap((int)blockIdx.x, (int)gridDim.x);
+        g_lo = p.total * share / p.nblk;
+        g_hi = p.total * (share + 1) / p.nblk;
+    }
     if (g_lo >= g_hi) return;
     MrfIter it;
     mrf_first(it, g_lo, g_hi, T, halo, ol, vcols);
@@ -337,6 +355,14 @@
     const unsigned t4 = (unsigned)T * 4u, ubytes = (unsigned)TL::C * (unsigned)T * 4u;
     const size_t ustride = (size_t)TL::C * (size_t)T;
     float x0[2][NF][4], xr[2][NF][4], sum[2][NF][4];
+    if constexpr (SPLIT) {
+#pragma unroll
+        for (int h = 0; h < 2; ++h)
+#pragma unroll
+            for (int f = 0; f < NF; ++f)
+#pragma unroll
+                for (int i = 0; i < 4; ++i) sum[h][f][i] = 0.f;
+    }
     auto load_x0 = [&](const MrfIter& at) {
         const __amdgpu_buffer_rsrc_t rx = make_rsrc(p.x + at.b * ustride, ubytes);
 #pragma unroll
@@ -363,7 +389,12 @@
         }
     }
     load_x0(it);
-    mrfw_dma<NG>(rb, wbuf, off0, 4 * (k0 < 4 ? k0 : 4), L.wave, L.lane);
+    if constexpr (SPLIT) {
+        const int kf = j_lo == 0 ? k0 : k2;
+        mrfw_dma<NG>(rb, wbuf, j_lo == 0 ? off0 : off6, 4 * (kf < 4 ? kf : 4), L.wave, L.lane);
+    } else {
+        mrfw_dma<NG>(rb, wbuf, off0, 4 * (k0 < 4 ? k0 : 4), L.wave, L.lane);
+    }
     for (int idx = L.tid; idx < 2 * 8 * 2 * TL::FM * 4; idx += TL::NT) {
         const int dw = idx & 3, row = (idx >> 2) % TL::FM, fb = (idx >> 2) / TL::FM % 2, part = (idx >> 2) / (2 * TL::FM) % 8,
                   im = (idx >> 2) / (16 * TL::FM);
@@ -404,24 +435,29 @@
         wh.save = more && !it.cold;
         wh.zero_mid = wh.zero_next = cur.cold;
 #pragma unroll 1
-        for (int j = 0; j < 3; ++j) {
-            const int kj = j == 0 ? k0 : j == 1 ? k1 : k2, kn = j == 0 ? k1 : j == 1 ? k2 : k0;
-            const unsigned offn = j == 0 ? off3 : j == 1 ? off6 : off0;
-            const int kbn = (j < 2 || more) ? 4 * (kn < 4 ? kn : 4) : 0;
+        for (int j = SPLIT ? j_lo : 0; j < (SPLIT ? j_hi : 3); ++j) {
+            auto last_j = [&] { return SPLIT ? j == j_hi - 1 : j == 2; };
+            auto inner_j = [&] { return SPLIT ? j < j_hi - 1 : j < 2; };
+            const int jn = SPLIT ? (j == j_hi - 1 ? j_lo : j + 1) : 0;
+            const int kj = j == 0 ? k0 : j == 1 ? k1 : k2;
+            const int kn = SPLIT ? (jn == 0 ? k0 : jn == 1 ? k1 : k2) : (j == 0 ? k1 : j == 1 ? k2 : k0);
+            const unsigned offn = SPLIT ? (jn == 0 ? off0 : jn == 1 ? off3 : off6) : (j == 0 ? off3 : j == 1 ? off6 : off0);
+            const int kbn = (inner_j() || more) ? 4 * (kn < 4 ? kn : 4) : 0;
             const int pnext = (kn - 1) * D0 / 2;
-            const bool zero_after = j == 2 ? !wh.save : cur.cold;
+            const bool zero_after = last_j() ? !wh.save : cur.cold;
 #pragma unroll
             for (int h = 0; h < 2; ++h)
 #pragma unroll
                 for (int f = 0; f < NF; ++f)
 #pragma unroll
                     for (int i = 0; i < 4; ++i) xr[h][f][i] = x0[h][f][i];
-            if (j == 2 && more) load_x0(it);
-            const bool wn = j < 2 || more;
-            if (kj == 11) mrfw_block_run<TL, 11, D0, D1, D2>(p, L, wbuf, par, j, pnext, xr, x0, wn, wh, zero_after, low, rb, rh, offn, kbn, tile_no);
-            else if (kj == 7) mrfw_block_run<TL, 7, D0, D1, D2>(p, L, wbuf, par, j, pnext, xr, x0, wn, wh, zero_after, low, rb, rh, offn, kbn, tile_no);
-            else mrfw_block_run<TL, 3, D0, D1, D2>(p, L, wbuf, par, j, pnext, xr, x0, wn, wh, zero_after, low, rb, rh, offn, kbn, tile_no);
-            if (j < 2) {
+            if (last_j() && more) load_x0(it);
+            const bool wn = inner_j() || more;
+            const int jf = SPLIT ? j_lo : 0, jl = SPLIT ? j_hi - 1 : 2;
+            if (kj == 11) mrfw_block_run<TL, 11, D0, D1, D2>(p, L, wbuf, par, j, pnext, xr, x0, wn, wh, zero_after, low, rb, rh, offn, kbn, tile_no, jf, jl);
+            else if (kj == 7) mrfw_block_run<TL, 7, D0, D1, D2>(p, L, wbuf, par, j, pnext, xr, x0, wn, wh, zero_after, low, rb, rh, offn, kbn, tile_no, jf, jl);
+            else mrfw_block_run<TL, 3, D0, D1, D2>(p, L, wbuf, par, j, pnext, xr, x0, wn, wh, zero_after, low, rb, rh, offn, kbn, tile_no, jf, jl);
+            if (inner_j()) {
 #pragma unroll
                 for (int h = 0; h < 2; ++h)
 #pragma unroll
@@ -431,7 +467,24 @@
             }
         }
         if (tile_no == 0) mrf_stamp(p, NG, L.wave, L.lane, 2, 2);
-        if constexpr (FOLD) {
+        if constexpr (SPLIT) {
+            const bool two = j_hi - j_lo > 1;
+            const __amdgpu_buffer_rsrc_t ry = make_rsrc((j_lo == 0 ? p.y : p.y2) + cur.b * ustride, ubytes);
+#pragma unroll
+            for (int h = 0; h < 2; ++h)
+#pragma unroll
+                for (int f = 0; f < NF; ++f) {
+                    float out[4];
+#pragma unroll
+                    for (int i = 0; i < 4; ++i) out[i] = two ? sum[h][f][i] + xr[h][f][i] : xr[h][f][i];
+                    const int t = cur.tw + L.colw + f * 16;
+                    const bool ok = t >= cur.lo && t < cur.hi;
+                    range_note4(bad, out[0], out[1], out[2], out[3], ok);
+                    const unsigned voff = ok ? (unsigned)((L.row0 + 16 * h) * T + t) * 4u : kOutOfRange;
+#pragma unroll
+                    for (int i = 0; i < 4; ++i) buffer_store1s(ry, voff, (unsigned)i * t4, out[i]);
+                }
+        } else if constexpr (FOLD) {
             char* const sb = mimg0;
 #pragma unroll
             for (int h = 0; h < 2; ++h) {
diff --git a/fastvocoder_amd/csrc/plan.hip b/fastvocoder_amd/csrc/plan.hip
--- a/fastvocoder_amd/csrc/plan.hip
+++ b/fastvocoder_amd/csrc/plan.hip
@@ -434,6 +434,21 @@
     return 0;
 }
 
+int fv_plan_add_mrf_stage_classes_f16(fv_plan_t* plan, int x_slot, int ys_slot, int yr2_slot, const float* packed, int C,
+                                      const int* k, const int* dil, float slope, void* workspace, int64_t workspace_bytes) {
+    if (C != 32 || yr2_slot == FV_SLOT_NONE || yr2_slot == ys_slot)
+        return fail(FV_ERR_UNSUPPORTED, "plan_add_mrf_stage_classes: 32 channels and two distinct output slots");
+    if (int rc = fv_plan_add_mrf_stage_split_f16(plan, x_slot, ys_slot, yr2_slot, packed, C, k, dil, slope, 1.f, FV_POST_NONE, 1.f,
+                                                 workspace, workspace_bytes))
+        return rc;
+    if (k[0] != 3 || k[1] != 7 || k[2] != 11) {
+        plan->ops.pop_back();
+        return fail(FV_ERR_UNSUPPORTED, "plan_add_mrf_stage_classes: taps (3, 7, 11) in this order");
+    }
+    plan->ops.back().classes = true;
+    return 0;
+}
+
 int fv_plan_add_resblock_pair(fv_plan_t* plan, int x_slot, int y_slot, int y_act_slot, const float* packed1,
                               const float* packed2, const float* bias1, const float* bias2, int C, int k, int dil,
                               float slope, float act_slope) {
@@ -679,6 +694,8 @@
 
 static int run_stage(const Run& r, const Op& o) {
     float* const y = r.base[o.y];
+    if (o.classes)
+        return launch_mrfw_split(mrf_split_params(o, r.base[o.x], y, r.at(o.y2), r.B, r.T(o), r.guard()), o.sdil, r.s);
     return launch_mrfh(mrf_params(o, r.base[o.x], o.fold_w ? nullptr : y, o.fold_w ? nullptr : r.at(o.y2), o.fold_w ? y : nullptr,
                                   r.B, r.T(o), r.guard()),
                        o.Cin, o.sdil, r.s);
diff --git a/fastvocoder_amd/generator/engine.py b/fastvocoder_amd/generator/engine.py
--- a/fastvocoder_amd/generator/engine.py
+++ b/fastvocoder_amd/generator/engine.py
@@ -239,9 +239,15 @@
                 and all([c.dilation[0] for c in b.convs1] == dils for b in blocks)
                 and all(self.pair_fusable(c1, c2, _native.PAIR_SPLIT_F16) for b in blocks for c1, c2 in zip(b.convs1, b.convs2)))
 
-    def mrf_stage(self, blocks, src, dst, slope, out_div, fold=None):
+    def mrf_stage_classes_supported(self, blocks):
+        return (self.mrf_stage_supported(blocks) and blocks[0].channels == 32
+                and [b.convs1[0].kernel_size[0] for b in blocks] == [3, 7, 11])
+
+    def mrf_stage(self, blocks, src, dst, slope, out_div, fold=None, classes_r2=SLOT_NONE):
         if not self.mrf_stage_supported(blocks):
             raise _native.NativeError("mrf stage: shape not built into the one-launch kernel")
+        if classes_r2 != SLOT_NONE and (fold is not None or not self.mrf_stage_classes_supported(blocks)):
+            raise _native.NativeError("mrf stage: two block classes exist at 32 channels, taps (3, 7, 11), without a folded conv")
         ks = [b.convs1[0].kernel_size[0] for b in blocks]
         dils = [c.dilation[0] for c in blocks[0].convs1]
         c1s = [c for b in blocks for c in b.convs1]
@@ -257,6 +263,8 @@
                 raise _native.NativeError("mrf stage: this output conv cannot be folded into the stage")
             op.update(fold_w=effective_weight(out_conv).detach().float().reshape(blocks[0].channels, 7).contiguous(),
                       fold_b=self._bias(out_conv), fold_post=fpost, act_slope=float(fslope))
+        if classes_r2 != SLOT_NONE:
+            op.update(out_div=1.0, y2=classes_r2, tmps=[classes_r2])
         self.ops.append(op)
 
     def conv_split_supported(self, conv, pad, pad_mode=PAD_ZERO):
@@ -316,12 +324,16 @@
                              post=post))
 
     def conv_transpose_takes_merge(self, convt):
+        return self.conv_transpose_merges(convt, self.precision)
+
+    @classmethod
+    def conv_transpose_merges(cls, convt, precision):
         if not isinstance(convt, torch.nn.ConvTranspose1d) or convt.groups != 1 or convt.dilation[0] != 1:
             return False
         k, s = convt.kernel_size[0], convt.stride[0]
-        return ((self.SPLIT_CONVT_MIN_CIN <= convt.in_channels <= 128
+        return ((cls.SPLIT_CONVT_MIN_CIN <= convt.in_channels <= 128
                  or _native.conv_transpose_small(convt.in_channels, convt.out_channels, k, s))
-                and self.pair_precision(convt.in_channels) == _native.PAIR_SPLIT_F16
+                and pair_precision(precision, convt.in_channels) == _native.PAIR_SPLIT_F16
                 and _native.conv_transpose_split_supported(convt.in_channels, convt.out_channels, k, s, convt.padding[0],
                                                            convt.output_padding[0]))
 
@@ -444,7 +456,7 @@
     def receptive_halo(self):
         need = {}
         for op in reversed(self.ops):
-            h_out = max(need.pop(op["y"], 0), need.pop(op.get("y_act", SLOT_NONE), 0))
+            h_out = max(need.pop(op["y"], 0), need.pop(op.get("y_act", SLOT_NONE), 0), need.pop(op.get("y2", SLOT_NONE), 0))
             if op["kind"] == "conv":
                 reach = op["dil"] * (op["k"] - 1)
                 own, rate = max(op["pad"], reach - op["pad"]), 1
@@ -508,6 +520,11 @@
                                             post=op["post"], mid=op["mid"])
                 if "fold_w" in op:
                     self.plan.set_pair_output_conv(op["fold_w"], op["fold_b"], op["y"], op["act_slope"], op["fold_post"])
+            elif op["kind"] == "stage" and "y2" in op:
+                if op["y_act"] != SLOT_NONE or op["act_slope"] != 1.0:
+                    raise _native.NativeError("mrf stage in two classes: its sums are stored raw")
+                self.plan.add_mrf_stage_classes(op["x"], op["y"], op["y2"], op["packed"], op["channels"], op["ks"], op["dils"],
+                                                op["slope"])
             elif op["kind"] == "stage":
                 self.plan.add_mrf_stage(op["x"], op["y"], op["packed"], op["channels"], op["ks"], op["dils"], op["slope"],
                                         out_div=op["out_div"], y_act=op["y_act"], act_slope=op["act_slope"])
@@ -608,7 +625,7 @@
     def _fv_policy(self):
         prec = "f32" if (self.precision == "f32" or self._fv_overflow or getattr(self, "_fv_force_f32", False)) else "split"
         return (prec, bool(self.fuse_pairs), bool(self.fold_post), self.range_guard != "off", bool(self.merge_in_upsampler),
-                self.fuse_stage if isinstance(self.fuse_stage, tuple) else bool(self.fuse_stage))
+                tuple(self.fuse_stage) if isinstance(self.fuse_stage, (tuple, list)) else bool(self.fuse_stage))
 
     def _fv_state(self):
         if self._fv_tensors is None or self._fv_epoch != _registration_epoch[0]:
diff --git a/fastvocoder_amd/generator/hifigan.py b/fastvocoder_amd/generator/hifigan.py
--- a/fastvocoder_amd/generator/hifigan.py
+++ b/fastvocoder_amd/generator/hifigan.py
@@ -1,5 +1,6 @@
 import torch
 
+from .. import _native
 from .._native import PAIR_SPLIT_F16
 from .engine import (GradPrecision, NativeModule, PlanBuilder, POST_TANH, SLOT_IN, SLOT_NONE, SLOT_OUT, pair_precision,
                      weight_norm)
@@ -21,6 +22,28 @@
     share = -(-cols // nblk)
     windows = 1 if share <= 264 else 1 + -(-(share - 264) // 324)
     return share >= fill * 384 * windows
+
+
+_STAGE32_US_PER_UNIT = 70.5 / 1490
+_STAGE32_ONE_FIXED_US, _STAGE32_CLASSES_FIXED_US, _STAGE32_CLASSES_SHARING = 10.0, 8.0, 1.17
+_STAGE32_PAIRS_FIXED_US, _STAGE32_PAIRS_US_PER_COLUMN_CU = 24.0, 0.97e-3 * 256
+
+
+def stage32_form(batch, t, cus):
+    cols = int(batch) * int(t)
+    base = "s" if stage32_windows_fit(cols, cus) else "pairs"
+    nblk = max(1, min(int(cus), 256, -(-cols // 128)))
+    if cols <= 0 or nblk < 2 * int(batch):
+        return base
+    plan = _native.mrf_class_schedule(batch, t, nblk)
+    if not plan["split"]:
+        return base
+    classes_us = _STAGE32_CLASSES_FIXED_US + _STAGE32_CLASSES_SHARING * plan["makespan"] * _STAGE32_US_PER_UNIT
+    if base == "s":
+        base_us = _STAGE32_ONE_FIXED_US + plan["makespan_one"] * _STAGE32_US_PER_UNIT
+    else:
+        base_us = _STAGE32_PAIRS_FIXED_US + _STAGE32_PAIRS_US_PER_COLUMN_CU * cols / int(cus)
+    return "c" if classes_us < base_us else base
 
 
 class _HiFiGANBase(GradPrecision, NativeModule):
@@ -97,22 +120,39 @@
                 t = (t - 1) * up.stride[0] - 2 * up.padding[0] + up.kernel_size[0] + up.output_padding[0]
             fusable = t > 0 and t % 4 == 0 and self._stage_fusable(i, precision)
             ch = self.resblocks[i * self.num_kernels].channels
-            flags.append("s" if fusable and self._stage_one_launch(ch, t) else bool(fusable))
+            form = self._stage_one_launch(ch, t, classes=self._stage_classes_possible(i, precision)) if fusable else False
+            flags.append(form or bool(fusable))
         return tuple(flags)
 
-    def _stage_one_launch(self, channels, t):
+    def _stage_classes_possible(self, i, precision):
+        nk = self.num_kernels
+        if not (self.merge_in_upsampler and nk == 3 and i + 1 < self.num_upsamples):
+            return False
+        blocks = [self.resblocks[i * nk + j] for j in range(nk)]
+        ks = [b.convs1[0].kernel_size[0] for b in blocks]
+        dils = [c.dilation[0] for c in blocks[0].convs1]
+        return (blocks[0].channels == 32 and ks == [3, 7, 11] and _native.mrf_stage_supported(32, ks, dils)
+                and pair_precision(precision, 32) == PAIR_SPLIT_F16
+                and PlanBuilder.conv_transpose_merges(self.ups[i + 1], precision))
+
+    def _stage_one_launch(self, channels, t, classes=False):
         fs = self.fuse_stage
         if isinstance(fs, (tuple, list)):
-            return channels in fs
+            if any(isinstance(v, str) and v != "32c" for v in fs):
+                raise _native.NativeError(f"fuse_stage = {fs!r}: channel counts, and \"32c\" for the 32-channel stage in two classes")
+            return "c" if channels == 32 and classes and "32c" in fs else "s" if channels in fs else False
         if not fs or channels == 16:
-            return bool(fs)
+            return "s" if fs else False
         if channels != 32:
             return False
         dev = self._device()
         cus = _CU_COUNT.get(dev)
         if cus is None:
             cus = _CU_COUNT[dev] = torch.cuda.get_device_properties(dev).multi_processor_count
-        return stage32_windows_fit(getattr(self, "_fv_batch", 1) * int(t), cus)
+        if not classes:
+            return "s" if stage32_windows_fit(getattr(self, "_fv_batch", 1) * int(t), cus) else False
+        form = stage32_form(getattr(self, "_fv_batch", 1), int(t), cus)
+        return False if form == "pairs" else form
 
     def _emit_fused_stage(self, pb, blocks, up, x, scratch, parts, fold=None, merge_next=False, one_launch=False):
         nk = len(blocks)
@@ -208,7 +248,7 @@
                 pb.upsample_conv(self.ups[i], x, up, pre_slope=LRELU_SLOPE)
             else:
                 pb.conv_transpose(self.ups[i], x, up, pre_slope=LRELU_SLOPE,
-                                  merge=(parts[0], parts[1], float(nk)) if merged else None)
+                                  merge=(parts[0], SLOT_NONE if merged == "two" else parts[1], float(nk)) if merged else None)
             merged = False
             blocks = [self.resblocks[i * nk + j] for j in range(nk)]
             if fused is not None and fused[i]:
@@ -220,6 +260,12 @@
                           and pb.pair_precision(blocks[0].channels) == PAIR_SPLIT_F16
                           and pb.conv_transpose_takes_merge(self.ups[i + 1])
                           and not (fused[i] == "s" and pb.mrf_stage_supported(blocks)))
+                if fused[i] == "c":
+                    if not (merged and pb.mrf_stage_classes_supported(blocks)):
+                        raise _native.NativeError("stage flagged for two block classes cannot run so")
+                    pb.mrf_stage(blocks, up, x, LRELU_SLOPE, float(nk), classes_r2=parts[0])
+                    merged = "two"
+                    continue
                 self._emit_fused_stage(pb, blocks, up, x, scratch, parts, merge_next=merged, one_launch=fused[i] == "s")
                 continue
             if nk <= 3:
@@ -267,8 +313,11 @@
     def _flag_tag(self, T):
         return "".join("s" if f == "s" else "f" if f else "-" for f in self._fused_flags(T))
 
+    def _plan_tag(self, T):
+        return "".join(f if f in ("s", "c") else "f" if f else "-" for f in self._fused_flags(T))
+
     def _trunk_plan(self, T):
-        return self._plan(lambda: "trunk" + self._flag_tag(T),
+        return self._plan(lambda: "trunk" + self._plan_tag(T),
                           lambda pb: self._emit_trunk(pb, SLOT_OUT, self._fused_flags(T), fold_post=True), 80)
 
     def _emit_inference(self, pb, fused):
@@ -278,7 +327,7 @@
         def emit(pb):
             self._emit_inference(pb, self._fused_flags(T))
             pb.subtract_output(0, second=True)
-        return self._plan(lambda: "minus" + self._flag_tag(T), emit, 80)
+        return self._plan(lambda: "minus" + self._plan_tag(T), emit, 80)
 
     def inference_minus(self, x, bias):
         x = self._prepare(x).transpose(1, 0).unsqueeze(0).contiguous()
@@ -338,7 +387,7 @@
         self._emit_full(pb, fused)
 
     def _full_plan(self, T):
-        return self._plan(lambda: "inference" + self._flag_tag(T),
+        return self._plan(lambda: "inference" + self._plan_tag(T),
                           lambda pb: self._emit_full(pb, self._fused_flags(T)), 80)
 
     def inference(self, x):
diff --git a/include/fastvocoder_hip.h b/include/fastvocoder_hip.h
--- a/include/fastvocoder_hip.h
+++ b/include/fastvocoder_hip.h
@@ -77,6 +77,8 @@
                            const int* dil, float slope, float out_div, int post, float act_slope, const float* fold_w,
                            const float* fold_b, float* fold_y, void* workspace, int64_t workspace_bytes, int* guard,
                            void* stream);
+int fv_mrf_stage_classes_f16(const float* x, const float* packed, float* y_s, float* y_r2, int B, int C, int T, const int* k,
+                             const int* dil, float slope, void* workspace, int64_t workspace_bytes, int* guard, void* stream);
 
 int fv_conv1d_split_f16(int n, const float* const* x, const float* const* packed, const float* const* bias,
                         const float* const* res, const float* const* add1, const float* const* add2, float* const* y,
@@ -380,6 +382,8 @@
 int fv_plan_add_mrf_stage_split_f16(fv_plan_t* plan, int x_slot, int y_slot, int y_act_slot, const float* packed, int C,
                                     const int* k, const int* dil, float slope, float out_div, int post, float act_slope,
                                     void* workspace, int64_t workspace_bytes);
+int fv_plan_add_mrf_stage_classes_f16(fv_plan_t* plan, int x_slot, int ys_slot, int yr2_slot, const float* packed, int C,
+                                      const int* k, const int* dil, float slope, void* workspace, int64_t workspace_bytes);
 int fv_plan_add_conv1d_split_f16(fv_plan_t* plan, int x_slot, int y_slot, int y_act_slot, int res_slot, int add1_slot,
                                  int add2_slot, const float* packed, const float* bias, int C, int k, int dil,
                                  int pad_mode, float pre_slope, float out_div, int post, float act_slope);
@@ -430,6 +434,9 @@
 int fv_tuning_set(const char* key, int value);
 int fv_debug_pair_schedule(int n_members, const int* n_items, const int* cost, int nblk, int mode, int three_members,
                            unsigned* table);
+int fv_debug_mrf_class_schedule(int B, int T, int nblk, int force, int64_t* info, unsigned* table);
+int fv_debug_mrf_stage_class_f16(const float* x, const float* packed, float* y, int cls, int B, int C, int T, const int* k,
+                                 const int* dil, float slope, void* workspace, int64_t workspace_bytes, void* stream);
 
 #define FV_KERNEL_CONV_MFMA32 0
 #define FV_KERNEL_CONV_MFMA16 1
```

Result: faster. 404.4 million samples/s, median of 6 (+2.6%).
